# arhik/GaussianSplat

Hardware: AMD Instinct MI355X
Metric: fwd+bwd Msplats/sec at 1M Gaussians, 1920x1080, SH deg 3 (higher is better)
Workload: dtype f32; 1 GPU; C3: 1000000 gaussians, 1920x1080, SH3, ONE camera view per step, fwd+bwd; the steps cycle over the cameras [0, 4] (view k: eye rotated about +y by 45k degrees; one view slot per camera); synthetic scene of SURVEY 8d with the quaternions NORMALISED (8d leaves N(0,1)^4 raw: the reference never normalises q and |q| scales every footprint by |q|^4; un-normalised q is parity-tested, tests/test_gpu_size; views_per_rank=1, nranks=1, settle_steps=24, rank_mode=1, binning_rounds=1, schedule=3, view_slots=True, order=depth_desc, tile=16, instances=30150056, coarse_instances=2175944, walked_fwd=8350144, alpha_cull=True, list_cap=0, tile_parts=1, lists_capped=False

## Files before the change

### gaussiansplat_amd/backend.py

```python
from __future__ import annotations

import ctypes as C
import os
from collections import namedtuple

import numpy as np

_HERE = os.path.dirname(os.path.abspath(__file__))
LIB_PATH = os.environ.get("GSPLAT_HIP_LIB") or os.path.join(_HERE, "lib", "libgsplat_hip.so")

GS_MEM_HOST, GS_MEM_DEVICE = 0, 1
ORDER_INDEX, ORDER_DEPTH_DESC, ORDER_DEPTH_ASC = 0, 1, 2

(ARR_TS, ARR_TPS, ARR_MU, ARR_COV3D, ARR_COV2D, ARR_INVCOV, ARR_BBS, ARR_RGB, ARR_SIG, ARR_DEPTH_KEY,
 ARR_TILE_RECT, ARR_SORT_IDXS, ARR_TILE_RANGES, ARR_SORTED_IDS, ARR_SORTED_KEYS, ARR_GRAD2D) = range(16)

STAGES = ("preprocess", "depth_sort", "count_scan", "emit", "tile_sort", "ranges", "composite_fwd",
          "composite_bwd", "preprocess_bwd")

GS_CAMERA_GRAD_FLOATS = 40
GS_METRIC_SUMS = 4
GS_EXPOSURE_FLOATS = 12
(METRIC_MSE, METRIC_MAE, METRIC_SSIM, METRIC_PSNR, GS_METRIC_COUNT) = range(5)
GS_ABI_VERSION = 3
GS_DEBUG_WIDE_CURSORS = 1
GS_DEBUG_ALWAYS_ORDER = 2
GS_DEBUG_SUPER16 = 8
GS_DEBUG_SUPER8 = 16
GS_DEBUG_NO_TAIL_FILL = 32
GS_DEBUG_TINY_CAPS = 4
GS_MAX_VIEW_SLOTS = 4096
GS_BWD_OVERWRITE, GS_BWD_COMPOSITE_ONLY, GS_BWD_PARAMS_ONLY, GS_BWD_PARAMS_SH, GS_BWD_PARAMS_GEOM = 1, 2, 4, 8, 16
GS_ADAM_GROUPS = 6
GS_ADAM_SELECTIVE = 1
GS_ERR_INVALID, GS_ERR_UNSUPPORTED = -1, -5
KNN_BOX = 64
TOUCHED_CHUNK = 256


class GsConfig(C.Structure):
    _fields_ = [("struct_size", C.c_int32), ("abi_version", C.c_int32), ("tile_size", C.c_int32), ("order", C.c_int32), ("t_min", C.c_float),
                ("deterministic", C.c_int32), ("export_debug", C.c_int32), ("profile_stages", C.c_int32),
                ("bin_path", C.c_int32), ("rank_mode", C.c_int32), ("alpha_cull", C.c_int32), ("schedule", C.c_int32),
                ("slab_mode", C.c_int32), ("slab_max_ratio", C.c_float), ("slab_fractions", C.c_float * 3), ("debug_flags", C.c_int32),
                ("depth_sort", C.c_int32), ("list_cap", C.c_int32), ("tile_parts", C.c_int32), ("reserved", C.c_int32 * 3)]


class GsGrads(C.Structure):
    _fields_ = [("d_means", C.c_void_p), ("d_scales", C.c_void_p), ("d_quats", C.c_void_p),
                ("d_opacities", C.c_void_p), ("d_shs", C.c_void_p)]


class GsDensityStats(C.Structure):
    _fields_ = [("grad_sum", C.c_void_p), ("count", C.c_void_p), ("max_extent", C.c_void_p)]


class GsDensityParams(C.Structure):
    _fields_ = [("struct_size", C.c_int32), ("grad_threshold", C.c_float), ("log_split_scale", C.c_float), ("log_shrink", C.c_float),
                ("min_opacity_logit", C.c_float), ("log_max_world_scale", C.c_float), ("max_extent_px", C.c_int32)]


class GsError(RuntimeError):
    def __init__(self, code: int, msg: str):
# ... 47 lines not shown
    "gs_adam_step": Sig(_i, [_vp, _G, _G, _G, _fp, _f, _f, _f, _i64, _i]),
    "gs_backward_adam": Sig(_i, [_vp, _vp, _i, _G, _G, _fp, _f, _f, _f, _i64, _i]),
    "gs_density_accumulate": Sig(_i, [_vp, C.POINTER(GsDensityStats)]),
    "gs_density_decide": Sig(_i, [_vp, C.POINTER(GsDensityStats), C.POINTER(GsDensityParams), _vp]),
    "gs_density_plan": Sig(_i, [_vp, _vp, _i64p]),
    "gs_density_restructure": Sig(_i, [_vp, _vp, _vp, _G, _i32, _G, _G, _i64]),
    "gs_opacity_reset": Sig(_i, [_vp, _f, _vp, _vp]),
    "gs_mcmc_plan": Sig(_i, [_vp, _f, _vp, _vp, _i64p]),
    "gs_mcmc_sample": Sig(_i, [_vp, _vp, _i64, _vp, _i64, _vp]),
    "gs_mcmc_relocate": Sig(_i, [_vp, _vp, _vp, _i64, _f, _i32, _G]),
    "gs_mcmc_noise": Sig(_i, [_vp, _vp, _f, _f, _f]),
    "gs_mcmc_regularize": Sig(_i, [_vp, _G, _f, _f]),
    "gs_knn_mean_dist2": Sig(_i, [_vp, _vp, _i64, _vp]),
    "gs_init_from_points": Sig(_i, [_vp, _vp, _vp, _vp, _i64, _i, _f, _G]),
    "gs_view_depth": Sig(_i, [_vp, _vp]),
    "gs_view_depth_backward": Sig(_i, [_vp, _vp, _vp]),
    "gs_render_features": Sig(_i, [_vp, _vp, _vp, _vp]),
    "gs_backward_features": Sig(_i, [_vp, _vp, _vp, _vp, _vp, _G]),
    "gs_backward_camera": Sig(_i, [_vp, _vp, _i]),
    "gs_image_metrics": Sig(_i, [_vp, _vp, _vp, _vp, _i32, _i32, _i32, _vp, _vp, _i]),
    "gs_metrics_finish": Sig(_i, [_dp, _dp]),
    "gs_exposure_apply": Sig(_i, [_vp, _vp, _vp, _vp, _i32, _i32, _vp]),
    "gs_exposure_backward": Sig(_i, [_vp, _vp, _vp, _vp, _vp, _i32, _i32, _vp, _vp]),
    "gs_exposure_adam": Sig(_i, [_vp, _vp, _vp, _vp, _vp, _f, _f, _f, _f, _i64]),
    "gs_num_gaussians": Sig(_i64, [_vp]),
    "gs_num_instances": Sig(_i64, [_vp]),
    "gs_num_coarse_instances": Sig(_i64, [_vp]),
    "gs_num_rounds": Sig(_i, [_vp]),
    "gs_get_array": Sig(_i, [_vp, _i, _vp, _i64]),
    "gs_get_stage_times": Sig(_i, [_vp, _fp]),
    "gs_get_stage_stats": Sig(_i, [_vp, _dp, _i64p, _i]),
    "gs_get_work_counters": Sig(_i, [_vp, _i64p, _i64p]),
    "gs_get_list_stats": Sig(_i, [_vp, _i64p]),
    "gs_get_tile_parts": Sig(_i, [_vp]),
    "gs_get_bin_path": Sig(_i, [_vp]),
    "gs_get_work_counters_ex": Sig(_i, [_vp, _i64p]),
    "gs_debug_time_composite": Sig(_i, [_vp, _i, _i, _i, _fp]),
    "gs_debug_tile_clock": Sig(_i, [_vp, _i, _i, _vp]),
    "gs_debug_tile_clock_rows": Sig(_i, [_vp]),
    "gs_debug_tail_fill": Sig(_i, [_vp, _i32p], optional=True),
    "gs_debug_clock_mhz": Sig(_i, [_vp, _fp]),
    "gs_debug_set_window": Sig(_i, [_vp, _i32, _i32]),
    "gs_rank_probe_result": Sig(_i, [_vp]),
}
SYMBOLS = tuple(ABI)

_lib = None


def load():
    global _lib
    if _lib is not None:
        return _lib
    try:
        import torch
    except ImportError:
        pass
    if not os.path.exists(LIB_PATH):
        raise FileNotFoundError(f"{LIB_PATH} not found: build it with `python -m gaussiansplat_amd.build` "
                                "(there is no CPU fallback)")
    L = C.CDLL(LIB_PATH)
    for name, sig in ABI.items():
        try:
            f = getattr(L, name)
        except AttributeError:
            if sig.optional:
# ... 388 lines not shown
                ARR_BBS: ((n, 4), np.float32), ARR_RGB: ((n, 3), np.float32), ARR_SIG: ((n,), np.float32),
                ARR_DEPTH_KEY: ((n,), np.uint32), ARR_TILE_RECT: ((n, 4), np.uint16), ARR_SORT_IDXS: ((n,), np.uint32),
                ARR_SORTED_IDS: ((ni,), np.uint32), ARR_SORTED_KEYS: ((ni,), np.uint64), ARR_GRAD2D: ((n, 10), np.float32)}
        if which == ARR_TILE_RANGES:
            ntiles = ((self.W + 15) // 16) * ((self.H + 15) // 16)
            shape, dt = (ntiles, 2), np.uint32
        else:
            shape, dt = spec[which]
        out = np.empty(shape, dt)
        self._chk(self.L.gs_get_array(self.h, which, out.ctypes.data, out.nbytes))
        return out

    def stage_stats(self, reset: bool = False) -> dict:
        sm = (C.c_double * len(STAGES))()
        ct = (C.c_int64 * len(STAGES))()
        self._chk(self.L.gs_get_stage_stats(self.h, sm, ct, int(reset)))
        return {k: (float(sm[i]), int(ct[i])) for i, k in enumerate(STAGES)}

    def work_counters(self):
        a, b = C.c_int64(), C.c_int64()
        self._chk(self.L.gs_get_work_counters(self.h, C.byref(a), C.byref(b)))
        return int(a.value), int(b.value)

    def work_counters_ex(self) -> dict:
        o = (C.c_int64 * 4)()
        self._chk(self.L.gs_get_work_counters_ex(self.h, o))
        return dict(walked_fwd=int(o[0]), walked_bwd=int(o[1]), evaluated_fwd=int(o[2]), evaluated_bwd=int(o[3]))

    def list_stats(self) -> dict:
        o = (C.c_int64 * 3)()
        self._chk(self.L.gs_get_list_stats(self.h, o))
        return dict(listed=int(o[0]), extended_segments=int(o[1]), capped=bool(o[2]))

    def tile_parts_of_frame(self) -> int:
        rc = self.L.gs_get_tile_parts(self.h)
        if rc < 0:
            self._chk(rc)
        return int(rc)

    def bin_path_of_frame(self) -> int:
        rc = self.L.gs_get_bin_path(self.h)
        if rc < 0:
            self._chk(rc)
        return int(rc)

    def time_composite(self, which: int, variant: int, reps: int = 10) -> float:
        ms = C.c_float()
        self._chk(self.L.gs_debug_time_composite(self.h, which, variant, reps, C.byref(ms)))
        return float(ms.value)

    def tile_clock(self, which: int, variant: int = 0) -> np.ndarray:
        ntiles = ((self.W + 15) // 16) * ((self.H + 15) // 16)
        rows = ntiles
        if variant < 0:
            rows = int(self.L.gs_debug_tile_clock_rows(self.h))
            if rows <= 0:
                raise GsError(-1, "tile_clock: records by workgroup need a frame with a launch order")
        out = np.zeros((rows, 15), np.uint64)
        self._chk(self.L.gs_debug_tile_clock(self.h, which, variant, out.ctypes.data))
        return out

    def tail_fill_blocks(self):
        o = (C.c_int32 * 2)()
        self._chk(self.L.gs_debug_tail_fill(self.h, o))
        return int(o[0]), int(o[1])

# ... 20 lines not shown
```

### gaussiansplat_amd/csrc/gs_adam.hip

```cpp
#include "gs_ctx.h"
#include "gs_adam.h"
#include "gs_wave.h"

#define GS_ADAM_ROWS 64
#define GS_ADAM_MAX_BLOCKS 2048

namespace {

struct AdamSeg {
    float *p;
    const float *g;
    float *m, *v;
    int64_t len;
    int64_t units;
    int w;
    int sh;
    int vec;
    int lds_off;
    float ss;
};
struct AdamArgs {
    AdamSeg seg[5];
    int nseg;
    int64_t n;
// ... 156 lines not shown
    if (!grads || !exp_avg || !exp_avg_sq) return fail(c, GS_ERR_INVALID, "gs_adam_step: NULL argument");
    const Five<float> p = c->model5_mut(), g = five(*grads), m = five(*exp_avg), v = five(*exp_avg_sq);
    AdamArgs a{};
    if (const int rc = gs_adam_prepare(c, "gs_adam_step", p.p, g.p, m.p, v.p, lr, beta1, beta2, eps, step, flags, &a.h)) return rc;
    if (bind_device(c)) return GS_ERR_HIP;
    const int64_t n = c->n;
    int64_t most = 0;
    int lds = 0;
    for (int i = 0; i < 5; ++i) {
        if (!g[i] || n <= 0) continue;
        AdamSeg &s = a.seg[a.nseg++];
        s.p = p[i]; s.g = g[i]; s.m = m[i]; s.v = v[i];
        s.w = (int)c->width[i]; s.len = (int64_t)s.w * n;
        s.sh = i == 4; s.ss = a.h.step_size[i < 4 ? i : 4];
        s.vec = ((reinterpret_cast<uintptr_t>(s.p) | reinterpret_cast<uintptr_t>(s.g) | reinterpret_cast<uintptr_t>(s.m) |
                  reinterpret_cast<uintptr_t>(s.v)) & 15) == 0;
        s.units = s.vec ? (s.len + 3) / 4 : s.len;
        s.lds_off = lds; lds += GS_ADAM_ROWS * s.w;
        most = std::max(most, s.units);
    }
    a.n = n;
    if (a.nseg) {
        if (flags & GS_ADAM_SELECTIVE) {
            const int64_t npass = (n + GS_ADAM_ROWS - 1) / GS_ADAM_ROWS;
            const unsigned grid = (unsigned)std::min<int64_t>(npass, GS_ADAM_MAX_BLOCKS);
            hipLaunchKernelGGL(gs_adam_selective_kernel, dim3(grid), dim3(256), sizeof(float) * lds, c->stream, a);
        } else {
            const unsigned grid = (unsigned)std::min<int64_t>((most + 255) / 256, GS_ADAM_MAX_BLOCKS);
            hipLaunchKernelGGL(gs_adam_dense_kernel, dim3(grid), dim3(256), 0, c->stream, a);
        }
        HIPCHK(c, hipGetLastError());
    }
    c->inputs_changed();
    return GS_OK;
}
```

### gaussiansplat_amd/csrc/gs_api.hip

```cpp
#include "gs_ctx.h"

std::string g_create_error;

template <typename A> static int preprocess_outputs(gs_ctx *c, A &a) {
    a.gx = c->gx; a.gy = c->gy;
    a.payload = c->payload.as<GsPayload>(); a.invcov = c->invcov.as<float>(); a.depth_key = c->depth_key.as<uint32_t>(); a.rect = c->rect.as<uint16_t>();
    if (!c->cfg.export_debug) return GS_OK;
    for (int i = 0; i < gs_ctx::DBG_COUNT; ++i) HIPCHK(c, c->dbg[i].ensure(sizeof(float) * gs_ctx::DBG_WIDTH[i] * c->n1()));
    auto arr = [c](gs_ctx::Dbg i) { return c->dbg[i].as<float>(); };
    a.dbg.mu = arr(gs_ctx::DBG_MU); a.dbg.cov2d = arr(gs_ctx::DBG_COV2D); a.dbg.invcov = arr(gs_ctx::DBG_INVCOV); a.dbg.bbs = arr(gs_ctx::DBG_BBS);
    if (c->kind == 0) { a.dbg.ts = arr(gs_ctx::DBG_TS); a.dbg.tps = arr(gs_ctx::DBG_TPS); a.dbg.cov3d = arr(gs_ctx::DBG_COV3D); }
    return GS_OK;
}

extern "C" {

void gs_default_config(gs_config *cfg) {
    if (!cfg) return;
    std::memset(cfg, 0, sizeof(*cfg));
    cfg->struct_size = (int32_t)sizeof(gs_config);
    cfg->abi_version = GS_ABI_VERSION;
    cfg->tile_size = GS_TILE;
    cfg->order = GS_ORDER_DEPTH_DESC;
    cfg->t_min = 1e-5f;
    cfg->deterministic = 0;
    cfg->export_debug = 0;
    cfg->profile_stages = 0;
    cfg->rank_mode = 1;
    cfg->alpha_cull = 1;
    cfg->schedule = 3;
    cfg->slab_mode = 1;
}

int gs_abi_version(void) { return GS_ABI_VERSION; }

const char *gs_last_error(const gs_ctx *ctx) { return ctx ? ctx->err.c_str() : g_create_error.c_str(); }

int gs_create(gs_ctx **out, int device, const gs_config *cfg) {
    if (!out) return fail(nullptr, GS_ERR_INVALID, "gs_create: out is NULL");
    *out = nullptr;
    gs_config c0;
    gs_default_config(&c0);
    if (cfg) {
        if (cfg->struct_size != (int32_t)sizeof(gs_config) || cfg->abi_version != GS_ABI_VERSION)
            return fail(nullptr, GS_ERR_INVALID, "gs_create: gs_config.struct_size / abi_version mismatch (caller built against another gsplat.h)");
        c0 = *cfg;
    }
    if (c0.schedule == 0) c0.schedule = 3;
    if (c0.tile_size != GS_TILE) return fail(nullptr, GS_ERR_UNSUPPORTED, "gs_create: only tile_size 16 is supported (reference threads=(16,16))");
    if (c0.order < GS_ORDER_INDEX || c0.order > GS_ORDER_DEPTH_ASC) return fail(nullptr, GS_ERR_INVALID, "gs_create: bad order");
    if (!(c0.t_min >= 0.0f)) return fail(nullptr, GS_ERR_INVALID, "gs_create: t_min must be >= 0");
    if (c0.schedule != 1 && c0.schedule != 3 && c0.schedule != 4) return fail(nullptr, GS_ERR_INVALID, "gs_create: bad schedule (0, 1, 3 or 4)");
    if (c0.slab_mode < 0 || c0.slab_mode > 1) return fail(nullptr, GS_ERR_INVALID, "gs_create: bad slab_mode");
    if (c0.bin_path < 0 || c0.bin_path > 3) return fail(nullptr, GS_ERR_INVALID, "gs_create: bad bin_path");
    if (!(c0.slab_max_ratio >= 0.0f && c0.slab_max_ratio <= 1.0f)) return fail(nullptr, GS_ERR_INVALID, "gs_create: slab_max_ratio must be in [0, 1]");
    for (int i = 0; i < 3; ++i)
        if (!(c0.slab_fractions[i] >= 0.0f && c0.slab_fractions[i] < 1.0f)) return fail(nullptr, GS_ERR_INVALID, "gs_create: slab_fractions must be in [0, 1)");
    if (c0.debug_flags & ~(GS_DEBUG_WIDE_CURSORS | GS_DEBUG_ALWAYS_ORDER | GS_DEBUG_TINY_CAPS | GS_DEBUG_SUPER16 | GS_DEBUG_SUPER8 | GS_DEBUG_NO_TAIL_FILL)) return fail(nullptr, GS_ERR_INVALID, "gs_create: unknown debug_flags");
    if (c0.depth_sort < 0 || c0.depth_sort > 2) return fail(nullptr, GS_ERR_INVALID, "gs_create: depth_sort must be 0, 1 or 2");
    if (c0.list_cap < 0 || c0.list_cap > 2) return fail(nullptr, GS_ERR_INVALID, "gs_create: list_cap must be 0, 1 or 2");
    if (c0.tile_parts != 0 && c0.tile_parts != 1 && c0.tile_parts != 2 && c0.tile_parts != 4) return fail(nullptr, GS_ERR_INVALID, "gs_create: tile_parts must be 0, 1, 2 or 4");
    int ndev = 0;
    hipError_t e = hipGetDeviceCount(&ndev);
    if (e != hipSuccess || ndev <= 0)
        return fail(nullptr, GS_ERR_NO_DEVICE, "gs_create: no HIP device (this library has no CPU fallback)");
    if (device < 0 || device >= ndev) return fail(nullptr, GS_ERR_INVALID, "gs_create: device index out of range");
    gs_ctx *c = new (std::nothrow) gs_ctx();
    if (!c) return fail(nullptr, GS_ERR_OOM, "gs_create: host allocation failed");
    c->device = device;
    c->cfg = c0;
    c->slots.resize(GS_MAX_VIEW_SLOTS + 1);
    if ((e = hipSetDevice(device)) != hipSuccess) { delete c; return hipfail(nullptr, e, "hipSetDevice"); }
    if ((e = hipStreamCreateWithFlags(&c->stream, hipStreamNonBlocking)) != hipSuccess) { delete c; return hipfail(nullptr, e, "hipStreamCreate"); }
    c->own_stream = true;
    {
        hipDeviceProp_t prop;
        if (hipGetDeviceProperties(&prop, device) == hipSuccess && prop.multiProcessorCount > 0) c->wave_slots = prop.multiProcessorCount * 4 * 5;
        else (void)hipGetLastError();
    }
    if ((e = hipHostMalloc((void **)&c->pinned, sizeof(PinnedWords), hipHostMallocCoherent | hipHostMallocMapped)) != hipSuccess) { delete c; return hipfail(nullptr, e, "hipHostMalloc"); }
    if ((e = hipHostMalloc((void **)&c->pinned_split, sizeof(uint32_t) * 2 * (GS_MAX_VIEW_SLOTS + 1), hipHostMallocCoherent | hipHostMallocMapped)) != hipSuccess) {
        (void)hipGetLastError(); c->pinned_split = nullptr;
    } else std::memset(c->pinned_split, 0, sizeof(uint32_t) * 2 * (GS_MAX_VIEW_SLOTS + 1));
    for (auto &pair : c->ev)
        for (hipEvent_t &ev : pair) if ((e = hipEventCreate(&ev)) != hipSuccess) { delete c; return hipfail(nullptr, e, "hipEventCreate"); }
    if ((e = hipEventCreateWithFlags(&c->ev_count, hipEventDisableTiming | hipEventReleaseToSystem)) != hipSuccess) { delete c; return hipfail(nullptr, e, "hipEventCreate"); }
    if ((e = hipStreamCreateWithFlags(&c->side, hipStreamNonBlocking)) != hipSuccess) { delete c; return hipfail(nullptr, e, "hipStreamCreate"); }
    for (hipEvent_t *ev : {&c->ev_main, &c->ev_order})
        if ((e = hipEventCreateWithFlags(ev, hipEventDisableTiming)) != hipSuccess) { delete c; return hipfail(nullptr, e, "hipEventCreate"); }
    if (c->cfg.rank_mode == 0) {
        int bad = 0;
        if ((e = gs_probe_lds_atomic_order(c->stream, &bad)) != hipSuccess) { delete c; return hipfail(nullptr, e, "gs_probe_lds_atomic_order"); }
        c->rank_probe = bad ? 1 : 0;
        if (bad) c->cfg.rank_mode = 1;
    }
    *out = c;
    return GS_OK;
}

int gs_destroy(gs_ctx *c) {
    if (!c) return GS_OK;
    (void)hipSetDevice(c->device);
    (void)hipStreamSynchronize(c->stream);
    if (c->side) (void)hipStreamSynchronize(c->side);
    delete c;
    return GS_OK;
}

int gs_set_stream(gs_ctx *c, void *hip_stream) {
    if (!c) return GS_ERR_INVALID;
    hipStream_t want = hip_stream == (void *)1 ? (hipStream_t) nullptr : (hipStream_t)hip_stream;
    if (hip_stream && !c->own_stream && c->stream == want && c->borrowed_stream) return GS_OK;
    if (bind_device(c)) return GS_ERR_HIP;
    HIPCHK(c, hipStreamSynchronize(c->stream));
    if (c->side) HIPCHK(c, hipStreamSynchronize(c->side));
    if (c->own_stream && c->stream) { (void)hipStreamDestroy(c->stream); c->own_stream = false; }
    if (hip_stream) { c->stream = want; c->borrowed_stream = true; }
    else { HIPCHK(c, hipStreamCreateWithFlags(&c->stream, hipStreamNonBlocking)); c->own_stream = true; c->borrowed_stream = false; }
    return GS_OK;
}

int gs_synchronize(gs_ctx *c) {
    if (!c) return GS_ERR_INVALID;
    if (bind_device(c)) return GS_ERR_HIP;
    HIPCHK(c, hipStreamSynchronize(c->stream));
    if (c->side) HIPCHK(c, hipStreamSynchronize(c->side));
    return GS_OK;
}

static int adopt_model(gs_ctx *c, int64_t n, int sh_degree, int kind, const float *const src[5], const size_t (&width)[5], int mem) {
    if (bind_device(c)) return GS_ERR_HIP;
    const float *dst[5];
    for (int i = 0; i < 5; ++i) {
        dst[i] = src[i];
        if (mem != GS_MEM_HOST) continue;
        const size_t bytes = sizeof(float) * width[i] * (size_t)n;
        HIPCHK(c, c->model[i].ensure(bytes ? bytes : 4));
        if (bytes) HIPCHK(c, hipMemcpyAsync(c->model[i].p, src[i], bytes, hipMemcpyHostToDevice, c->stream));
        dst[i] = c->model[i].as<float>();
    }
    if (mem == GS_MEM_HOST) HIPCHK(c, hipStreamSynchronize(c->stream));
    c->n = n; c->sh_degree = sh_degree; c->kind = kind;
    for (int i = 0; i < 5; ++i) c->width[i] = width[i];
    c->set_model5(dst);
    c->inputs_changed();
    return GS_OK;
}

int gs_set_model(gs_ctx *c, int64_t n, int sh_degree, const float *means, const float *scales, const float *quats,
                 const float *opacities, const float *shs, int mem) {
    if (!c) return GS_ERR_INVALID;
    if (n < 0 || n > 0x7FFFFFF0LL) return fail(c, GS_ERR_INVALID, "gs_set_model: n out of range");
    if (sh_degree < 0 || sh_degree > 3) return fail(c, GS_ERR_UNSUPPORTED, "gs_set_model: sh_degree must be 0..3");
    if (n > 0 && (!means || !scales || !quats || !opacities || !shs)) return fail(c, GS_ERR_INVALID, "gs_set_model: NULL array");
    if (const int rc = need_mem(c, "gs_set_model", mem)) return rc;
    const int K = (sh_degree + 1) * (sh_degree + 1);
    const float *src[5] = {means, scales, quats, opacities, shs};
    return adopt_model(c, n, sh_degree, 0, src, {3, 3, 4, 1, (size_t)3 * K}, mem);
}

int gs_set_model_2d(gs_ctx *c, int64_t n, const float *means, const float *scales, const float *rotations,
                    const float *opacities, const float *colors, int mem) {
    if (!c) return GS_ERR_INVALID;
    if (n < 0 || n > 0x7FFFFFF0LL) return fail(c, GS_ERR_INVALID, "gs_set_model_2d: n out of range");
    if (n > 0 && (!means || !scales || !rotations || !opacities || !colors)) return fail(c, GS_ERR_INVALID, "gs_set_model_2d: NULL array");
    if (const int rc = need_mem(c, "gs_set_model_2d", mem)) return rc;
    const float *src[5] = {means, scales, rotations, opacities, colors};
    return adopt_model(c, n, 0, 1, src, {2, 2, 1, 1, 3}, mem);
}

int gs_set_active_sh_degree(gs_ctx *c, int degree) {
    if (!c) return GS_ERR_INVALID;
    if (const int rc = need_3d(c, "gs_set_active_sh_degree")) return rc;
    if (degree < -1 || degree > 3) return fail(c, GS_ERR_INVALID, "gs_set_active_sh_degree: degree must be -1 (the model's own) or 0..3");
    const int before = c->active_sh_degree();
    c->sh_active_request = degree;
    if (c->active_sh_degree() != before) c->inputs_changed();
    return GS_OK;
}

int gs_get_active_sh_degree(const gs_ctx *c) {
    if (!c) return GS_ERR_INVALID;
    if (c->kind != 0) return GS_ERR_UNSUPPORTED;
    return c->active_sh_degree();
}

int gs_set_background(gs_ctx *c, const float rgb[3]) {
    if (!c) return GS_ERR_INVALID;
    if (!rgb) return fail(c, GS_ERR_INVALID, "gs_set_background: NULL argument");
    for (int i = 0; i < 3; ++i)
        if (!std::isfinite(rgb[i])) return fail(c, GS_ERR_INVALID, "gs_set_background: the components must be finite");
    if (rgb[0] == c->background[0] && rgb[1] == c->background[1] && rgb[2] == c->background[2]) return GS_OK;
    for (int i = 0; i < 3; ++i) c->background[i] = rgb[i];
    c->fall_back(gs_ctx::Stage::BINNED);
    return GS_OK;
}

int gs_get_background(const gs_ctx *c, float rgb[3]) {
    if (!c || !rgb) return GS_ERR_INVALID;
    for (int i = 0; i < 3; ++i) rgb[i] = c->background[i];
    return GS_OK;
}

int gs_compose_target(gs_ctx *c, const float *rgba, int32_t W, int32_t H, float *rgb_out) {
    if (!c) return GS_ERR_INVALID;
    if (!rgba || !rgb_out) return fail(c, GS_ERR_INVALID, "gs_compose_target: NULL argument");
    if (const int rc = need_image_size(c, "gs_compose_target", W, H)) return rc;
    const size_t px = (size_t)W * H;
    if (overlaps({rgb_out, sizeof(float) * 3 * px}, {rgba, sizeof(float) * 4 * px})) return fail(c, GS_ERR_INVALID, "gs_compose_target: rgb_out overlaps rgba");
    if (bind_device(c)) return GS_ERR_HIP;
    HIPCHK(c, gs_launch_compose_target(rgba, rgb_out, px, c->background, c->stream));
    return GS_OK;
}

int gs_set_image_size(gs_ctx *c, int32_t W, int32_t H) {
    if (!c) return GS_ERR_INVALID;
    if (const int rc = need_image_size(c, "gs_set_image_size", W, H)) return rc;
    if (!c->have_cam) {
        std::memset(&c->cam, 0, sizeof(c->cam));
        c->cam.near_ = -1.0f; c->cam.far_ = 1.0f;
    }
    c->cam.W = W; c->cam.H = H;
    c->have_cam = true;
    c->inputs_changed();
    return GS_OK;
}

int gs_set_camera(gs_ctx *c, const float T[16], const float P[16], float fx, float fy, float near_, float far_,
                  const float eye[3], const float lookAt[3], int32_t W, int32_t H) {
    if (!c) return GS_ERR_INVALID;
    if (!T || !P || !eye || !lookAt) return fail(c, GS_ERR_INVALID, "gs_set_camera: NULL argument");
    if (const int rc = need_image_size(c, "gs_set_camera", W, H)) return rc;
    std::memcpy(c->cam.T, T, sizeof(float) * 16);
    std::memcpy(c->cam.P, P, sizeof(float) * 16);
    c->cam.fx = fx; c->cam.fy = fy; c->cam.near_ = near_; c->cam.far_ = far_;
    for (int i = 0; i < 3; ++i) { c->cam.eye[i] = eye[i]; c->cam.lookAt[i] = lookAt[i]; }
    c->cam.W = W; c->cam.H = H;
    c->have_cam = true;
    c->inputs_changed();
    return GS_OK;
}

int gs_preprocess(gs_ctx *c) {
    if (!c) return GS_ERR_INVALID;
    if (!c->have_cam) return fail(c, GS_ERR_INVALID, "gs_preprocess: gs_set_camera first");
    if (bind_device(c)) return GS_ERR_HIP;
    if (int rc = settle_totals(c, nullptr, false)) return rc;
    c->frame_id += 1;
    HIPCHK(c, c->payload.ensure(sizeof(GsPayload) * c->n1()));
    HIPCHK(c, c->invcov.ensure(sizeof(float) * 4 * c->n1()));
    HIPCHK(c, c->depth_key.ensure(sizeof(uint32_t) * c->n1()));
    HIPCHK(c, c->rect.ensure(sizeof(uint16_t) * 4 * c->n1()));
    c->gx = (c->cam.W + GS_TILE - 1) / GS_TILE;
    c->gy = (c->cam.H + GS_TILE - 1) / GS_TILE;
    c->range_valid = false;
    GsPreprocessArgs a{};
    GsPreprocess2DArgs a2{};
    if (c->kind == 1) {
        a2.n = c->n; a2.W = c->cam.W; a2.H = c->cam.H;
        a2.means = c->means; a2.scales = c->scales; a2.rots = c->quats; a2.opac = c->opac; a2.colors = c->shs;
        if (int rc = preprocess_outputs(c, a2)) return rc;
    } else {
        model_head(c, a);
        a.order = c->cfg.order;
        if (c->dsort_can_bucket() && c->order() != GS_ORDER_INDEX && c->n > 0 && !c->small_bin_possible()) {
            if (!c->key_range.p) {
                HIPCHK(c, c->key_range.ensure(sizeof(uint32_t) * gs_depth_range_words()));
                HIPCHK(c, gs_depth_range_reset(c->key_range.as<uint32_t>(), c->stream));
            }
            c->range_parity ^= 1;
            a.key_range = key_range_of(c, c->range_parity);
            c->range_valid = true;
        }
        if (int rc = preprocess_outputs(c, a)) return rc;
    }
    StageTimer t(c, GS_STAGE_PREPROCESS);
    HIPCHK(c, c->kind == 1 ? gs_launch_preprocess2d(a2, c->stream) : gs_launch_preprocess(a, c->cam, c->sh_row_floats(), c->stream));
    c->reach(gs_ctx::Stage::PREPROCESSED);
    return GS_OK;
}

int gs_loss_l1_dssim(gs_ctx *c, const float *img, const float *gt, int32_t W, int32_t H, int32_t C, float lam, float *dC,
                     double *loss_out, int mem) {
    if (!c || !img || !gt) return GS_ERR_INVALID;
    if (W <= 0 || H <= 0 || C <= 0) return fail(c, GS_ERR_INVALID, "gs_loss_l1_dssim: bad image size");
    if (const int rc = need_mem(c, "gs_loss_l1_dssim", mem)) return rc;
    if (bind_device(c)) return GS_ERR_HIP;
    const size_t n = (size_t)W * H * C;
    HIPCHK(c, c->loss_maps.ensure(sizeof(float) * 3 * n));
    HIPCHK(c, c->loss_acc.ensure(sizeof(double) * GS_LOSS_SLOTS * GS_LOSS_SLOT_STRIDE));
    const float *d_img = img, *d_gt = gt;
    float *d_dc = dC;
    if (mem == GS_MEM_HOST) {
        HIPCHK(c, c->loss_in[0].ensure(sizeof(float) * n));
        HIPCHK(c, c->loss_in[1].ensure(sizeof(float) * n));
        HIPCHK(c, hipMemcpyAsync(c->loss_in[0].p, img, sizeof(float) * n, hipMemcpyHostToDevice, c->stream));
        HIPCHK(c, hipMemcpyAsync(c->loss_in[1].p, gt, sizeof(float) * n, hipMemcpyHostToDevice, c->stream));
        d_img = c->loss_in[0].as<float>(); d_gt = c->loss_in[1].as<float>();
    }
    if (mem == GS_MEM_HOST || !dC) { HIPCHK(c, c->loss_dc.ensure(sizeof(float) * n)); d_dc = c->loss_dc.as<float>(); }
    float win[121];
    {
        double k[121], sum = 0.0;
        for (int j = 0; j < 11; ++j)
            for (int i = 0; i < 11; ++i) { k[j * 11 + i] = std::exp(-std::sqrt((double)((5 - j) * (5 - j) + (5 - i) * (5 - i)))); sum += k[j * 11 + i]; }
        for (int i = 0; i < 121; ++i) win[i] = (float)(k[i] / sum);
    }
    HIPCHK(c, gs_loss_run(W, H, C, d_img, d_gt, c->loss_maps.as<float>(), c->loss_acc.as<double>(), d_dc, lam, win, c->stream));
    if (mem == GS_MEM_HOST && dC) HIPCHK(c, hipMemcpyAsync(dC, d_dc, sizeof(float) * n, hipMemcpyDeviceToHost, c->stream));
    if (loss_out) {
        double slots[GS_LOSS_SLOTS * GS_LOSS_SLOT_STRIDE], acc[2] = {0.0, 0.0};
        HIPCHK(c, hipMemcpyAsync(slots, c->loss_acc.p, sizeof(slots), hipMemcpyDeviceToHost, c->stream));
        HIPCHK(c, hipStreamSynchronize(c->stream));
        for (int k = 0; k < GS_LOSS_SLOTS; ++k) { acc[0] += slots[k * GS_LOSS_SLOT_STRIDE]; acc[1] += slots[k * GS_LOSS_SLOT_STRIDE + 1]; }
        *loss_out = (1.0 - (double)lam) * acc[0] / (2.0 * (double)n) + (double)lam * (1.0 - acc[1] / (double)n) / 2.0;
    } else if (mem == GS_MEM_HOST) {
        HIPCHK(c, hipStreamSynchronize(c->stream));
    }
    return GS_OK;
}

int gs_sgd_step(gs_ctx *c, float lr, const gs_grads *g) {
    if (!c || !g) return GS_ERR_INVALID;
    if (bind_device(c)) return GS_ERR_HIP;
    const size_t n = (size_t)c->n;
    const Five<float> p = c->model5_mut(), gr = five(*g);
    for (int i = 0; i < 5; ++i) HIPCHK(c, gs_launch_sgd(p[i], gr[i], lr, c->width[i] * n, c->stream));
    c->inputs_changed();
    return GS_OK;
}

int gs_reset_grads(gs_ctx *c, const gs_grads *g) {
    if (!c || !g) return GS_ERR_INVALID;
    if (bind_device(c)) return GS_ERR_HIP;
    const size_t n = (size_t)c->n;
    const Five<float> p = five(*g);
    for (int i = 0; i < 5; ++i)
        if (p[i] && n) HIPCHK(c, hipMemsetAsync(p[i], 0, sizeof(float) * c->width[i] * n, c->stream));
    return GS_OK;
}

int gs_grads_alloc(gs_ctx *c, gs_grads *out) {
    if (!c || !out) return GS_ERR_INVALID;
    if (bind_device(c)) return GS_ERR_HIP;
    const size_t n = (size_t)c->n;
    size_t off[6] = {0, 0, 0, 0, 0, 0};
    for (int i = 0; i < 5; ++i) off[i + 1] = off[i] + c->width[i] * n;
    const size_t total = off[5];
    HIPCHK(c, c->grads_flat.ensure(sizeof(float) * (total ? total : 1)));
    HIPCHK(c, hipMemsetAsync(c->grads_flat.p, 0, sizeof(float) * total, c->stream));
    float *f = c->grads_flat.as<float>();
    out->d_means = f; out->d_scales = f + off[1]; out->d_quats = f + off[2]; out->d_opacities = f + off[3]; out->d_shs = f + off[4];
    return GS_OK;
}

int gs_grads_read(gs_ctx *c, const gs_grads *g, float *h_means, float *h_scales, float *h_quats, float *h_opacities, float *h_shs) {
    if (!c || !g) return GS_ERR_INVALID;
    if (bind_device(c)) return GS_ERR_HIP;
    const size_t n = (size_t)c->n;
    const Five<float> src = five(*g);
    float *dst[5] = {h_means, h_scales, h_quats, h_opacities, h_shs};
    for (int i = 0; i < 5; ++i)
// ... 7 lines not shown
```

### gaussiansplat_amd/csrc/gs_api_bin.hip

```cpp
#include "gs_ctx.h"
using Path = gs_ctx::BinPlan::Path;

#define GS_SLAB_MAX_RATIO 0.03
static double slab_max_ratio(const gs_ctx *c) { return c->cfg.slab_max_ratio > 0.0f ? (double)c->cfg.slab_max_ratio : GS_SLAB_MAX_RATIO; }
static void plan_rounds(const gs_ctx *c, gs_ctx::BinPlan &p) {
    p.n_rounds = 1;
    p.slab_lo[0] = 0; p.slab_lo[1] = c->n;
    if ((p.path != Path::TWO_LEVEL && p.path != Path::RADIX32) || c->cfg.t_min <= 0.0f || c->n < 1024 || c->order() == GS_ORDER_INDEX) return;
    double f[GS_MAX_ROUNDS] = {1.0, 1.0, 1.0, 1.0};
    int R = 1;
    if (c->cfg.slab_fractions[0] > 0.0f) {
        for (int k = 0; k < 3 && k + 1 < GS_MAX_ROUNDS && c->cfg.slab_fractions[k] > 0.0f; ++k) { f[k] = c->cfg.slab_fractions[k]; R = k + 2; }
    } else if (c->cfg.slab_mode == 1 && c->walked_ratio >= 0.0 && c->walked_ratio < slab_max_ratio(c)) {
        const double rho = c->walked_ratio;
        f[0] = std::min(0.9, std::max(0.02, 2.0 * rho + 0.02));
        f[1] = std::min(0.95, std::max(f[0] + 0.05, 6.0 * rho + 0.05));
        R = 3;
    }
    if (R == 1) return;
    int64_t prev = 0;
    int r = 0;
    for (int k = 0; k + 1 < R; ++k) {
        int64_t b = (int64_t)(f[k] * (double)c->n);
        b = std::min(c->n, std::max(prev, b));
        if (b > prev && b < c->n) { p.slab_lo[++r] = b; prev = b; }
    }
    p.slab_lo[++r] = c->n;
    p.n_rounds = r;
}

static void plan_bin(gs_ctx *c) {
    gs_ctx::BinPlan p{};
    const int64_t ntiles = c->ntiles();
    p.tile_bits = 1;
    while ((1LL << p.tile_bits) < ntiles) ++p.tile_bits;
    p.gid_bits = 1;
    while ((1LL << p.gid_bits) < c->n) ++p.gid_bits;
    const int passes = (p.tile_bits + 7) / 8;
    p.lo_bits = passes <= 1 ? p.tile_bits : (p.tile_bits + 1) / 2; p.hi_bits = p.tile_bits - p.lo_bits;
    p.sbs = gs_bin3_sb_shift(c->gx, c->gy, (c->cfg.debug_flags & GS_DEBUG_SUPER16) ? 4 : (c->cfg.debug_flags & GS_DEBUG_SUPER8) ? 3 : 0);
    const int sb = 1 << p.sbs;
    p.sgx = (c->gx + sb - 1) / sb; p.sgy = (c->gy + sb - 1) / sb;
    const int asked = c->cfg.bin_path == 3 ? 0 : c->cfg.bin_path;
    const bool fast = asked != 1 && passes <= 2 && p.hi_bits + p.gid_bits <= 32 && gs_tile_ranges_supported(c->gx, c->gy);
    p.path = c->small_bin_possible() ? Path::SMALL : fast && asked == 0 && gs_bin3_supported(p.ns()) ? Path::TWO_LEVEL : fast ? Path::RADIX32 : Path::RADIX64;
    p.perm_on_demand = p.path == Path::SMALL && c->order() != GS_ORDER_INDEX;
    plan_rounds(c, p);
    c->bin = p;
}

static GsBin3L1 two_level_args(gs_ctx *c, const uint32_t *perm_slab, int64_t n_all, int64_t nr, const uint8_t *sdone, size_t cap_coarse, size_t cap_fine) {
    GsBin3L1 b{};
    b.rect = c->rect.as<uint16_t>(); b.perm = perm_slab; b.sdone = sdone; b.n = n_all; b.n_slab = nr; b.sgx = c->bin.sgx; b.ns = c->bin.ns(); b.sbs = c->bin.sbs;
    b.rect_sorted = c->rect_sorted.as<uint32_t>(); b.table = c->l1_table.as<uint32_t>(); b.row_total = c->l1_rows.as<uint32_t>();
    b.partials = c->l1_partials.as<uint32_t>(); b.totals = c->bin_totals(); b.cranges = c->cranges.as<uint32_t>();
    b.cids = c->cids.as<uint32_t>(); b.clr = c->clr.as<uint16_t>();
    b.tilecnt = c->tilecnt.as<uint32_t>(); b.ntiles = (int)c->ntiles();
    b.cap_coarse = (uint32_t)std::min<size_t>(cap_coarse, 0xFFFFFFFEu); b.cap_fine = (uint32_t)std::min<size_t>(cap_fine, 0xFFFFFFFEu);
    return b;
}
static int two_level_count(gs_ctx *c, const uint32_t *perm_slab, int64_t n_all, int64_t nr, const uint8_t *sdone, bool to_host = false) {
    const int ns = c->bin.ns();
    HIPCHK(c, c->rect_sorted.ensure(sizeof(uint32_t) * 2 * (size_t)(nr ? nr : 1)));
    HIPCHK(c, c->l1_table.ensure(sizeof(uint32_t) * gs_bin3_table_words(nr, ns)));
    HIPCHK(c, c->l1_rows.ensure(sizeof(uint32_t) * (size_t)ns));
    HIPCHK(c, c->l1_partials.ensure(sizeof(uint32_t) * gs_bin3_partial_words(n_all, ns)));
    HIPCHK(c, c->counters.ensure(GS_COUNTER_BYTES));
    HIPCHK(c, c->cranges.ensure(sizeof(uint32_t) * 2 * (size_t)ns));
    HIPCHK(c, c->tilecnt.ensure(sizeof(uint32_t) * c->ntiles()));
    GsBin3L1 b = two_level_args(c, perm_slab, n_all, nr, sdone, 0, 0);
    if (to_host) {
        b.host_totals = c->pinned->counters.totals; b.host_walked = c->pinned->counters.work; b.walked_src = c->counters.as<uint32_t>();
        if (!c->counters_here()) c->prev_counters_valid = false;
        b.tile_walked = c->prev_counters_valid ? c->last_walked : nullptr; b.n_tile_walked = (int)c->ntiles();
    }
    HIPCHK(c, gs_bin3_l1_count(b, c->stream));
    return GS_OK;
}
static int two_level_lists(gs_ctx *c, const uint32_t *perm_slab, int64_t n_all, int64_t nr, size_t coarse, size_t fine, uint32_t *ranges, uint32_t *ids_out,
                           const uint8_t *done, const uint8_t *sdone, const uint32_t *cap_src = nullptr) {
    const int ns = c->bin.ns();
    gs_ctx::FrameLive &live = c->live;
    assert(done || (!live.frame_capped && !live.have_l2));
    if (!done) live.cap_src = cap_src;
    if (coarse == 0) {
        HIPCHK(c, hipMemsetAsync(ranges, 0, sizeof(uint32_t) * 2 * c->ntiles(), c->stream));
        return GS_OK;
    }
    const int64_t max_work = gs_bin3_max_work((int64_t)coarse, ns);
    HIPCHK(c, c->cids.ensure(sizeof(uint32_t) * coarse));
    HIPCHK(c, c->clr.ensure(sizeof(uint16_t) * coarse));
    HIPCHK(c, c->segcnt.ensure(sizeof(uint32_t) * ((size_t)1 << (2 * c->bin.sbs)) * (size_t)max_work));
    HIPCHK(c, gs_bin3_l1_scatter(two_level_args(c, perm_slab, n_all, nr, sdone, coarse, fine), c->stream));
    GsBin3Args a{};
    a.cranges = c->cranges.as<uint32_t>(); a.cids = c->cids.as<uint32_t>(); a.clr = c->clr.as<uint16_t>(); a.ranges = ranges; a.tilecnt = c->tilecnt.as<uint32_t>();
    a.done = done; a.segcnt = c->segcnt.as<uint32_t>(); a.ids_out = ids_out;
    a.gx = c->gx; a.gy = c->gy; a.sgx = c->bin.sgx; a.ns = ns; a.sbs = c->bin.sbs; a.max_work = (int)max_work;
    a.wide = (uint64_t)fine * 4ull >= (1ull << 32) || (c->cfg.debug_flags & GS_DEBUG_WIDE_CURSORS) != 0;
    a.totals = c->bin_totals(); a.cap_coarse = (uint32_t)std::min<size_t>(coarse, 0xFFFFFFFEu); a.cap_fine = (uint32_t)std::min<size_t>(fine, 0xFFFFFFFEu);
    if (cap_src && !done) {
        const size_t nt = (size_t)c->ntiles();
        HIPCHK(c, c->tile_nopen.ensure(sizeof(uint32_t) * nt));
        HIPCHK(c, c->smax.ensure(sizeof(uint32_t) * (size_t)ns));
        HIPCHK(c, c->tile_ext.ensure(sizeof(uint2) * nt));
        a.cap_src = cap_src; a.tile_nopen = c->tile_nopen.as<uint32_t>(); a.smax = c->smax.as<uint32_t>(); a.tile_ext = c->tile_ext.as<uint2>();
        a.ext_count = c->ext_count();
        live.frame_capped = true;
    }
    HIPCHK(c, gs_bin3_build_lists(a, c->stream));
    if (!done) { live.last_l2 = a; live.have_l2 = true; }
    return GS_OK;
}

#define GS_LIST_CAP_MAX_RATIO 0.15
static int list_cap_source(gs_ctx *c, const uint32_t **out) {
    *out = nullptr;
    const int64_t ntiles = c->ntiles(), grid = c->grid_key();
    if (c->bin.path != Path::TWO_LEVEL || c->bin.n_rounds != 1 || c->cfg.list_cap == 1 || !(c->cfg.t_min > 0.0f) || ntiles <= 0) return GS_OK;
    if (c->cfg.debug_flags & GS_DEBUG_TINY_CAPS) {
        if (c->zero_tiles.cap < sizeof(uint32_t) * (size_t)ntiles) {
            HIPCHK(c, c->zero_tiles.ensure(sizeof(uint32_t) * (size_t)ntiles));
            HIPCHK(c, hipMemsetAsync(c->zero_tiles.p, 0, c->zero_tiles.cap, c->stream));
        }
        *out = c->zero_tiles.as<uint32_t>();
        return GS_OK;
    }
    if (c->cfg.list_cap != 2 && (ntiles <= c->wave_slots || !(c->walked_ratio >= 0.0 && c->walked_ratio < GS_LIST_CAP_MAX_RATIO))) return GS_OK;
    const int k = order_index(c);
    if (k == GS_MAX_VIEW_SLOTS && c->cfg.schedule != 4) return GS_OK;
    if (c->slots[k].walked_grid != grid || !c->slots[k].walked().p) return GS_OK;
    *out = c->slots[k].walked().as<uint32_t>();
    return GS_OK;
}

static GsBin2Args bin2_args(gs_ctx *c, int r) {
    const gs_ctx::BinPlan &p = c->bin;
    GsBin2Args b{};
    b.n = p.slab_lo[r + 1] - p.slab_lo[r]; b.n_inst = c->round_gen[r]; b.gx = c->gx; b.lo_bits = p.lo_bits; b.hi_bits = p.hi_bits; b.gid_bits = p.gid_bits;
    b.offsets = (r ? c->offsets_r : c->offsets).as<uint32_t>(); b.perm = c->live.perm_ptr ? c->live.perm_ptr + p.slab_lo[r] : nullptr;
    b.rect = (r ? c->rect_r : c->rect).as<uint16_t>();
    b.cs = c->cs.as<uint32_t>(); b.block_hist = c->table.as<uint32_t>(); b.digit_total = c->digit_total.as<uint32_t>();
    b.buf_a = c->words.as<uint32_t>(); b.ids_out = c->ids.as<uint32_t>() + c->round_ids_off[r]; b.ballot_ranks = c->cfg.rank_mode != 0;
    if (r) { b.done = c->tile_done.as<uint8_t>(); b.live_total = c->live_total.as<uint32_t>() + r; }
    return b;
}

static int bin_round_two_level(gs_ctx *c, int r) {
    const gs_ctx::BinPlan &p = c->bin;
    const int64_t lo = p.slab_lo[r], nr = p.slab_lo[r + 1] - lo;
    const uint32_t *perm = c->live.perm_ptr + lo;
    HIPCHK(c, c->ranges_r[r].ensure(sizeof(uint32_t) * 2 * c->ntiles()));
    HIPCHK(c, c->sdone.ensure((size_t)p.ns()));
    {
        StageTimer t(c, GS_STAGE_COUNT_SCAN);
        HIPCHK(c, gs_launch_super_done(c->tile_done.as<uint8_t>(), c->gx, c->gy, p.sgx, p.sgy, p.sbs, c->sdone.as<uint8_t>(), c->stream));
        if (int rc = two_level_count(c, perm, nr, nr, c->sdone.as<uint8_t>())) return rc;
    }
    HIPCHK(c, hipMemcpyAsync(c->pinned->readback, c->bin_totals(), 2 * sizeof(uint32_t), hipMemcpyDeviceToHost, c->stream));
    HIPCHK(c, hipEventRecord(c->ev_count, c->stream));
    HIPCHK(c, hipEventSynchronize(c->ev_count));
    harvest_events(c);
    const int64_t coarse = (int64_t)c->pinned->readback[0];
    c->round_gen[r] = (int64_t)c->pinned->readback[1];
    c->round_ids_off[r] = c->round_ids_off[r - 1] + (size_t)c->round_gen[r - 1];
    if (c->round_ids_off[r] + (size_t)c->round_gen[r] > (size_t)c->n_inst) return fail(c, GS_ERR_HIP, "gs_forward: slab instance accounting out of range");
    {
        StageTimer t(c, GS_STAGE_TILE_SORT);
        if (int rc = two_level_lists(c, perm, nr, nr, (size_t)coarse, (size_t)c->round_gen[r], c->ranges_r[r].as<uint32_t>(), c->ids.as<uint32_t>() + c->round_ids_off[r],
                                     c->tile_done.as<uint8_t>(), c->sdone.as<uint8_t>())) return rc;
    }
    return GS_OK;
}

int bin_round(gs_ctx *c, int r) {
    if (c->bin.path == Path::TWO_LEVEL) return bin_round_two_level(c, r);
    const int64_t lo = c->bin.slab_lo[r], nr = c->bin.slab_lo[r + 1] - lo;
    const uint32_t *perm = c->live.perm_ptr + lo;
    HIPCHK(c, c->live2d.ensure(sizeof(uint32_t) * 2 * (size_t)(c->gx + 1) * (c->gy + 1)));
    HIPCHK(c, c->rect_r.ensure(sizeof(uint16_t) * 4 * c->n1()));
    HIPCHK(c, c->offsets_r.ensure(sizeof(uint32_t) * ((size_t)nr + 1)));
    HIPCHK(c, c->live_total.ensure(sizeof(uint32_t) * GS_MAX_ROUNDS));
    HIPCHK(c, c->ranges_r[r].ensure(sizeof(uint32_t) * 2 * c->ntiles()));
    {
        StageTimer t(c, GS_STAGE_COUNT_SCAN);
        HIPCHK(c, gs_launch_live_prefix(c->tile_done.as<uint8_t>(), c->gx, c->gy, c->live2d.as<uint32_t>(),
                                        c->live2d.as<uint32_t>() + (size_t)(c->gx + 1) * (c->gy + 1), c->stream));
        HIPCHK(c, gs_launch_count_scan_live(c->rect.as<uint16_t>(), perm, c->live2d.as<uint32_t>(), c->gx, c->rect_r.as<uint16_t>(),
                                            c->offsets_r.as<uint32_t>(), c->block_sums.as<uint32_t>(), nr, c->stream));
    }
    HIPCHK(c, hipMemcpyAsync(c->pinned->readback, c->offsets_r.as<uint32_t>() + nr, sizeof(uint32_t), hipMemcpyDeviceToHost, c->stream));
    HIPCHK(c, hipEventRecord(c->ev_count, c->stream));
    {
        StageTimer t(c, GS_STAGE_RANGES);
        HIPCHK(c, gs_launch_tile_ranges(c->rect_r.as<uint16_t>(), perm, nr, c->diff.as<int>(), c->gx, c->gy, c->ranges_r[r].as<uint32_t>(),
                                        c->tile_done.as<uint8_t>(), c->stream));
    }
    HIPCHK(c, hipEventSynchronize(c->ev_count));
    harvest_events(c, GS_STAGE_RANGES);
    c->round_gen[r] = (int64_t)c->pinned->readback[0];
    c->round_ids_off[r] = c->round_ids_off[r - 1] + (size_t)c->round_gen[r - 1];
    if (c->round_gen[r] == 0) return GS_OK;
    if (c->round_ids_off[r] + (size_t)c->round_gen[r] > (size_t)c->n_inst) return fail(c, GS_ERR_HIP, "gs_forward: slab instance accounting out of range");
    {
        StageTimer t(c, GS_STAGE_TILE_SORT);
        HIPCHK(c, gs_bin2_build_lists(bin2_args(c, r), c->stream));
    }
    return GS_OK;
}

static void dsort_feedback(gs_ctx *c) {
    if (!c->dsort_buckets_used) return;
    c->dsort_buckets_used = false;
    if (*c->dsort_stat() != 0u && c->cfg.depth_sort != 2) c->dsort_classic_until = c->frame_id + 64;
}

static int totals_arrived(gs_ctx *c, uint32_t coarse, uint32_t fine_slab, uint32_t fine_all, const uint32_t *walked_prev) {
    if (fine_all == 0xFFFFFFFFu)
        return fail(c, GS_ERR_UNSUPPORTED, "gs_bin: more than 2^32 - 2 tile instances (32-bit list offsets); reduce the scene or the image");
    if (c->prev_counters_valid && c->prev_n_inst > 0) {
        unsigned long long w = 0;
        std::memcpy(&w, walked_prev, sizeof(w));
        c->walked_ratio = (double)w / (double)c->prev_n_inst;
    }
    c->prev_counters_valid = false;
    c->n_inst = (int64_t)fine_all;
    c->n_coarse = (int64_t)coarse;
    c->round_gen[0] = c->bin.n_rounds > 1 ? (int64_t)fine_slab : c->n_inst;
    c->round_ids_off[0] = 0;
    return GS_OK;
}

int settle_totals(gs_ctx *c, bool *redo, bool may_relist) {
    if (redo) *redo = false;
    if (!c->pending_totals) return GS_OK;
    HIPCHK(c, hipEventSynchronize(c->ev_count));
    c->pending_totals = false;
    harvest_events(c);
    dsort_feedback(c);
    const CounterBlock &h = c->pinned->counters;
    const uint32_t coarse = h.totals[0], fine_slab = h.totals[1];
    if (int rc = totals_arrived(c, coarse, fine_slab, h.totals[2], h.work)) return rc;
    if (!c->live.spec_lists || c->live.speculation_held(coarse, fine_slab)) return GS_OK;
    if (!may_relist) { c->fall_back(gs_ctx::Stage::PREPROCESSED); return GS_OK; }
    HIPCHK(c, c->ids.ensure(sizeof(uint32_t) * (size_t)(c->n_inst ? c->n_inst : 1)));
    c->live.relist_in_full();
    {
        StageTimer t(c, GS_STAGE_TILE_SORT);
        if (int rc = two_level_lists(c, c->live.perm_ptr, c->n, c->bin.slab_lo[1], (size_t)coarse, (size_t)fine_slab, c->ranges.as<uint32_t>(), c->ids.as<uint32_t>(), nullptr, nullptr,
                                     nullptr)) return rc;
    }
    if (redo) *redo = true;
    return GS_OK;
}

int depth_order(gs_ctx *c) {
    const size_t n1 = c->n1();
    StageTimer t(c, GS_STAGE_DEPTH_SORT);
    HIPCHK(c, c->pairs_a.ensure(sizeof(uint64_t) * n1));
    HIPCHK(c, c->pairs_b.ensure(sizeof(uint64_t) * n1));
    HIPCHK(c, c->perm.ensure(sizeof(uint32_t) * n1));
    HIPCHK(c, c->table.ensure(sizeof(uint32_t) * gs_sort_table_entries(c->n)));
    HIPCHK(c, c->digit_total.ensure(sizeof(uint32_t) * 4 * 256));
    int in_b = 0;
    uint32_t *perm = c->perm.as<uint32_t>();
    const bool buckets = c->range_valid && c->dsort_can_bucket();
    c->dsort_buckets_used = buckets;
    if (c->range_valid && !buckets)
        HIPCHK(c, gs_depth_range_reset(key_range_of(c, c->range_parity), c->stream, 1));
    if (buckets) {
        uint32_t *range = key_range_of(c, c->range_parity), *other = key_range_of(c, c->range_parity ^ 1);
        c->dsort_stat_parity = c->range_parity;
        *c->dsort_stat() = 0u;
        HIPCHK(c, gs_depth_sort_buckets(c->depth_key.as<uint32_t>(), c->pairs_a.as<uint64_t>(), c->pairs_b.as<uint64_t>(), c->n, c->table.as<uint32_t>(),
                                        c->digit_total.as<uint32_t>(), perm, range, other, c->dsort_stat(), c->stream, c->cfg.rank_mode != 0));
    } else {
        HIPCHK(c, gs_radix_sort_u64(c->pairs_a.as<uint64_t>(), c->pairs_b.as<uint64_t>(), c->n, 32, 64, c->table.as<uint32_t>(),
                                    c->digit_total.as<uint32_t>(), &in_b, c->stream, c->cfg.rank_mode != 0, perm, c->depth_key.as<uint32_t>()));
    }
    c->live.perm_ptr = perm;
    return GS_OK;
}

static int bin_small(gs_ctx *c) {
    const size_t n = (size_t)c->n, nt = (size_t)c->ntiles();
    HIPCHK(c, c->ids.ensure(sizeof(uint32_t) * n * nt));
    if (c->range_valid)
        HIPCHK(c, gs_depth_range_reset(key_range_of(c, c->range_parity), c->stream, 1));
    GsBinSmallArgs a{};
    a.depth_key = c->order() != GS_ORDER_INDEX ? c->depth_key.as<uint32_t>() : nullptr; a.rect = c->rect.as<uint2>();
    a.n = (int)c->n; a.gx = c->gx; a.gy = c->gy; a.ntiles = (int)nt;
    a.ranges = c->ranges.as<uint32_t>(); a.ids = c->ids.as<uint32_t>(); a.totals = c->bin_totals();
    a.host_totals = c->pinned->counters.totals; a.host_walked = c->pinned->counters.work; a.walked_src = c->counters.as<uint32_t>();
    if (!c->counters_here()) c->prev_counters_valid = false;
    a.tile_walked = c->prev_counters_valid ? c->last_walked : nullptr; a.n_tile_walked = (int)nt;
    {
        HIPCHK(c, c->g2d.ensure(c->g2d_bytes()));
        a.zero = c->g2d.as<uint4>(); a.zero_words16 = c->g2d_bytes() / sizeof(uint4);
    }
    {
        StageTimer t(c, GS_STAGE_TILE_SORT);
        HIPCHK(c, gs_bin_small(a, c->stream));
    }
    c->live.g2d_clean = true;
    HIPCHK(c, hipEventRecord(c->ev_count, c->stream));
    c->pending_totals = true;
    return GS_OK;
}

static int bin_two_level(gs_ctx *c) {
    uint32_t *perm = c->live.perm_ptr;
    const int64_t n0 = c->bin.slab_lo[1];
    {
        StageTimer t(c, GS_STAGE_COUNT_SCAN);
        if (int rc = two_level_count(c, perm, c->n, n0, nullptr, c->n > 0)) return rc;
    }
    if (c->n <= 0) HIPCHK(c, hipMemcpyAsync(&c->pinned->counters, c->counters.p, GS_COUNTER_BYTES, hipMemcpyDeviceToHost, c->stream));
    HIPCHK(c, hipEventRecord(c->ev_count, c->stream));
    c->pending_totals = true;
    const size_t cap_coarse = std::min(c->cids.cap / sizeof(uint32_t), c->clr.cap / sizeof(uint16_t)), cap_fine = c->ids.cap / sizeof(uint32_t);
    const uint32_t *cap_src = nullptr;
    if (int rc = list_cap_source(c, &cap_src)) return rc;
    if (c->bin.n_rounds == 1 && cap_coarse > 0 && cap_fine > 0) {
        c->live.speculate(cap_coarse, cap_fine);
        StageTimer t(c, GS_STAGE_TILE_SORT);
        return two_level_lists(c, perm, c->n, n0, cap_coarse, cap_fine, c->ranges.as<uint32_t>(), c->ids.as<uint32_t>(), nullptr, nullptr, cap_src);
    }
    if (int rc = settle_totals(c, nullptr, true)) return rc;
    HIPCHK(c, c->ids.ensure(sizeof(uint32_t) * (size_t)(c->n_inst ? c->n_inst : 1)));
    StageTimer t(c, GS_STAGE_TILE_SORT);
    return two_level_lists(c, perm, c->n, n0, (size_t)c->n_coarse, (size_t)c->round_gen[0], c->ranges.as<uint32_t>(), c->ids.as<uint32_t>(), nullptr, nullptr, cap_src);
}

static int radix64_lists(gs_ctx *c) {
    const size_t ni1 = c->n_inst ? (size_t)c->n_inst : 1;
    HIPCHK(c, c->inst_a.ensure(sizeof(uint64_t) * ni1));
    HIPCHK(c, c->inst_b.ensure(sizeof(uint64_t) * ni1));
    {
        StageTimer t(c, GS_STAGE_EMIT);
        HIPCHK(c, gs_launch_emit(c->rect.as<uint16_t>(), c->live.perm_ptr, c->offsets.as<uint32_t>(), c->inst_a.as<uint64_t>(), c->n, c->gx, c->stream));
    }
    uint64_t *sorted = nullptr;
    {
        StageTimer t(c, GS_STAGE_TILE_SORT);
        int in_b = 0;
        HIPCHK(c, gs_radix_sort_u64(c->inst_a.as<uint64_t>(), c->inst_b.as<uint64_t>(), c->n_inst, 32, 32 + c->bin.tile_bits,
                                    c->table.as<uint32_t>(), c->digit_total.as<uint32_t>(), &in_b, c->stream, c->cfg.rank_mode != 0));
        sorted = in_b ? c->inst_b.as<uint64_t>() : c->inst_a.as<uint64_t>();
    }
    StageTimer t(c, GS_STAGE_RANGES);
    HIPCHK(c, gs_launch_ranges(sorted, c->n_inst, c->ranges.as<uint32_t>(), c->ntiles(), c->stream));
    HIPCHK(c, gs_launch_split_ids(sorted, c->ids.as<uint32_t>(), c->n_inst, c->stream));
    return GS_OK;
}

static int bin_radix(gs_ctx *c) {
    const size_t n = (size_t)c->n;
    const bool fast = c->bin.path == Path::RADIX32, slabs = c->bin.n_rounds > 1;
    const int64_t n0 = c->bin.slab_lo[1];
    uint32_t *perm = c->live.perm_ptr;
    PinnedWords *h = c->pinned;
    {
        StageTimer t(c, GS_STAGE_COUNT_SCAN);
        HIPCHK(c, c->offsets.ensure(sizeof(uint32_t) * (n + 1)));
        HIPCHK(c, gs_launch_count_scan(c->rect.as<uint16_t>(), perm, c->offsets.as<uint32_t>(), c->block_sums.as<uint32_t>(), c->n, c->stream));
    }
    HIPCHK(c, hipMemcpyAsync(&h->readback[0], c->offsets.as<uint32_t>() + n, sizeof(uint32_t), hipMemcpyDeviceToHost, c->stream));
    HIPCHK(c, hipMemcpyAsync(&h->readback[1], c->offsets.as<uint32_t>() + n0, sizeof(uint32_t), hipMemcpyDeviceToHost, c->stream));
    if (!c->counters_here()) c->prev_counters_valid = false;
    if (c->prev_counters_valid) {
        HIPCHK(c, gs_launch_sum_tiles(c->last_walked, c->tile_work.as<uint32_t>(), (int)c->ntiles(), c->counters.as<unsigned long long>(), c->stream));
        HIPCHK(c, hipMemcpyAsync(h->walked_prev, c->counters.p, sizeof(uint64_t), hipMemcpyDeviceToHost, c->stream));
    }
    HIPCHK(c, hipEventRecord(c->ev_count, c->stream));
    if (fast) {
        HIPCHK(c, c->diff.ensure(sizeof(int) * gs_tile_ranges_scratch_ints(c->gx, c->gy)));
        StageTimer t(c, GS_STAGE_RANGES);
        HIPCHK(c, gs_launch_tile_ranges(c->rect.as<uint16_t>(), slabs ? perm : nullptr, slabs ? n0 : c->n, c->diff.as<int>(), c->gx, c->gy,
                                        c->ranges.as<uint32_t>(), nullptr, c->stream));
    }
    HIPCHK(c, hipEventSynchronize(c->ev_count));
    harvest_events(c, fast ? GS_STAGE_RANGES : -1);
    dsort_feedback(c);
    if (int rc = totals_arrived(c, 0, h->readback[1], h->readback[0], h->walked_prev)) return rc;
    const size_t ni1 = c->n_inst ? (size_t)c->n_inst : 1;
    HIPCHK(c, c->table.ensure(sizeof(uint32_t) * gs_sort_table_entries(c->n_inst > c->n ? c->n_inst : c->n)));
    HIPCHK(c, c->digit_total.ensure(sizeof(uint32_t) * 4 * 256));
    HIPCHK(c, c->ids.ensure(sizeof(uint32_t) * ni1));
    if (!fast) return radix64_lists(c);
    const size_t nchunks = ((size_t)c->n_inst + 4095) / 4096;
    HIPCHK(c, c->cs.ensure(sizeof(uint32_t) * (nchunks + 2)));
    if (c->bin.hi_bits > 0) HIPCHK(c, c->words.ensure(sizeof(uint32_t) * ni1));
    StageTimer t(c, GS_STAGE_TILE_SORT);
    HIPCHK(c, gs_bin2_build_lists(bin2_args(c, 0), c->stream));
    return GS_OK;
}

static int bin_frame(gs_ctx *c) {
    const Path path = c->bin.path;
    if (c->order() != GS_ORDER_INDEX && path != Path::SMALL) { if (int rc = depth_order(c)) return rc; }
    HIPCHK(c, c->ranges.ensure(sizeof(uint32_t) * 2 * c->ntiles1()));
    HIPCHK(c, c->counters.ensure(GS_COUNTER_BYTES));
    if (path != Path::SMALL) HIPCHK(c, c->block_sums.ensure(sizeof(uint32_t) * 3 * ((size_t)c->n / 2048 + 2)));
    if (int rc = path == Path::SMALL ? bin_small(c) : path == Path::TWO_LEVEL ? bin_two_level(c) : bin_radix(c)) return rc;
    c->reach(gs_ctx::Stage::BINNED);
    return GS_OK;
}

extern "C" int gs_bin(gs_ctx *c, int32_t gx, int32_t gy) {
    if (!c) return GS_ERR_INVALID;
    if (const int rc = need_stage(c, gs_ctx::Stage::PREPROCESSED, "gs_bin: gs_preprocess first")) return rc;
    if ((gx != 0 || gy != 0) && (gx != c->gx || gy != c->gy))
        return fail(c, GS_ERR_UNSUPPORTED, "gs_bin: blocks must equal ceil(W/16) x ceil(H/16)");
    if (bind_device(c)) return GS_ERR_HIP;
    if (int rc = settle_totals(c, nullptr, false)) return rc;
    c->live = gs_ctx::FrameLive{};
    plan_bin(c);
    return bin_frame(c);
}
```

### gaussiansplat_amd/csrc/gs_api_composite.hip

```cpp
#include "gs_ctx.h"

using Snap = gs_ctx::FramePlan::Snap;
using Stage = gs_ctx::Stage;
using BackwardPlan = gs_ctx::BackwardPlan;
using Update = BackwardPlan::Update;

static const uint32_t *forward_order(gs_ctx *c, const uint32_t **split) {
    const int64_t ntiles = c->ntiles();
    if (!lpt_schedule(c) || ntiles <= 0 || ntiles > GS_LPT_MAX_TILES) return nullptr;
    const int k = order_index(c);
    if (k == GS_MAX_VIEW_SLOTS && c->cfg.schedule != 4) return nullptr;
    gs_ctx::ViewSlot &vs = c->slots[k];
    if (vs.tiles != c->grid_key()) return nullptr;
    if (c->order_pending) {
        if (hipStreamWaitEvent(c->stream, c->ev_order, 0) != hipSuccess) return nullptr;
        c->order_pending = false;
    }
    *split = c->split_word(k, vs.sel);
    return vs.order[vs.sel].as<uint32_t>();
}

static int parts_that_fit(const gs_ctx *c, int units) {
    const long long w = (long long)units * c->ntiles();
    return 4 * w <= c->wave_slots ? 4 : 2 * w <= c->wave_slots ? 2 : 1;
}

static void plan_frame(gs_ctx *c, const uint32_t *order, const uint32_t *order_split, const uint32_t *hist) {
    gs_ctx::FramePlan p;
    const int want = c->cfg.tile_parts;
    const bool whole = !(c->cfg.t_min > 0.0f) || c->bin.n_rounds > 1 || c->live.frame_capped;
    p.parts = p.bwd_parts = want == 1 || whole ? 1 : (want == 2 || want == 4) ? want : parts_that_fit(c, 1);
    p.order = p.bwd_order = order;
    p.side = order && use_side_stream(c);
    p.front = lpt_front(c);
    p.split = p.front > 0 && p.parts == 1 && c->bin.n_rounds == 1;
    const bool may_split = !order_split || *order_split != 0u;
    if (order && p.split && c->snap_walked.p && may_split) {
        p.snap = Snap::HEAVY;
        p.snap_walked = c->snap_walked.as<uint32_t>() + (size_t)c->snap_parity * GS_SEG_SLOTS;
    } else if (hist && want == 0 && p.parts > 1 && !lpt_schedule(c) && c->kind == 0 && c->ntiles() > 0) {
        p.snap = Snap::ALL;
        p.seg_n = 2; p.seg_hist = hist;
        p.bwd_parts = parts_that_fit(c, p.seg_n);
    }
    c->plan = p;
}

GsCompositeArgs composite_args(gs_ctx *c, bool bwd, int r, bool debug) {
    const gs_ctx::FramePlan &p = c->plan;
    GsCompositeArgs a{};
    a.W = c->cam.W; a.H = c->cam.H; a.gx = c->gx; a.gy = c->gy; a.t_min = c->cfg.t_min;
    a.payload = c->payload.as<GsPayload>(); a.image = c->img(); a.trans = c->tr();
    a.cull = c->cfg.alpha_cull != 0;
    for (int q = 0; q < c->bin.n_rounds; ++q) {
        if (q > 0 && c->round_gen[q] == 0) continue;
        a.seg_ranges[a.nseg] = q == 0 ? c->ranges.as<uint32_t>() : c->ranges_r[q].as<uint32_t>();
        a.seg_ids[a.nseg] = c->ids.as<uint32_t>() + c->round_ids_off[q];
        ++a.nseg;
    }
    a.ranges = r == 0 ? c->ranges.as<uint32_t>() : c->ranges_r[r].as<uint32_t>(); a.ids = c->ids.as<uint32_t>() + c->round_ids_off[r];
    if (bwd) c->rows_mut(c->g2d).into(a);
    a.tile_order = bwd || debug ? p.bwd_order : p.order; a.order_len = a.tile_order ? lpt_order_entries(c) : 0;
    a.parts = bwd ? p.bwd_parts : p.parts;
    a.split_ok = a.tile_order && p.split && !c->live.frame_capped;
    if (c->live.frame_capped && c->bin.n_rounds == 1) {
        a.tile_ext = c->tile_ext.as<uint2>();
        if (!bwd) {
            a.cranges = c->cranges.as<uint32_t>(); a.cids = c->cids.as<uint32_t>(); a.clr = c->clr.as<uint16_t>();
            a.ids_w = c->ids.as<uint32_t>(); a.sgx = c->bin.sgx; a.sbs = c->bin.sbs; a.ext_count = c->ext_count();
        }
    }
    if (bwd ? p.bwd_segments : !debug) {
        if (p.snap == Snap::ALL) { a.snap = c->snap.as<float>(); a.seg_hist = p.seg_hist; a.seg_n = p.seg_n; }
        if (p.snap == Snap::HEAVY && a.split_ok) {
            a.snap = c->snap.as<float>(); a.seg_len = order_seg_len(c, a.tile_order); a.front = p.front; a.snap_walked = p.snap_walked;
        }
    }
    return a;
}

static int build_frame_order(gs_ctx *c) {
    gs_ctx::FramePlan &p = c->plan;
    const int64_t ntiles = c->ntiles();
    if (!lpt_schedule(c) || ntiles <= 0 || ntiles > GS_LPT_MAX_TILES) return GS_OK;
    const int k = order_index(c);
    gs_ctx::ViewSlot &vs = c->slots[k];
    const int dst = vs.order_dst(p.order != nullptr);
    DevBuf &ob = vs.order[dst];
    HIPCHK(c, ob.ensure(sizeof(uint32_t) * ((size_t)lpt_order_entries(c) + GS_SEG_SLOTS + 16)));
    const uint32_t *walked = p.front > 0 ? c->last_walked : nullptr;
    uint32_t *rearm = nullptr, *nsplit = c->split_word(k, dst);
    if (nsplit) *nsplit = 0xFFFFFFFFu;
    if (p.front > 0) {
        if (!c->snap_walked.p) {
            HIPCHK(c, c->snap_walked.ensure(sizeof(uint32_t) * 2 * GS_SEG_SLOTS));
            HIPCHK(c, hipMemsetAsync(c->snap_walked.p, 0, sizeof(uint32_t) * 2 * GS_SEG_SLOTS, c->stream));
        }
        rearm = c->snap_walked.as<uint32_t>() + (size_t)(c->snap_parity ^ 1) * GS_SEG_SLOTS;
    }
    if (p.side) {
        if (c->order_pending) HIPCHK(c, hipStreamWaitEvent(c->stream, c->ev_order, 0));
        HIPCHK(c, hipEventRecord(c->ev_main, c->stream));
// ... 72 lines not shown
    c->counters_grid = c->grid_key();
    gs_ctx::ViewSlot *vs = order_index(c) < GS_MAX_VIEW_SLOTS || c->cfg.schedule == 4 ? &c->slots[order_index(c)] : nullptr;
    const uint32_t *hist = nullptr;
    if (vs) {
        HIPCHK(c, vs->walk_dst().ensure(sizeof(uint32_t) * nt1));
        if (vs->walked_grid == c->counters_grid) hist = vs->walked().as<uint32_t>();
        c->last_walked = vs->walk_dst().as<uint32_t>();
    } else {
        HIPCHK(c, c->tile_walked.ensure(sizeof(uint32_t) * nt1));
        c->last_walked = c->tile_walked.as<uint32_t>();
    }
    const int R = c->bin.n_rounds;
    if (R > 1) {
        HIPCHK(c, c->tile_pos.ensure(sizeof(uint32_t) * nt1));
        HIPCHK(c, c->tile_done.ensure(nt1));
        HIPCHK(c, c->tile_dead.ensure(sizeof(unsigned long long) * 4 * nt1));
        HIPCHK(c, hipMemsetAsync(c->tile_pos.p, 0, sizeof(uint32_t) * ntiles, c->stream));
    }
    c->snap_parity ^= 1;
    const uint32_t *order_split = nullptr, *const order = forward_order(c, &order_split);
    if (c->order_pending) { HIPCHK(c, hipStreamWaitEvent(c->stream, c->ev_order, 0)); c->order_pending = false; }
    plan_frame(c, order, order_split, hist);
    c->fwd_fills_g2d = c->tail_fill() && !c->live.g2d_clean && c->g2d.p && c->g2d.cap >= c->g2d_bytes() &&
                       gs_composite_fill_blocks(c->g2d.p, c->g2d_bytes()) > 0;
    for (int r = 0; r < R; ++r) {
        if (r > 0) { if (int rc = bin_round(c, r)) return rc; }
        if (int rc = enqueue_forward_round(c, r)) return rc;
        if (r == 0) {
            bool redo = false;
            if (int rc = settle_totals(c, &redo, true)) return rc;
            if (redo) { if (int rc = enqueue_forward_round(c, 0)) return rc; }
        }
    }
    if (c->fwd_fills_g2d) c->live.g2d_clean = true;
    if (vs) vs->walk_written(c->counters_grid);
    if (int rc = build_frame_order(c)) return rc;
    const hipMemcpyKind kind = mem == GS_MEM_HOST ? hipMemcpyDeviceToHost : hipMemcpyDeviceToDevice;
    if (image && image != c->img()) HIPCHK(c, hipMemcpyAsync(image, c->img(), sizeof(float) * 3 * px, kind, c->stream));
    if (transmittance && transmittance != c->tr()) HIPCHK(c, hipMemcpyAsync(transmittance, c->tr(), sizeof(float) * px, kind, c->stream));
    if (mem == GS_MEM_HOST && (image || transmittance)) HIPCHK(c, hipStreamSynchronize(c->stream));
    c->reach(Stage::RENDERED);
    c->prev_counters_valid = true; c->prev_n_inst = c->n_inst;
    return GS_OK;
}

static int plan_backward(gs_ctx *c, const float *dC, int mem, const gs_grads *grads, int flags, BackwardPlan &p) {
    if (!c) return GS_ERR_INVALID;
    if (p.fused()) { if (const int rc = need_3d(c, p.update == Update::SGD ? "gs_backward_sgd" : "gs_backward_adam")) return rc; }
    if (const int rc = need_stage(c, Stage::RENDERED, "gs_backward: gs_forward first")) return rc;
    const bool params_only = (flags & GS_BWD_PARAMS_ONLY) != 0, composite_only = (flags & GS_BWD_COMPOSITE_ONLY) != 0;
    if (params_only && composite_only) return fail(c, GS_ERR_INVALID, "gs_backward: COMPOSITE_ONLY and PARAMS_ONLY exclude each other");
    const int chain = (flags & (GS_BWD_PARAMS_SH | GS_BWD_PARAMS_GEOM)) >> 3;
    if (chain && !params_only) return fail(c, GS_ERR_INVALID, "gs_backward: GS_BWD_PARAMS_SH / _GEOM need GS_BWD_PARAMS_ONLY");
    if (chain) { if (const int rc = need_3d(c, "gs_backward: GS_BWD_PARAMS_SH / _GEOM")) return rc; }
    if (params_only) { if (const int rc = need_stage(c, Stage::COMPOSITE_ADJOINT, "gs_backward: GS_BWD_PARAMS_ONLY needs a GS_BWD_COMPOSITE_ONLY call on this frame")) return rc; }
    if ((!dC && !params_only) || (!grads && !p.fused() && !composite_only)) return fail(c, GS_ERR_INVALID, "gs_backward: NULL argument");
    if (const int rc = need_mem(c, "gs_backward", mem)) return rc;
    p.composite = !params_only;
    p.chain = composite_only ? 0 : chain ? chain : 3;
    if (!p.fused() && (flags & GS_BWD_OVERWRITE)) p.update = Update::OVERWRITE;
    if (p.fused()) p.target = c->model5_mut(); else if (grads) p.target = five(*grads);
    p.dC = dC;
    p.stage_dC = mem == GS_MEM_HOST && p.composite;
    p.host_sync = mem == GS_MEM_HOST;
    p.fill_g2d = p.composite && !c->live.g2d_clean;
    p.fill_shs = c->tail_fill() && p.composite && p.chain == 3 && c->kind == 0 && p.update == Update::OVERWRITE &&
                 gs_composite_fill_blocks(p.target[4], c->shs_bytes()) > 0;
    return GS_OK;
}

static int run_backward(gs_ctx *c, const BackwardPlan &p) {
    if (bind_device(c)) return GS_ERR_HIP;
    const size_t px = c->pixels();
    const float *dC_dev = p.dC;
    if (p.stage_dC) {
        HIPCHK(c, c->stage_in.ensure(sizeof(float) * 3 * px));
        HIPCHK(c, hipMemcpyAsync(c->stage_in.p, p.dC, sizeof(float) * 3 * px, hipMemcpyHostToDevice, c->stream));
        dC_dev = c->stage_in.as<float>();
    }
    HIPCHK(c, c->g2d.ensure(c->g2d_bytes()));
    HIPCHK(c, c->ensure_bwd_counters());
    if (p.composite) {
        GsCompositeArgs a = composite_args(c, true, 0);
        a.dC = c->last_dC = dC_dev;
        a.tile_walked = c->tile_walked_b.as<uint32_t>(); a.tile_work = c->tile_work_b.as<uint32_t>();
        if (p.fill_shs) { a.fill_dst = p.target[4]; a.fill_bytes = c->shs_bytes(); a.fill_blocks = gs_composite_fill_blocks(a.fill_dst, a.fill_bytes); a.fill_nt = 1; }
        if (p.fill_g2d) HIPCHK(c, hipMemsetAsync(c->g2d.p, 0, c->g2d_bytes(), c->stream));
        c->live.rows_dirtied();
        {
            StageTimer t(c, GS_STAGE_COMPOSITE_BWD);
            HIPCHK(c, gs_launch_composite_bwd(a, c->stream));
        }
        c->fill_blocks_bwd = a.fill_blocks;
    }
    const int overwrite = p.update == Update::ACCUMULATE || p.update == Update::SGD ? 0 : 1;
    if (p.chain && c->kind == 1) {
        GsPreprocess2DBwdArgs b2{};
        b2.n = c->n; b2.W = c->cam.W; b2.H = c->cam.H;
        b2.scales = c->scales; b2.rots = c->quats; b2.opac = c->opac;
        c->rows(c->g2d).into(b2); b2.overwrite = overwrite;
        b2.d_means = p.target[0]; b2.d_scales = p.target[1]; b2.d_rots = p.target[2]; b2.d_opac = p.target[3]; b2.d_colors = p.target[4];
        StageTimer t(c, GS_STAGE_PREPROCESS_BWD);
        HIPCHK(c, gs_launch_preprocess2d_bwd(b2, c->stream));
    } else if (p.chain) {
        HIPCHK(c, c->dpc.ensure(sizeof(float) * 4 * c->n1()));
        const GsPreprocessBwdArgs b = chain_args(c, c->rows(c->g2d), c->dpc.as<float>(), p.target, overwrite, p.fill_shs ? 1 : 0,
                                                 p.update == Update::SGD ? -p.lr : 0.0f);
        const GsPreprocessBwdMode mode{p.chain, p.adam, p.update == Update::ADAM_DENSE ? 1 : p.update == Update::ADAM_SELECTIVE ? 2 : 0};
        StageTimer t(c, GS_STAGE_PREPROCESS_BWD);
        HIPCHK(c, gs_launch_preprocess_bwd(b, c->cam, c->stream, mode));
    }
    if (p.host_sync) HIPCHK(c, hipStreamSynchronize(c->stream));
    if (p.model_changes()) c->inputs_changed();
    else c->reach(p.chain ? Stage::BACKWARD : Stage::COMPOSITE_ADJOINT);
    return GS_OK;
}

int gs_backward(gs_ctx *c, const float *dC, int mem, const gs_grads *grads) { return gs_backward_ex(c, dC, mem, grads, 0); }

int gs_backward_ex(gs_ctx *c, const float *dC, int mem, const gs_grads *grads, int flags) {
    BackwardPlan p;
    if (const int rc = plan_backward(c, dC, mem, grads, flags, p)) return rc;
    return run_backward(c, p);
}

int gs_backward_sgd(gs_ctx *c, const float *dC, int mem, float lr) {
    if (!c) return GS_ERR_INVALID;
    if (!(lr != 0.0f)) return fail(c, GS_ERR_INVALID, "gs_backward_sgd: lr must be non-zero");
    BackwardPlan p;
    p.update = Update::SGD; p.lr = lr;
    if (const int rc = plan_backward(c, dC, mem, nullptr, 0, p)) return rc;
    return run_backward(c, p);
}

int gs_backward_adam(gs_ctx *c, const float *dC, int mem, const gs_grads *exp_avg, const gs_grads *exp_avg_sq, const float lr[GS_ADAM_GROUPS],
                     float beta1, float beta2, float eps, int64_t step, int flags) {
    if (!c) return GS_ERR_INVALID;
    if (!dC || !exp_avg || !exp_avg_sq) return fail(c, GS_ERR_INVALID, "gs_backward_adam: NULL argument");
    GsAdamFused ad{};
    const Five<float> m = five(*exp_avg), v = five(*exp_avg_sq);
    for (int i = 0; i < 5; ++i) {
        if (!m[i] || !v[i]) return fail(c, GS_ERR_INVALID, "gs_backward_adam: all ten moment arrays must be non-NULL");
        ad.m[i] = m[i]; ad.v[i] = v[i];
    }
    if (const int rc = gs_adam_prepare(c, "gs_backward_adam", c->model5().p, nullptr, m.p, v.p, lr, beta1, beta2, eps, step, flags, &ad.h)) return rc;
    BackwardPlan p;
    p.update = (flags & GS_ADAM_SELECTIVE) ? Update::ADAM_SELECTIVE : Update::ADAM_DENSE; p.adam = &ad;
// ... 28 lines not shown
```

### gaussiansplat_amd/csrc/gs_api_debug.hip

```cpp
#include "gs_ctx.h"
#include "gs_pergaussian.h"

using Stage = gs_ctx::Stage;

extern "C" {

int64_t gs_num_gaussians(const gs_ctx *c) { return c ? c->n : 0; }
int64_t gs_num_instances(gs_ctx *c) { if (!c) return 0; (void)settle_totals(c, nullptr, true); return c->n_inst; }
int64_t gs_num_coarse_instances(gs_ctx *c) { if (!c) return 0; (void)settle_totals(c, nullptr, true); return c->bin.radix() ? 0 : c->n_coarse; }
int gs_num_rounds(const gs_ctx *c) { return c ? c->bin.n_rounds : 0; }

int gs_get_array(gs_ctx *c, int which, void *dst, int64_t bytes) {
    if (!c || !dst) return GS_ERR_INVALID;
    if (bind_device(c)) return GS_ERR_HIP;
    const size_t n = (size_t)c->n;
    const void *src = nullptr;
    size_t need = 0;
    auto need_dbg = [&](gs_ctx::Dbg i) -> int {
        if (!c->cfg.export_debug) return fail(c, GS_ERR_INVALID, "gs_get_array: needs gs_config.export_debug = 1");
        src = c->dbg[i].p; need = sizeof(float) * gs_ctx::DBG_WIDTH[i] * n; return GS_OK;
    };
    int rc = GS_OK;
    if (which <= GS_ARR_TILE_RECT && (rc = need_stage(c, Stage::PREPROCESSED, "gs_get_array: gs_preprocess first"))) return rc;
    if (which >= GS_ARR_SORT_IDXS && which <= GS_ARR_SORTED_KEYS && (rc = need_stage(c, Stage::BINNED, "gs_get_array: gs_bin first"))) return rc;
    if (which >= GS_ARR_TILE_RANGES && which <= GS_ARR_SORTED_KEYS && (rc = settle_totals(c, nullptr, true))) return rc;
    if (which >= GS_ARR_TILE_RANGES && which <= GS_ARR_SORTED_KEYS && c->bin.n_rounds > 1)
        return fail(c, GS_ERR_INVALID, "gs_get_array: this frame was binned in depth slabs (lists spread over rounds); use gs_config.slab_mode = 0");
    if ((which == GS_ARR_SORTED_IDS || which == GS_ARR_SORTED_KEYS) && c->live.frame_capped && c->live.have_l2) {
        GsBin3Args a = c->live.last_l2;
        a.cap_src = nullptr; a.tile_nopen = nullptr; a.smax = nullptr; a.tile_ext = nullptr;
        HIPCHK(c, gs_bin3_write_lists(a, c->stream));
        c->live.frame_capped = false;
    }
    switch (which) {
        case GS_ARR_TS: if ((rc = need_dbg(gs_ctx::DBG_TS))) return rc; break;
        case GS_ARR_TPS: if ((rc = need_dbg(gs_ctx::DBG_TPS))) return rc; break;
        case GS_ARR_COV3D: if ((rc = need_dbg(gs_ctx::DBG_COV3D))) return rc; break;
        case GS_ARR_COV2D: if ((rc = need_dbg(gs_ctx::DBG_COV2D))) return rc; break;
        case GS_ARR_BBS: if ((rc = need_dbg(gs_ctx::DBG_BBS))) return rc; break;
        case GS_ARR_INVCOV: src = c->invcov.p; need = sizeof(float) * 4 * n; break;
        case GS_ARR_MU: case GS_ARR_RGB: case GS_ARR_SIG: {
            const size_t w = which == GS_ARR_MU ? 2 : which == GS_ARR_RGB ? 3 : 1;
            if ((size_t)bytes != sizeof(float) * w * n) return fail(c, GS_ERR_INVALID, "gs_get_array: size mismatch");
            std::vector<GsPayload> h(c->n1());
            HIPCHK(c, hipMemcpyAsync(h.data(), c->payload.p, sizeof(GsPayload) * n, hipMemcpyDeviceToHost, c->stream));
            HIPCHK(c, hipStreamSynchronize(c->stream));
            float *o = static_cast<float *>(dst);
            for (size_t g = 0; g < n; ++g) {
                const GsPayload &p = h[g];
                if (which == GS_ARR_MU) { o[2 * g] = p.mx; o[2 * g + 1] = p.my; }
                else if (which == GS_ARR_RGB) { o[3 * g] = p.r; o[3 * g + 1] = p.g; o[3 * g + 2] = p.b; }
                else o[g] = p.sig;
            }
            return GS_OK;
        }
        case GS_ARR_DEPTH_KEY: src = c->depth_key.p; need = sizeof(uint32_t) * n; break;
        case GS_ARR_TILE_RECT: src = c->rect.p; need = sizeof(uint16_t) * 4 * n; break;
        case GS_ARR_SORT_IDXS: {
            if ((size_t)bytes != sizeof(uint32_t) * n) return fail(c, GS_ERR_INVALID, "gs_get_array: size mismatch");
            if (c->bin.perm_on_demand && !c->live.perm_ptr && (rc = depth_order(c))) return rc;
            if (c->live.perm_ptr) { src = c->live.perm_ptr; need = sizeof(uint32_t) * n; break; }
            uint32_t *o = static_cast<uint32_t *>(dst);
            for (size_t g = 0; g < n; ++g) o[g] = (uint32_t)g;
            return GS_OK;
        }
        case GS_ARR_TILE_RANGES: src = c->ranges.p; need = sizeof(uint32_t) * 2 * c->ntiles(); break;
        case GS_ARR_SORTED_IDS: case GS_ARR_SORTED_KEYS: {
            const size_t ni = (size_t)c->n_inst, nt = (size_t)c->ntiles();
            const size_t w = which == GS_ARR_SORTED_IDS ? sizeof(uint32_t) : sizeof(uint64_t);
            if ((size_t)bytes != w * ni) return fail(c, GS_ERR_INVALID, "gs_get_array: size mismatch");
            std::vector<uint32_t> h(ni ? ni : 1), dk(c->n1()), rg(2 * c->ntiles1());
            HIPCHK(c, hipMemcpyAsync(h.data(), c->ids.p, sizeof(uint32_t) * ni, hipMemcpyDeviceToHost, c->stream));
            HIPCHK(c, hipMemcpyAsync(dk.data(), c->depth_key.p, sizeof(uint32_t) * n, hipMemcpyDeviceToHost, c->stream));
            HIPCHK(c, hipMemcpyAsync(rg.data(), c->ranges.p, sizeof(uint32_t) * 2 * nt, hipMemcpyDeviceToHost, c->stream));
            HIPCHK(c, hipStreamSynchronize(c->stream));
            if (which == GS_ARR_SORTED_IDS) {
                std::memcpy(dst, h.data(), sizeof(uint32_t) * ni);
            } else {
                uint64_t *o = static_cast<uint64_t *>(dst);
                const bool by_index = c->order() == GS_ORDER_INDEX;
                for (size_t t = 0; t < nt; ++t)
                    for (size_t p = rg[2 * t]; p < rg[2 * t + 1] && p < ni; ++p)
                        o[p] = ((uint64_t)t << 32) | (by_index ? h[p] : dk[h[p]]);
            }
            return GS_OK;
        }
        case GS_ARR_GRAD2D: {
            if ((rc = need_stage(c, Stage::COMPOSITE_ADJOINT, "gs_get_array: gs_backward first"))) return rc;
            if ((size_t)bytes != sizeof(float) * 10 * n) return fail(c, GS_ERR_INVALID, "gs_get_array: size mismatch");
            float *o = static_cast<float *>(dst);
            const bool fixed = c->cfg.deterministic;
            std::vector<long long> fx(fixed ? GS_G2D_STRIDE * c->n1() : 0);
            std::vector<float> fl(fixed ? 0 : GS_G2D_STRIDE * c->n1());
            std::vector<GsPayload> pay(c->n1());
            std::vector<float> ic(4 * c->n1());
            if (n) HIPCHK(c, hipMemcpyAsync(fixed ? (void *)fx.data() : (void *)fl.data(), c->g2d.p, c->g2d_bytes(), hipMemcpyDeviceToHost, c->stream));
            if (n) HIPCHK(c, hipMemcpyAsync(pay.data(), c->payload.p, sizeof(GsPayload) * n, hipMemcpyDeviceToHost, c->stream));
            if (n) HIPCHK(c, hipMemcpyAsync(ic.data(), c->invcov.p, sizeof(float) * 4 * n, hipMemcpyDeviceToHost, c->stream));
            HIPCHK(c, hipStreamSynchronize(c->stream));
            for (size_t g = 0; g < n; ++g) {
                float row[10];
                gs_g2d_row_load(GsG2dRows{fl.data(), fixed ? fx.data() : nullptr}, (int64_t)g, row);
                gs_g2d_to_grads(row, pay[g].sig, ic[4 * g], 0.5f * (ic[4 * g + 1] + ic[4 * g + 2]), ic[4 * g + 3]);
                for (int i = 0; i < 10; ++i) o[10 * g + i] = row[i];
            }
            return GS_OK;
        }
        default: return fail(c, GS_ERR_INVALID, "gs_get_array: unknown array");
    }
    if ((size_t)bytes != need) return fail(c, GS_ERR_INVALID, "gs_get_array: size mismatch");
    if (need) HIPCHK(c, hipMemcpyAsync(dst, src, need, hipMemcpyDeviceToHost, c->stream));
    HIPCHK(c, hipStreamSynchronize(c->stream));
    return GS_OK;
}

int gs_get_stage_times(gs_ctx *c, float ms[GS_STAGE_COUNT]) {
    if (!c || !ms) return GS_ERR_INVALID;
    if (!c->cfg.profile_stages) return fail(c, GS_ERR_INVALID, "gs_get_stage_times: needs gs_config.profile_stages = 1");
    if (bind_device(c)) return GS_ERR_HIP;
    HIPCHK(c, hipStreamSynchronize(c->stream));
    for (int s = 0; s < GS_STAGE_COUNT; ++s) {
        ms[s] = 0.0f;
        if (c->ev_valid[s]) HIPCHK(c, hipEventElapsedTime(&ms[s], c->ev[s][0], c->ev[s][1]));
    }
    return GS_OK;
}

int gs_get_stage_stats(gs_ctx *c, double sum_ms[GS_STAGE_COUNT], int64_t count[GS_STAGE_COUNT], int reset) {
    if (!c || !sum_ms || !count) return GS_ERR_INVALID;
    if (!c->cfg.profile_stages) return fail(c, GS_ERR_INVALID, "gs_get_stage_stats: needs gs_config.profile_stages = 1");
    if (bind_device(c)) return GS_ERR_HIP;
// ... 114 lines not shown
}

int gs_rank_probe_result(const gs_ctx *c) { return c ? c->rank_probe : -1; }

static int sum_work_counters(gs_ctx *c) {
    unsigned long long *w = c->counters.as<unsigned long long>();
    const int nt = (int)c->ntiles();
    HIPCHK(c, gs_launch_sum_tiles(c->last_walked, c->tile_work.as<uint32_t>(), nt, w, c->stream));
    if (c->stage >= Stage::COMPOSITE_ADJOINT && c->tile_walked_b.p && c->tile_work_b.p)
        HIPCHK(c, gs_launch_sum_tiles(c->tile_walked_b.as<uint32_t>(), c->tile_work_b.as<uint32_t>(), nt, w + 2, c->stream));
    else HIPCHK(c, hipMemsetAsync(w + 2, 0, 16, c->stream));
    return GS_OK;
}

int gs_get_work_counters(gs_ctx *c, int64_t *walked_fwd, int64_t *walked_bwd) {
    if (!c) return GS_ERR_INVALID;
    if (const int rc = need_stage(c, Stage::RENDERED, "gs_get_work_counters: gs_forward first")) return rc;
    int64_t o[4];
    if (int rc = gs_get_work_counters_ex(c, o)) return rc;
    if (walked_fwd) *walked_fwd = o[0];
    if (walked_bwd) *walked_bwd = o[1];
    return GS_OK;
}

int gs_get_list_stats(gs_ctx *c, int64_t out[3]) {
    if (!c || !out) return GS_ERR_INVALID;
    if (const int rc = need_stage(c, Stage::RENDERED, "gs_get_list_stats: gs_forward first")) return rc;
    if (bind_device(c)) return GS_ERR_HIP;
    if (int rc = settle_totals(c, nullptr, true)) return rc;
    out[0] = c->n_inst; out[1] = 0; out[2] = 0;
    if (!c->live.frame_capped || c->bin.n_rounds != 1) return GS_OK;
    unsigned long long *d = c->counters.as<CounterBlock>()->scratch, h = 0;
    uint32_t e = 0;
    HIPCHK(c, gs_launch_sum_listed(c->tile_ext.as<uint2>(), (int)c->ntiles(), d, c->stream));
    HIPCHK(c, hipMemcpyAsync(&h, d, sizeof(h), hipMemcpyDeviceToHost, c->stream));
    HIPCHK(c, hipMemcpyAsync(&e, c->ext_count(), sizeof(e), hipMemcpyDeviceToHost, c->stream));
    HIPCHK(c, hipStreamSynchronize(c->stream));
    out[0] = (int64_t)h; out[1] = (int64_t)e; out[2] = 1;
    return GS_OK;
}

int gs_get_tile_parts(gs_ctx *c) {
    if (!c) return GS_ERR_INVALID;
    if (const int rc = need_stage(c, Stage::RENDERED, "gs_get_tile_parts: gs_forward first")) return rc;
    return c->plan.parts;
}

int gs_get_bin_path(gs_ctx *c) {
    if (!c) return GS_ERR_INVALID;
    if (const int rc = need_stage(c, Stage::BINNED, "gs_get_bin_path: gs_bin first")) return rc;
    return (int)c->bin.path;
}

int gs_get_work_counters_ex(gs_ctx *c, int64_t out[4]) {
    if (!c || !out) return GS_ERR_INVALID;
    if (const int rc = need_stage(c, Stage::RENDERED, "gs_get_work_counters_ex: gs_forward first")) return rc;
    if (bind_device(c)) return GS_ERR_HIP;
    unsigned long long h[4] = {0, 0, 0, 0};
    if (int rc = sum_work_counters(c)) return rc;
    HIPCHK(c, hipMemcpyAsync(h, c->counters.p, 32, hipMemcpyDeviceToHost, c->stream));
    HIPCHK(c, hipStreamSynchronize(c->stream));
    out[0] = (int64_t)h[0]; out[1] = (int64_t)h[2]; out[2] = (int64_t)h[1]; out[3] = (int64_t)h[3];
    return GS_OK;
}

}
```

### gaussiansplat_amd/csrc/gs_api_density.hip

```cpp
#include "gs_ctx.h"
#include "gs_density.h"


extern "C" {

int gs_density_accumulate(gs_ctx *c, const gs_density_stats *st) {
    if (!c) return GS_ERR_INVALID;
    if (!st) return fail(c, GS_ERR_INVALID, "gs_density_accumulate: NULL stats");
    if (const int rc = need_3d(c, "gs_density_accumulate")) return rc;
    if (const int rc = need_stage(c, gs_ctx::Stage::COMPOSITE_ADJOINT, "gs_density_accumulate: gs_backward first (a non-fused backward of the frame)")) return rc;
    if (c->n > 0 && (!st->grad_sum || !st->count || !st->max_extent)) return fail(c, GS_ERR_INVALID, "gs_density_accumulate: NULL statistics array");
    if (bind_device(c)) return GS_ERR_HIP;
    GsDensityAccArgs a{};
    a.n = c->n;
    a.payload = c->payload.as<GsPayload>(); a.invcov = c->invcov.as<float>();
    c->rows(c->g2d).into(a);
    a.half_w = 0.5f * (float)c->cam.W; a.half_h = 0.5f * (float)c->cam.H;
    a.grad_sum = st->grad_sum; a.count = st->count; a.max_extent = st->max_extent;
    HIPCHK(c, gs_launch_density_accumulate(a, c->stream));
    return GS_OK;
}

int gs_density_decide(gs_ctx *c, const gs_density_stats *st, const gs_density_params *p, int32_t *action) {
    if (!c) return GS_ERR_INVALID;
    if (!st || !p) return fail(c, GS_ERR_INVALID, "gs_density_decide: NULL argument");
    if (const int rc = need_3d(c, "gs_density_decide")) return rc;
    if (p->struct_size != (int32_t)sizeof(gs_density_params)) return fail(c, GS_ERR_INVALID, "gs_density_decide: gs_density_params.struct_size mismatch");
    if (std::isnan(p->grad_threshold) || std::isnan(p->log_shrink)) return fail(c, GS_ERR_INVALID, "gs_density_decide: grad_threshold and log_shrink must not be NaN");
    if (c->n > 0 && (!st->grad_sum || !st->count || !st->max_extent || !action)) return fail(c, GS_ERR_INVALID, "gs_density_decide: NULL array");
    if (bind_device(c)) return GS_ERR_HIP;
    GsDensityDecideArgs a{};
    a.n = c->n; a.scales = c->scales; a.opac = c->opac;
    a.grad_sum = st->grad_sum; a.count = st->count; a.max_extent = st->max_extent;
    a.grad_threshold = p->grad_threshold; a.log_split_scale = p->log_split_scale; a.log_shrink = p->log_shrink;
    a.min_opacity_logit = p->min_opacity_logit; a.log_max_world_scale = p->log_max_world_scale; a.max_extent_px = p->max_extent_px;
    a.action = action;
    HIPCHK(c, gs_launch_density_decide(a, c->stream));
    c->density_log_shrink = p->log_shrink;
    return GS_OK;
}

int gs_density_plan(gs_ctx *c, const int32_t *action, int64_t counts[4]) {
    if (!c) return GS_ERR_INVALID;
    if (!counts) return fail(c, GS_ERR_INVALID, "gs_density_plan: NULL counts");
    if (const int rc = need_3d(c, "gs_density_plan")) return rc;
    if (c->n > 0 && !action) return fail(c, GS_ERR_INVALID, "gs_density_plan: NULL action");
    if (bind_device(c)) return GS_ERR_HIP;
    c->density.planned = false;
// ... 42 lines not shown
    for (int t = 0; t < nsets; ++t) {
        const Five<float> ss = five(src_sets[t]), sd = five(dst_sets[t]);
        for (int i = 0; i < 5; ++i) {
            if (!ss[i] || !sd[i]) continue;
            a.set_src[t][i] = ss[i]; a.set_dst[t][i] = sd[i];
            rd[nd++] = {sd[i], sizeof(float) * c->width[i] * no};
            rs[ns++] = {ss[i], sizeof(float) * c->width[i] * n};
        }
    }
    for (int i = 0; i < nd; ++i) {
        for (int j = 0; j < ns; ++j)
            if (overlaps(rd[i], rs[j])) return fail(c, GS_ERR_INVALID, "gs_density_restructure: a destination overlaps the model or a source set");
        for (int j = i + 1; j < nd; ++j)
            if (overlaps(rd[i], rd[j])) return fail(c, GS_ERR_INVALID, "gs_density_restructure: destinations overlap");
    }
    if (bind_device(c)) return GS_ERR_HIP;
    if (!n || !no) return GS_OK;
    a.n = c->n; a.k3 = (int)c->width[4];
    a.action = action; a.noise = noise; a.chunk_off = c->density_off.as<int64_t>();
    a.survivors = d.survivors; a.clones = d.clones; a.splits = d.splits;
    a.log_shrink = c->density_log_shrink;
    a.nsets = nsets;
    HIPCHK(c, gs_launch_density_restructure(a, c->stream));
    return GS_OK;
}

int gs_opacity_reset(gs_ctx *c, float max_logit, float *m_opac, float *v_opac) {
    if (!c) return GS_ERR_INVALID;
    if (const int rc = need_3d(c, "gs_opacity_reset")) return rc;
    if (c->n > 0 && !c->opac) return fail(c, GS_ERR_INVALID, "gs_opacity_reset: no model (gs_set_model first)");
    if (bind_device(c)) return GS_ERR_HIP;
    HIPCHK(c, gs_launch_opacity_reset(const_cast<float *>(c->opac), max_logit, m_opac, v_opac, c->n, c->stream));
    c->inputs_changed();
    return GS_OK;
}

}
```

### gaussiansplat_amd/csrc/gs_api_features.hip

```cpp
#include "gs_ctx.h"
#include "gs_features.h"

using Stage = gs_ctx::Stage;

static int feature_frame_ok(gs_ctx *c, const char *who) {
    if (const int rc = need_3d(c, who)) return rc;
    if (c->stage < Stage::RENDERED) return fail(c, GS_ERR_INVALID, std::string(who) + ": gs_forward first");
    if (c->bin.n_rounds > 1)
        return fail(c, GS_ERR_UNSUPPORTED, std::string(who) + ": this frame was binned in depth slabs (lists spread over rounds); use gs_config.slab_mode = 0");
    return GS_OK;
}

static int build_feature_payload(gs_ctx *c, const float *feat) {
    HIPCHK(c, c->feat_payload.ensure(sizeof(GsPayload) * c->n1()));
    HIPCHK(c, gs_launch_feature_payload(c->payload.as<GsPayload>(), feat, c->n, c->feat_payload.as<GsPayload>(), c->stream));
    return GS_OK;
}

extern "C" {

int gs_view_depth(gs_ctx *c, float *z) {
    if (!c) return GS_ERR_INVALID;
    if (const int rc = need_3d(c, "gs_view_depth")) return rc;
    if (!z) return fail(c, GS_ERR_INVALID, "gs_view_depth: NULL argument");
    if (!c->have_cam || (c->n > 0 && !c->means)) return fail(c, GS_ERR_INVALID, "gs_view_depth: gs_set_model and gs_set_camera first");
    if (bind_device(c)) return GS_ERR_HIP;
    HIPCHK(c, gs_launch_view_depth(c->means, c->n, c->cam, z, c->stream));
    return GS_OK;
}

int gs_view_depth_backward(gs_ctx *c, const float *dz, float *d_means) {
    if (!c) return GS_ERR_INVALID;
    if (const int rc = need_3d(c, "gs_view_depth_backward")) return rc;
    if (!dz || !d_means) return fail(c, GS_ERR_INVALID, "gs_view_depth_backward: NULL argument");
    if (!c->have_cam) return fail(c, GS_ERR_INVALID, "gs_view_depth_backward: gs_set_camera first");
    if (bind_device(c)) return GS_ERR_HIP;
    HIPCHK(c, gs_launch_view_depth_bwd(dz, c->n, c->cam, d_means, c->stream));
    return GS_OK;
}

int gs_render_features(gs_ctx *c, const float *feat, float *out, float *trans_out) {
    if (!c) return GS_ERR_INVALID;
    if (const int rc = feature_frame_ok(c, "gs_render_features")) return rc;
    if (!feat || !out) return fail(c, GS_ERR_INVALID, "gs_render_features: NULL argument");
    const size_t px = c->pixels(), fb = sizeof(float);
    const ByteRange o{out, 3 * px * fb}, t{trans_out, px * fb}, image{c->img(), 3 * px * fb}, trans{c->tr(), px * fb};
    if (overlaps(o, image) || overlaps(o, trans) || overlaps(t, image) || overlaps(t, trans) || overlaps(o, t))
        return fail(c, GS_ERR_INVALID, "gs_render_features: out / trans_out overlap the frame's image or transmittance, or each other");
    if (bind_device(c)) return GS_ERR_HIP;
    if (!trans_out) HIPCHK(c, c->feat_trans.ensure(fb * (px ? px : 1)));
    if (const int rc = build_feature_payload(c, feat)) return rc;
    GsCompositeArgs a = composite_args(c, false, 0, true);
    a.payload = c->feat_payload.as<GsPayload>();
    a.image = out;
    a.trans = trans_out ? trans_out : c->feat_trans.as<float>();
    a.final_round = 1;
    HIPCHK(c, gs_launch_composite_fwd(a, c->stream));
    return GS_OK;
}

int gs_backward_features(gs_ctx *c, const float *feat, const float *image_f, const float *dF, float *d_feat, const gs_grads *grads) {
    if (!c) return GS_ERR_INVALID;
    if (const int rc = feature_frame_ok(c, "gs_backward_features")) return rc;
    if (!feat || !image_f || !dF || !d_feat) return fail(c, GS_ERR_INVALID, "gs_backward_features: NULL argument");
    if (bind_device(c)) return GS_ERR_HIP;
    HIPCHK(c, c->feat_g2d.ensure(c->g2d_bytes()));
    const bool chain = grads && (grads->d_means || grads->d_scales || grads->d_quats || grads->d_opacities);
    if (chain) {
        HIPCHK(c, c->feat_dpc.ensure(sizeof(float) * 4 * c->n1()));
        if (c->feat_dpc_zeroed != c->feat_dpc.cap) {
            HIPCHK(c, hipMemsetAsync(c->feat_dpc.p, 0, c->feat_dpc.cap, c->stream));
            c->feat_dpc_zeroed = c->feat_dpc.cap;
        }
    }
    if (const int rc = build_feature_payload(c, feat)) return rc;
    HIPCHK(c, hipMemsetAsync(c->feat_g2d.p, 0, c->g2d_bytes(), c->stream));
    GsCompositeArgs a = composite_args(c, true, 0, true);
    a.split_ok = 0; a.snap = nullptr; a.seg_hist = nullptr; a.seg_n = 0; a.seg_len = nullptr; a.snap_walked = nullptr; a.front = 0;
    a.payload = c->feat_payload.as<GsPayload>();
    a.image = const_cast<float *>(image_f);
    a.trans = c->tr();
    a.dC = dF;
    c->rows_mut(c->feat_g2d).into(a);
    HIPCHK(c, gs_launch_composite_bwd(a, c->stream));
    const gs_ctx::Rows rows = c->rows(c->feat_g2d);
    HIPCHK(c, gs_launch_pack_drgb(rows.g2d, rows.g2d_fixed, d_feat, c->n, c->stream));
    if (chain) {
        const GsPreprocessBwdArgs b = chain_args(c, rows, c->feat_dpc.as<float>(), {{grads->d_means, grads->d_scales, grads->d_quats, grads->d_opacities, nullptr}}, 0, 0, 0.0f);
        const GsPreprocessBwdMode mode{2, nullptr, 0};
        HIPCHK(c, gs_launch_preprocess_bwd(b, c->cam, c->stream, mode));
    }
// ... 5 lines not shown
```

### gaussiansplat_amd/csrc/gs_api_mcmc.hip

```cpp
#include "gs_ctx.h"
#include "gs_mcmc.h"

typedef unsigned long long u64;

extern "C" {

int gs_mcmc_plan(gs_ctx *c, float min_opacity_logit, uint64_t *cdf, int32_t *dead, int64_t counts[3]) {
    if (!c) return GS_ERR_INVALID;
    if (!counts) return fail(c, GS_ERR_INVALID, "gs_mcmc_plan: NULL counts");
    if (const int rc = need_3d(c, "gs_mcmc_plan")) return rc;
    if (std::isnan(min_opacity_logit)) return fail(c, GS_ERR_INVALID, "gs_mcmc_plan: min_opacity_logit must not be NaN");
    if (const int rc = need_model(c, "gs_mcmc_plan")) return rc;
    if (c->n > 0 && (!cdf || !dead)) return fail(c, GS_ERR_INVALID, "gs_mcmc_plan: NULL array");
    if (c->n > 0x7fffffffLL) return fail(c, GS_ERR_UNSUPPORTED, "gs_mcmc_plan: more than 2^31 - 1 gaussians");
    if (bind_device(c)) return GS_ERR_HIP;
    c->mcmc.planned = false;
    const size_t cells = 2 * (size_t)std::max<int64_t>(gs_chunks(c->n), 1);
    HIPCHK(c, c->mcmc_sum.ensure(sizeof(u64) * cells));
    HIPCHK(c, c->mcmc_off.ensure(sizeof(u64) * cells));
    HIPCHK(c, c->mcmc_tot.ensure(sizeof(u64) * 2));
    HIPCHK(c, gs_launch_mcmc_plan(c->opac, c->n, min_opacity_logit, c->mcmc_sum.as<u64>(), c->mcmc_off.as<u64>(), c->mcmc_tot.as<u64>(),
                                  reinterpret_cast<u64 *>(cdf), dead, c->stream));
    u64 tot[2] = {0, 0};
    HIPCHK(c, hipMemcpyAsync(tot, c->mcmc_tot.p, sizeof(tot), hipMemcpyDeviceToHost, c->stream));
// ... 27 lines not shown
    if (nsets > 0 && !sets) return fail(c, GS_ERR_INVALID, "gs_mcmc_relocate: NULL companion sets");
    if (m > 0 && !src) return fail(c, GS_ERR_INVALID, "gs_mcmc_relocate: NULL src");
    if (!dst) {
        const gs_ctx::McmcPlan &p = c->mcmc;
        if (!p.planned || p.n != c->n)
            return fail(c, GS_ERR_INVALID, "gs_mcmc_relocate: dst is NULL and there is no plan for this model (gs_mcmc_plan first; a model change, a step or noise drop it)");
        if (m > p.dead_count) return fail(c, GS_ERR_INVALID, "gs_mcmc_relocate: m exceeds the plan's dead count");
        dst = p.dead;
    }
    if (const int rc = need_model(c, "gs_mcmc_relocate")) return rc;
    if (bind_device(c)) return GS_ERR_HIP;
    if (m == 0 || c->n == 0) return GS_OK;
    if (!c->mcmc_binom_ready) {
        static double table[GS_MCMC_BINOM];
        gs_mcmc_binom_fill(table);
        HIPCHK(c, c->mcmc_binom.ensure(sizeof(table)));
        HIPCHK(c, hipMemcpyAsync(c->mcmc_binom.p, table, sizeof(table), hipMemcpyHostToDevice, c->stream));
        c->mcmc_binom_ready = true;
    }
    HIPCHK(c, c->mcmc_hist.ensure(sizeof(int32_t) * c->n1()));
    GsMcmcRelocateArgs a{};
    a.n = c->n; a.m = m; a.k3 = (int)c->width[4];
    a.src = src; a.dst = dst; a.hist = c->mcmc_hist.as<int32_t>(); a.binom = c->mcmc_binom.as<double>();
    a.min_opacity = min_opacity;
    const Five<float> model = c->model5_mut();
    for (int i = 0; i < 5; ++i) a.model[i] = model[i];
    a.nsets = nsets;
    for (int t = 0; t < nsets; ++t) {
        const Five<float> s = five(sets[t]);
        for (int i = 0; i < 5; ++i) a.set[t][i] = s[i];
    }
    HIPCHK(c, gs_launch_mcmc_relocate(a, c->stream));
    c->inputs_changed();
    return GS_OK;
}

int gs_mcmc_noise(gs_ctx *c, const float *z, float lr, float gate_k, float gate_t) {
    if (!c) return GS_ERR_INVALID;
    if (const int rc = need_3d(c, "gs_mcmc_noise")) return rc;
    if (!std::isfinite(lr) || !std::isfinite(gate_k) || !std::isfinite(gate_t)) return fail(c, GS_ERR_INVALID, "gs_mcmc_noise: lr, gate_k and gate_t must be finite");
    if (lr < 0.0f) return fail(c, GS_ERR_INVALID, "gs_mcmc_noise: lr must be >= 0");
    if (lr == 0.0f) return GS_OK;
    if (const int rc = need_model(c, "gs_mcmc_noise")) return rc;
    if (c->n > 0 && !z) return fail(c, GS_ERR_INVALID, "gs_mcmc_noise: NULL z");
    const size_t n = (size_t)c->n;
    const Five<const float> model = c->model5();
    for (int i = 0; i < 5; ++i)
        if (overlaps({z, sizeof(float) * 3 * n}, {model[i], sizeof(float) * c->width[i] * n})) return fail(c, GS_ERR_INVALID, "gs_mcmc_noise: z overlaps the model");
    if (bind_device(c)) return GS_ERR_HIP;
    if (c->n == 0) return GS_OK;
    HIPCHK(c, gs_launch_mcmc_noise(const_cast<float *>(c->means), c->scales, c->quats, c->opac, z, c->n, lr, gate_k, gate_t, c->stream));
    c->inputs_changed();
    return GS_OK;
}

int gs_mcmc_regularize(gs_ctx *c, const gs_grads *grads, float c_opacity, float c_scale) {
    if (!c) return GS_ERR_INVALID;
    if (!grads) return fail(c, GS_ERR_INVALID, "gs_mcmc_regularize: NULL grads");
    if (const int rc = need_3d(c, "gs_mcmc_regularize")) return rc;
    if (!std::isfinite(c_opacity) || !std::isfinite(c_scale)) return fail(c, GS_ERR_INVALID, "gs_mcmc_regularize: the coefficients must be finite");
    if (const int rc = need_model(c, "gs_mcmc_regularize")) return rc;
    float *d_opac = c_opacity != 0.0f ? grads->d_opacities : nullptr;
    float *d_scales = c_scale != 0.0f ? grads->d_scales : nullptr;
    const size_t n = (size_t)c->n;
    const Five<const float> model = c->model5();
    for (int i = 0; i < 5; ++i)
        if (overlaps({d_opac, sizeof(float) * n}, {model[i], sizeof(float) * c->width[i] * n}) ||
            overlaps({d_scales, sizeof(float) * 3 * n}, {model[i], sizeof(float) * c->width[i] * n}))
            return fail(c, GS_ERR_INVALID, "gs_mcmc_regularize: a gradient array overlaps the model");
    if (bind_device(c)) return GS_ERR_HIP;
    HIPCHK(c, gs_launch_mcmc_regularize(c->scales, c->opac, d_scales, d_opac, c->n, c_opacity, c_scale, c->stream));
    return GS_OK;
}

}
```

### gaussiansplat_amd/csrc/gs_ctx.h

```cpp
#pragma once
#include "../../include/gsplat.h"
#include "gs_common.h"

#include <rccl/rccl.h>

#include <algorithm>
#include <cassert>
#include <cmath>
#include <cstddef>
#include <cstdio>
#include <cstdlib>
#include <cstring>
#include <new>
#include <string>
#include <vector>

struct DevBuf {
    void *p = nullptr;
    size_t cap = 0;
    DevBuf() = default;
    DevBuf(DevBuf &&o) noexcept : p(o.p), cap(o.cap) { o.p = nullptr; o.cap = 0; }
    ~DevBuf() { if (p) (void)hipFree(p); }
    hipError_t ensure(size_t bytes) {
        if (bytes <= cap) return hipSuccess;
        if (p) { hipError_t e = hipFree(p); p = nullptr; cap = 0; if (e != hipSuccess) return e; }
        size_t want = bytes + bytes / 8 + 256;
        hipError_t e = hipMalloc(&p, want);
        if (e == hipSuccess) cap = want;
        return e;
    }
    template <typename T> T *as() const { return static_cast<T *>(p); }
};
template <typename T> struct Five { T *p[5]; T *operator[](int i) const { return p[i]; } };
inline Five<float> five(const gs_grads &g) { return {{g.d_means, g.d_scales, g.d_quats, g.d_opacities, g.d_shs}}; }

extern std::string g_create_error;

#define GS_COUNTER_BYTES 192
struct CounterBlock {
    uint32_t work[8];
    uint32_t pad0[24];
    uint32_t totals[4];
    uint32_t ext_count;
    uint32_t pad1[3];
    unsigned long long scratch[4];
};
struct PinnedWords {
    uint32_t readback[2];
    uint32_t walked_prev[2];
    uint32_t pad0[4];
    CounterBlock counters;
    uint32_t pad1[44];
    uint32_t dsort_stat[2];
    uint32_t pad2[26];
};
static_assert(sizeof(CounterBlock) == GS_COUNTER_BYTES && offsetof(CounterBlock, totals) == 128 && offsetof(CounterBlock, ext_count) == 144 &&
              offsetof(CounterBlock, scratch) == 160, "counter block layout (the kernels address it by these offsets)");
static_assert(sizeof(PinnedWords) == 512 && offsetof(PinnedWords, readback) == 0 && offsetof(PinnedWords, walked_prev) == 8 &&
              offsetof(PinnedWords, counters) == 32 && offsetof(PinnedWords, dsort_stat) == 400, "pinned block layout");
void comm_release(struct gs_ctx *c);
struct gs_ctx {
    ~gs_ctx() {
        comm_release(this);
        for (auto &pair : ev) for (hipEvent_t e : pair) if (e) (void)hipEventDestroy(e);
        for (hipEvent_t e : {ev_count, ev_main, ev_order}) if (e) (void)hipEventDestroy(e);
        if (side) (void)hipStreamDestroy(side);
        for (void *h : {(void *)pinned, (void *)pinned_split}) if (h) (void)hipHostFree(h);
        if (own_stream && stream) (void)hipStreamDestroy(stream);
    }
    int device = 0;
    hipStream_t stream = nullptr;
    bool own_stream = false, borrowed_stream = false;
    gs_config cfg{};
    std::string err;

    int64_t n = 0;
    int sh_degree = 0;
    int sh_active_request = -1;
    int active_sh_degree() const { return sh_active_request < 0 || sh_active_request > sh_degree ? sh_degree : sh_active_request; }
    int sh_row_floats() const { return 3 * (sh_degree + 1) * (sh_degree + 1); }
    float background[3] = {0.0f, 0.0f, 0.0f};
    bool has_background() const { return background[0] != 0.0f || background[1] != 0.0f || background[2] != 0.0f; }
    int kind = 0;
    size_t width[5] = {3, 3, 4, 1, 3};
    int order() const { return kind == 1 ? (int)GS_ORDER_INDEX : cfg.order; }
    const float *means = nullptr, *scales = nullptr, *quats = nullptr, *opac = nullptr, *shs = nullptr;
    DevBuf model[5];
    Five<const float> model5() const { return {{means, scales, quats, opac, shs}}; }
    Five<float> model5_mut() const { return {{const_cast<float *>(means), const_cast<float *>(scales), const_cast<float *>(quats), const_cast<float *>(opac), const_cast<float *>(shs)}}; }
    void set_model5(const float *const a[5]) { means = a[0]; scales = a[1]; quats = a[2]; opac = a[3]; shs = a[4]; }
    GsCamera cam{};
    bool have_cam = false;
    enum class Stage {
        NOTHING,
        PREPROCESSED,
        BINNED,
        RENDERED,
        COMPOSITE_ADJOINT,
        BACKWARD
    } stage = Stage::NOTHING;
    void reach(Stage s) { stage = s; }
    void fall_back(Stage s) { if (stage > s) stage = s; }
    void inputs_changed() { fall_back(Stage::NOTHING); density.planned = false; mcmc.planned = false; }
    int gx = 0, gy = 0;
    int64_t grid_key() const { return ((int64_t)gx << 32) | (int64_t)gy; }
    int64_t ntiles() const { return (int64_t)gx * gy; }
    size_t ntiles1() const { const size_t nt = (size_t)ntiles(); return nt ? nt : 1; }
    size_t n1() const { return n ? (size_t)n : 1; }
    size_t pixels() const { return (size_t)cam.W * cam.H; }

    DevBuf invcov;
    DevBuf payload, depth_key, rect, pairs_a, pairs_b, perm, offsets, block_sums;
    DevBuf inst_a, inst_b, table, digit_total, ranges, image, trans, g2d, stage_in;
    enum Dbg { DBG_TS, DBG_TPS, DBG_MU, DBG_COV3D, DBG_COV2D, DBG_INVCOV, DBG_BBS, DBG_COUNT };
    static constexpr size_t DBG_WIDTH[DBG_COUNT] = {4, 4, 2, 9, 4, 4, 4};
    DevBuf dbg[DBG_COUNT];
    DevBuf ids, words, cs, diff;
    int64_t n_inst = 0;
    PinnedWords *pinned = nullptr;
    const float *last_dC = nullptr;

    hipEvent_t ev_count = nullptr;
    hipEvent_t ev[GS_STAGE_COUNT][2] = {};
    bool ev_valid[GS_STAGE_COUNT] = {};
    bool ev_fresh[GS_STAGE_COUNT] = {};
    double ev_sum[GS_STAGE_COUNT] = {};
    int64_t ev_cnt[GS_STAGE_COUNT] = {};
    DevBuf counters;
    DevBuf tile_work, tile_clock;
    int view_slot = -1;
    struct ViewSlot {
        DevBuf order[2];
        int sel = 0;
        int64_t tiles = 0;
        int order_dst(bool in_use) const { return in_use ? sel ^ 1 : sel; }
        void order_written(int buf, int64_t grid) { sel = buf; tiles = grid; }
        DevBuf walkbuf[2];
        int wsel = 0;
        int64_t walked_grid = 0;
        DevBuf &walked() { return walkbuf[wsel]; }
        DevBuf &walk_dst() { return walkbuf[wsel ^ 1]; }
        void walk_written(int64_t grid) { wsel ^= 1; walked_grid = grid; }
    };
    std::vector<ViewSlot> slots;
    const uint32_t *last_walked = nullptr;
    int wave_slots = 5120;
    DevBuf tile_nopen, smax, tile_ext, zero_tiles;
    struct FrameLive {
        bool frame_capped = false;
        const uint32_t *cap_src = nullptr;
        bool have_l2 = false;
        GsBin3Args last_l2{};
        bool spec_lists = false;
        size_t spec_cap_coarse = 0, spec_cap_fine = 0;
        bool g2d_clean = false;
        uint32_t *perm_ptr = nullptr;
        void speculate(size_t cap_coarse, size_t cap_fine) { spec_lists = true; spec_cap_coarse = cap_coarse; spec_cap_fine = cap_fine; }
        bool speculation_held(size_t coarse, size_t fine) { spec_lists = false; return coarse <= spec_cap_coarse && fine <= spec_cap_fine; }
        void relist_in_full() { cap_src = nullptr; frame_capped = false; have_l2 = false; }
        void rows_dirtied() { g2d_clean = false; }
    } live;
    struct BinPlan {
        enum class Path { TWO_LEVEL = 0, RADIX64 = 1, RADIX32 = 2, SMALL = 3 } path = Path::RADIX64;
        int tile_bits = 0, gid_bits = 0, lo_bits = 0, hi_bits = 0;
        int sbs = 3, sgx = 0, sgy = 0;
        int n_rounds = 1;
        int64_t slab_lo[GS_MAX_ROUNDS + 1] = {};
        bool perm_on_demand = false;
        int ns() const { return sgx * sgy; }
        bool radix() const { return path == Path::RADIX32 || path == Path::RADIX64; }
    } bin;
    struct FramePlan {
        int parts = 1;
        int bwd_parts = 1;
        const uint32_t *order = nullptr;
        const uint32_t *bwd_order = nullptr;
        bool side = false;
        int front = 0;
        bool split = false;
        enum class Snap { NONE, HEAVY, ALL } snap = Snap::NONE;
        uint32_t *snap_walked = nullptr;
        int seg_n = 0;
        const uint32_t *seg_hist = nullptr;
        bool bwd_segments = false;
    } plan;
    struct BackwardPlan {
        bool composite = true;
        int chain = 3;
        enum class Update { ACCUMULATE, OVERWRITE, SGD, ADAM_DENSE, ADAM_SELECTIVE } update = Update::ACCUMULATE;
        float lr = 0.0f; const GsAdamFused *adam = nullptr;
        bool fused() const { return update >= Update::SGD; }
        Five<float> target{};
        const float *dC = nullptr; bool stage_dC = false;
        bool host_sync = false;
        bool fill_g2d = false;
        bool fill_shs = false;
        bool model_changes() const { return fused(); }
    };
    DevBuf snap, snap_walked;
    uint32_t *pinned_split = nullptr;
    uint32_t *split_word(int slot, int buf) { return pinned_split ? pinned_split + 2 * slot + buf : nullptr; }
    int snap_parity = 0;
    hipStream_t side = nullptr;
    hipEvent_t ev_main = nullptr, ev_order = nullptr;
    bool order_pending = false;
    bool pending_totals = false;
    int64_t n_coarse = 0;
    DevBuf tile_dead;
    int dbg_win_start = 0, dbg_win_len = 0;
    int rank_probe = -1;
    int64_t round_gen[GS_MAX_ROUNDS] = {};
    size_t round_ids_off[GS_MAX_ROUNDS] = {};
    DevBuf ranges_r[GS_MAX_ROUNDS];
    DevBuf tile_pos, tile_done, live2d, rect_r, offsets_r, live_total;
    DevBuf rect_sorted, l1_table, l1_rows, l1_partials, cids, clr, cranges, segcnt, sdone, tilecnt;
    uint32_t *bin_totals() { return counters.as<CounterBlock>()->totals; }
    uint32_t *ext_count() { return &counters.as<CounterBlock>()->ext_count; }
    DevBuf tile_walked, tile_walked_b, tile_work_b;
    hipError_t ensure_bwd_counters() { const hipError_t e = tile_walked_b.ensure(sizeof(uint32_t) * ntiles1()); return e != hipSuccess ? e : tile_work_b.ensure(sizeof(uint32_t) * ntiles1()); }
    int64_t counters_grid = 0;
    bool counters_here() const { return counters_grid == grid_key() && last_walked; }
    DevBuf key_range;
    int range_parity = 0;
    bool range_valid = false;
    bool dsort_buckets_used = false;
    int64_t dsort_classic_until = 0;
    int dsort_stat_parity = 0;
    uint32_t *dsort_stat() { return &pinned->dsort_stat[dsort_stat_parity & 1]; }
    bool dsort_can_bucket() const {
        return cfg.depth_sort != 1 && (cfg.depth_sort == 2 || (n <= gs_depth_buckets_max_n() && frame_id > dsort_classic_until));
    }
    bool small_bin_possible() const {
        if (cfg.bin_path != 0 || cfg.depth_sort != 0 || cfg.list_cap == 2 || cfg.slab_fractions[0] > 0.0f) return false;
        if (cfg.debug_flags & (GS_DEBUG_WIDE_CURSORS | GS_DEBUG_SUPER8 | GS_DEBUG_SUPER16 | GS_DEBUG_TINY_CAPS)) return false;
        return gs_bin_small_supported(n, gx, gy);
    }
    template <typename F, typename L> struct RowsOf {
        F *g2d; L *g2d_fixed;
// ... 71 lines not shown
}
inline int need_stage(gs_ctx *c, gs_ctx::Stage s, const char *msg) { return c->stage >= s ? GS_OK : fail(c, GS_ERR_INVALID, msg); }
struct ByteRange { const void *p; size_t bytes; };
inline bool overlaps(const ByteRange &a, const ByteRange &b) {
    const uintptr_t x = reinterpret_cast<uintptr_t>(a.p), y = reinterpret_cast<uintptr_t>(b.p);
    return a.p && b.p && a.bytes && b.bytes && x < y + b.bytes && y < x + a.bytes;
}

template <typename A> auto model_head_stride(A &a, int stride, int) -> decltype((void)a.sh_stride) { a.sh_stride = stride; }
template <typename A> void model_head_stride(A &, int, long) {}
template <typename A> void model_head(const gs_ctx *c, A &a) {
    a.n = c->n; a.sh_degree = c->active_sh_degree(); model_head_stride(a, c->sh_row_floats(), 0);
    a.means = c->means; a.scales = c->scales; a.quats = c->quats; a.opac = c->opac; a.shs = c->shs;
}
inline GsPreprocessBwdArgs chain_args(const gs_ctx *c, gs_ctx::Rows rows, float *dpc, const Five<float> &target, int overwrite, int shs_zeroed, float sgd_scale) {
    GsPreprocessBwdArgs b{};
    model_head(c, b); rows.into(b);
    b.dpc = dpc; b.overwrite = overwrite; b.shs_zeroed = shs_zeroed; b.sgd_scale = sgd_scale;
    b.d_means = target[0]; b.d_scales = target[1]; b.d_quats = target[2]; b.d_opac = target[3]; b.d_shs = target[4];
    return b;
}

inline bool harvest_stage(gs_ctx *c, int s) {
    if (!c->ev_fresh[s]) return true;
    float ms = 0.0f;
    if (hipEventElapsedTime(&ms, c->ev[s][0], c->ev[s][1]) != hipSuccess) { (void)hipGetLastError(); return false; }
    c->ev_sum[s] += ms;
    if (c->ev_counted[s] != c->ev_frame[s]) { c->ev_counted[s] = c->ev_frame[s]; c->ev_cnt[s] += 1; }
    c->ev_fresh[s] = false;
    return true;
}
struct StageTimer {
    gs_ctx *c; int st; bool on;
    StageTimer(gs_ctx *c_, int st_) : c(c_), st(st_), on(c_->cfg.profile_stages == 1 || c_->cfg.profile_stages == 2 + st_) {
        if (on) {
            if (c->ev_fresh[st] && !harvest_stage(c, st)) {
                (void)hipEventSynchronize(c->ev[st][1]);
                (void)harvest_stage(c, st);
            }
            c->ev_frame[st] = c->frame_id;
            (void)hipEventRecord(c->ev[st][0], c->stream);
        }
    }
    ~StageTimer() {
        if (on) { (void)hipEventRecord(c->ev[st][1], c->stream); c->ev_valid[st] = true; c->ev_fresh[st] = true; }
    }
};

inline void harvest_events(gs_ctx *c, int skip_stage = -1) {
    if (!c->cfg.profile_stages) return;
    for (int s = 0; s < GS_STAGE_COUNT; ++s)
        if (s != skip_stage) (void)harvest_stage(c, s);
}

inline int bind_device(gs_ctx *c) {
    HIPCHK(c, hipSetDevice(c->device));
    return GS_OK;
}

inline bool lpt_schedule(const gs_ctx *c) {
    return (c->cfg.schedule == 3 || c->cfg.schedule == 4) && (c->ntiles() > c->wave_slots || (c->cfg.debug_flags & GS_DEBUG_ALWAYS_ORDER));
}
inline int lpt_front(const gs_ctx *c) {
    const int64_t ntiles = c->ntiles();
    return (lpt_schedule(c) && c->cfg.tile_parts == 0 && c->cfg.t_min > 0.0f && 2 * ntiles > c->wave_slots && ntiles <= GS_LPT_MAX_TILES) ? GS_LPT_FRONT : 0;
}
inline const uint32_t *order_seg_len(const gs_ctx *c, const uint32_t *order) { return order + lpt_front(c) + gs_lpt_order_len(c->gx, c->gy); }
inline int lpt_order_entries(const gs_ctx *c) { return lpt_front(c) + gs_lpt_order_len(c->gx, c->gy); }
inline int lpt_split_div(const gs_ctx *c) { return c->wave_slots * 4 / 5; }
inline bool use_side_stream(const gs_ctx *c) { return c->n >= 262144 || (c->cfg.debug_flags & GS_DEBUG_ALWAYS_ORDER); }
inline uint32_t *key_range_of(const gs_ctx *c, int parity) { return c->key_range.as<uint32_t>() + (size_t)parity * gs_depth_range_parity_words(); }
inline int order_index(const gs_ctx *c) { return c->view_slot >= 0 ? c->view_slot : GS_MAX_VIEW_SLOTS; }

int settle_totals(gs_ctx *c, bool *redo, bool may_relist);
int bin_round(gs_ctx *c, int r);
int depth_order(gs_ctx *c);
int blend_background(gs_ctx *c);
GsCompositeArgs composite_args(gs_ctx *c, bool bwd, int r, bool debug = false);
```

### include/gsplat.h

```cpp
#ifndef GSPLAT_H
#define GSPLAT_H

#include <stdint.h>

#ifdef __cplusplus
extern "C" {
#endif

#define GS_ABI_VERSION 3

typedef enum {
    GS_OK = 0,
    GS_ERR_INVALID = -1,
    GS_ERR_NO_DEVICE = -2,
    GS_ERR_HIP = -3,
    GS_ERR_OOM = -4,
    GS_ERR_UNSUPPORTED = -5
} gs_status;

typedef enum { GS_MEM_HOST = 0, GS_MEM_DEVICE = 1 } gs_mem;

typedef enum { GS_ORDER_INDEX = 0, GS_ORDER_DEPTH_DESC = 1, GS_ORDER_DEPTH_ASC = 2 } gs_order;

typedef struct {
    int32_t struct_size;
    int32_t abi_version;
    int32_t tile_size;
    int32_t order;
    float   t_min;
    int32_t deterministic;
    int32_t export_debug;
    int32_t profile_stages;
    int32_t bin_path;
    int32_t rank_mode;
    int32_t alpha_cull;
    int32_t schedule;
    int32_t slab_mode;
    float   slab_max_ratio;
    float   slab_fractions[3];
    int32_t debug_flags;
    int32_t depth_sort;
    int32_t list_cap;
    int32_t tile_parts;
    int32_t reserved[3];
} gs_config;
#define GS_DEBUG_WIDE_CURSORS 1
#define GS_DEBUG_ALWAYS_ORDER 2
#define GS_DEBUG_SUPER16 8
#define GS_DEBUG_SUPER8 16
#define GS_DEBUG_TINY_CAPS 4
#define GS_DEBUG_NO_TAIL_FILL 32

typedef struct gs_ctx gs_ctx;

void gs_default_config(gs_config *cfg);

int gs_abi_version(void);

int gs_create(gs_ctx **out, int device, const gs_config *cfg);
int gs_destroy(gs_ctx *ctx);
const char *gs_last_error(const gs_ctx *ctx);

#define GS_STREAM_LEGACY ((void *)1)
int gs_set_stream(gs_ctx *ctx, void *hip_stream);
int gs_synchronize(gs_ctx *ctx);

int gs_set_model(gs_ctx *ctx, int64_t n, int sh_degree,
                 const float *means, const float *scales, const float *quats,
                 const float *opacities, const float *shs, int mem);

int gs_set_model_2d(gs_ctx *ctx, int64_t n, const float *means, const float *scales, const float *rotations,
                    const float *opacities, const float *colors, int mem);

int gs_set_active_sh_degree(gs_ctx *ctx, int degree);
int gs_get_active_sh_degree(const gs_ctx *ctx);

int gs_set_background(gs_ctx *ctx, const float rgb[3]);
int gs_get_background(const gs_ctx *ctx, float rgb[3]);
int gs_compose_target(gs_ctx *ctx, const float *rgba, int32_t W, int32_t H, float *rgb_out);

int gs_set_image_size(gs_ctx *ctx, int32_t W, int32_t H);

int gs_set_camera(gs_ctx *ctx, const float T[16], const float P[16], float fx, float fy,
                  float near_, float far_, const float eye[3], const float lookAt[3],
// ... 143 lines not shown
    GS_ARR_BBS = 6,
    GS_ARR_RGB = 7,
    GS_ARR_SIG = 8,
    GS_ARR_DEPTH_KEY = 9,
    GS_ARR_TILE_RECT = 10,
    GS_ARR_SORT_IDXS = 11,
    GS_ARR_TILE_RANGES = 12,
    GS_ARR_SORTED_IDS = 13,
    GS_ARR_SORTED_KEYS = 14,
    GS_ARR_GRAD2D = 15
} gs_array;

int64_t gs_num_gaussians(const gs_ctx *ctx);
int64_t gs_num_instances(gs_ctx *ctx);
int64_t gs_num_coarse_instances(gs_ctx *ctx);
int gs_num_rounds(const gs_ctx *ctx);

int gs_get_array(gs_ctx *ctx, int which, void *host_dst, int64_t bytes);

typedef enum {
    GS_STAGE_PREPROCESS = 0, GS_STAGE_DEPTH_SORT, GS_STAGE_COUNT_SCAN, GS_STAGE_EMIT,
    GS_STAGE_TILE_SORT, GS_STAGE_RANGES, GS_STAGE_COMPOSITE_FWD, GS_STAGE_COMPOSITE_BWD,
    GS_STAGE_PREPROCESS_BWD, GS_STAGE_COUNT
} gs_stage;

int gs_get_stage_times(gs_ctx *ctx, float ms[GS_STAGE_COUNT]);

int gs_get_stage_stats(gs_ctx *ctx, double sum_ms[GS_STAGE_COUNT], int64_t count[GS_STAGE_COUNT], int reset);

int gs_get_work_counters(gs_ctx *ctx, int64_t *walked_fwd, int64_t *walked_bwd);

int gs_get_list_stats(gs_ctx *ctx, int64_t out[3]);

int gs_get_tile_parts(gs_ctx *ctx);

int gs_get_bin_path(gs_ctx *ctx);

int gs_get_work_counters_ex(gs_ctx *ctx, int64_t out[4]);

int gs_debug_time_composite(gs_ctx *ctx, int which, int variant, int reps, float *mean_ms);

int gs_debug_tile_clock(gs_ctx *ctx, int which, int variant, uint64_t *out);
int gs_debug_tile_clock_rows(gs_ctx *ctx);
int gs_debug_tail_fill(gs_ctx *ctx, int32_t blocks[2]);

int gs_debug_clock_mhz(gs_ctx *ctx, float *mhz);

int gs_debug_set_window(gs_ctx *ctx, int32_t start, int32_t len);

int gs_rank_probe_result(const gs_ctx *ctx);

#ifdef __cplusplus
}
#endif
#endif
```

Measured before the change: 834.2 Msplats/s.

## Overlap next frame's preprocess and binning with previous backward on a front stream

Adds a 'front' stream and double-buffers the per-frame payload, invcov, ranges, ids and tile_ext buffers by parity. When the model has not been written since the last forward, the single-round two-level binning path runs the next frame's preprocess and binning on the front stream while the previous frame's backward runs on the main stream. Events join the two streams before compositing. Model-writing calls such as Adam, SGD and MCMC now mark the model dirty and record an event, which disables overlap for that frame. The aim is to hide the front-half stages behind backward compute, at the cost of extra memory and more complex event bookkeeping.

```diff
diff --git a/gaussiansplat_amd/backend.py b/gaussiansplat_amd/backend.py
--- a/gaussiansplat_amd/backend.py
+++ b/gaussiansplat_amd/backend.py
@@ -29,6 +29,7 @@
 GS_DEBUG_SUPER8 = 16
 GS_DEBUG_NO_TAIL_FILL = 32
 GS_DEBUG_TINY_CAPS = 4
+GS_DEBUG_SERIAL_FRAMES = 64
 GS_MAX_VIEW_SLOTS = 4096
 GS_BWD_OVERWRITE, GS_BWD_COMPOSITE_ONLY, GS_BWD_PARAMS_ONLY, GS_BWD_PARAMS_SH, GS_BWD_PARAMS_GEOM = 1, 2, 4, 8, 16
 GS_ADAM_GROUPS = 6
@@ -142,6 +143,7 @@
     "gs_get_stage_stats": Sig(_i, [_vp, _dp, _i64p, _i]),
     "gs_get_work_counters": Sig(_i, [_vp, _i64p, _i64p]),
     "gs_get_list_stats": Sig(_i, [_vp, _i64p]),
+    "gs_get_overlapped_frames": Sig(_i, [_vp, _i64p]),
     "gs_get_tile_parts": Sig(_i, [_vp]),
     "gs_get_bin_path": Sig(_i, [_vp]),
     "gs_get_work_counters_ex": Sig(_i, [_vp, _i64p]),
@@ -596,6 +598,11 @@
         self._chk(self.L.gs_get_list_stats(self.h, o))
         return dict(listed=int(o[0]), extended_segments=int(o[1]), capped=bool(o[2]))
 
+    def overlapped_frames(self) -> int:
+        o = C.c_int64()
+        self._chk(self.L.gs_get_overlapped_frames(self.h, C.byref(o)))
+        return int(o.value)
+
     def tile_parts_of_frame(self) -> int:
         rc = self.L.gs_get_tile_parts(self.h)
         if rc < 0:
diff --git a/gaussiansplat_amd/csrc/gs_adam.hip b/gaussiansplat_amd/csrc/gs_adam.hip
--- a/gaussiansplat_amd/csrc/gs_adam.hip
+++ b/gaussiansplat_amd/csrc/gs_adam.hip
@@ -212,5 +212,5 @@
         HIPCHK(c, hipGetLastError());
     }
     c->inputs_changed();
-    return GS_OK;
-}
+    return model_written(c);
+}
diff --git a/gaussiansplat_amd/csrc/gs_api.hip b/gaussiansplat_amd/csrc/gs_api.hip
--- a/gaussiansplat_amd/csrc/gs_api.hip
+++ b/gaussiansplat_amd/csrc/gs_api.hip
@@ -1,10 +1,42 @@
 #include "gs_ctx.h"
 
 std::string g_create_error;
+
+#include <atomic>
+#include <mutex>
+static std::mutex g_ctx_mu;
+static std::vector<gs_ctx *> g_ctxs;
+static std::atomic<int> g_ctx_count{0};
+static void register_ctx(gs_ctx *c) { std::lock_guard<std::mutex> lock(g_ctx_mu); g_ctxs.push_back(c); g_ctx_count = (int)g_ctxs.size(); }
+static void unregister_ctx(gs_ctx *c) {
+    std::lock_guard<std::mutex> lock(g_ctx_mu);
+    g_ctxs.erase(std::remove(g_ctxs.begin(), g_ctxs.end(), c), g_ctxs.end());
+    g_ctx_count = (int)g_ctxs.size();
+}
+int model_written(gs_ctx *c) {
+    c->fr.model_written();
+    if (g_ctx_count.load(std::memory_order_relaxed) < 2) return GS_OK;
+    std::lock_guard<std::mutex> lock(g_ctx_mu);
+    HIPCHK(c, hipEventRecord(c->ev_model, c->stream));
+    c->model_ev_set = true;
+    return GS_OK;
+}
+int wait_model_final(gs_ctx *c, hipStream_t s) {
+    std::lock_guard<std::mutex> lock(g_ctx_mu);
+    for (gs_ctx *o : g_ctxs)
+        if (o->device == c->device && o->model_ev_set) HIPCHK(c, hipStreamWaitEvent(s, o->ev_model, 0));
+    return GS_OK;
+}
+int frame_read(gs_ctx *c) {
+    if (!c->front || !use_side_stream(c)) return GS_OK;
+    HIPCHK(c, hipEventRecord(c->ev_fwd, c->stream));
+    c->fr.mark();
+    return GS_OK;
+}
 
 template <typename A> static int preprocess_outputs(gs_ctx *c, A &a) {
     a.gx = c->gx; a.gy = c->gy;
-    a.payload = c->payload.as<GsPayload>(); a.invcov = c->invcov.as<float>(); a.depth_key = c->depth_key.as<uint32_t>(); a.rect = c->rect.as<uint16_t>();
+    a.payload = c->payload().as<GsPayload>(); a.invcov = c->invcov().as<float>(); a.depth_key = c->depth_key.as<uint32_t>(); a.rect = c->rect.as<uint16_t>();
     if (!c->cfg.export_debug) return GS_OK;
     for (int i = 0; i < gs_ctx::DBG_COUNT; ++i) HIPCHK(c, c->dbg[i].ensure(sizeof(float) * gs_ctx::DBG_WIDTH[i] * c->n1()));
     auto arr = [c](gs_ctx::Dbg i) { return c->dbg[i].as<float>(); };
@@ -56,7 +88,7 @@
     if (!(c0.slab_max_ratio >= 0.0f && c0.slab_max_ratio <= 1.0f)) return fail(nullptr, GS_ERR_INVALID, "gs_create: slab_max_ratio must be in [0, 1]");
     for (int i = 0; i < 3; ++i)
         if (!(c0.slab_fractions[i] >= 0.0f && c0.slab_fractions[i] < 1.0f)) return fail(nullptr, GS_ERR_INVALID, "gs_create: slab_fractions must be in [0, 1)");
-    if (c0.debug_flags & ~(GS_DEBUG_WIDE_CURSORS | GS_DEBUG_ALWAYS_ORDER | GS_DEBUG_TINY_CAPS | GS_DEBUG_SUPER16 | GS_DEBUG_SUPER8 | GS_DEBUG_NO_TAIL_FILL)) return fail(nullptr, GS_ERR_INVALID, "gs_create: unknown debug_flags");
+    if (c0.debug_flags & ~(GS_DEBUG_WIDE_CURSORS | GS_DEBUG_ALWAYS_ORDER | GS_DEBUG_TINY_CAPS | GS_DEBUG_SUPER16 | GS_DEBUG_SUPER8 | GS_DEBUG_NO_TAIL_FILL | GS_DEBUG_SERIAL_FRAMES)) return fail(nullptr, GS_ERR_INVALID, "gs_create: unknown debug_flags");
     if (c0.depth_sort < 0 || c0.depth_sort > 2) return fail(nullptr, GS_ERR_INVALID, "gs_create: depth_sort must be 0, 1 or 2");
     if (c0.list_cap < 0 || c0.list_cap > 2) return fail(nullptr, GS_ERR_INVALID, "gs_create: list_cap must be 0, 1 or 2");
     if (c0.tile_parts != 0 && c0.tile_parts != 1 && c0.tile_parts != 2 && c0.tile_parts != 4) return fail(nullptr, GS_ERR_INVALID, "gs_create: tile_parts must be 0, 1, 2 or 4");
@@ -86,7 +118,8 @@
         for (hipEvent_t &ev : pair) if ((e = hipEventCreate(&ev)) != hipSuccess) { delete c; return hipfail(nullptr, e, "hipEventCreate"); }
     if ((e = hipEventCreateWithFlags(&c->ev_count, hipEventDisableTiming | hipEventReleaseToSystem)) != hipSuccess) { delete c; return hipfail(nullptr, e, "hipEventCreate"); }
     if ((e = hipStreamCreateWithFlags(&c->side, hipStreamNonBlocking)) != hipSuccess) { delete c; return hipfail(nullptr, e, "hipStreamCreate"); }
-    for (hipEvent_t *ev : {&c->ev_main, &c->ev_order})
+    if ((e = hipStreamCreateWithFlags(&c->front, hipStreamNonBlocking)) != hipSuccess) { delete c; return hipfail(nullptr, e, "hipStreamCreate"); }
+    for (hipEvent_t *ev : {&c->ev_main, &c->ev_order, &c->ev_front, &c->ev_fwd, &c->ev_model})
         if ((e = hipEventCreateWithFlags(ev, hipEventDisableTiming)) != hipSuccess) { delete c; return hipfail(nullptr, e, "hipEventCreate"); }
     if (c->cfg.rank_mode == 0) {
         int bad = 0;
@@ -94,6 +127,7 @@
         c->rank_probe = bad ? 1 : 0;
         if (bad) c->cfg.rank_mode = 1;
     }
+    register_ctx(c);
     *out = c;
     return GS_OK;
 }
@@ -103,6 +137,8 @@
     (void)hipSetDevice(c->device);
     (void)hipStreamSynchronize(c->stream);
     if (c->side) (void)hipStreamSynchronize(c->side);
+    if (c->front) (void)hipStreamSynchronize(c->front);
+    unregister_ctx(c);
     delete c;
     return GS_OK;
 }
@@ -114,6 +150,8 @@
     if (bind_device(c)) return GS_ERR_HIP;
     HIPCHK(c, hipStreamSynchronize(c->stream));
     if (c->side) HIPCHK(c, hipStreamSynchronize(c->side));
+    if (c->front) HIPCHK(c, hipStreamSynchronize(c->front));
+    c->fr.stream_changed();
     if (c->own_stream && c->stream) { (void)hipStreamDestroy(c->stream); c->own_stream = false; }
     if (hip_stream) { c->stream = want; c->borrowed_stream = true; }
     else { HIPCHK(c, hipStreamCreateWithFlags(&c->stream, hipStreamNonBlocking)); c->own_stream = true; c->borrowed_stream = false; }
@@ -125,6 +163,7 @@
     if (bind_device(c)) return GS_ERR_HIP;
     HIPCHK(c, hipStreamSynchronize(c->stream));
     if (c->side) HIPCHK(c, hipStreamSynchronize(c->side));
+    if (c->front) HIPCHK(c, hipStreamSynchronize(c->front));
     return GS_OK;
 }
 
@@ -144,7 +183,7 @@
     for (int i = 0; i < 5; ++i) c->width[i] = width[i];
     c->set_model5(dst);
     c->inputs_changed();
-    return GS_OK;
+    return model_written(c);
 }
 
 int gs_set_model(gs_ctx *c, int64_t n, int sh_degree, const float *means, const float *scales, const float *quats,
@@ -175,8 +214,9 @@
     if (degree < -1 || degree > 3) return fail(c, GS_ERR_INVALID, "gs_set_active_sh_degree: degree must be -1 (the model's own) or 0..3");
     const int before = c->active_sh_degree();
     c->sh_active_request = degree;
-    if (c->active_sh_degree() != before) c->inputs_changed();
-    return GS_OK;
+    if (c->active_sh_degree() == before) return GS_OK;
+    c->inputs_changed();
+    return bind_device(c) ? GS_ERR_HIP : model_written(c);
 }
 
 int gs_get_active_sh_degree(const gs_ctx *c) {
@@ -193,7 +233,7 @@
     if (rgb[0] == c->background[0] && rgb[1] == c->background[1] && rgb[2] == c->background[2]) return GS_OK;
     for (int i = 0; i < 3; ++i) c->background[i] = rgb[i];
     c->fall_back(gs_ctx::Stage::BINNED);
-    return GS_OK;
+    return bind_device(c) ? GS_ERR_HIP : model_written(c);
 }
 
 int gs_get_background(const gs_ctx *c, float rgb[3]) {
@@ -241,18 +281,11 @@
     return GS_OK;
 }
 
-int gs_preprocess(gs_ctx *c) {
-    if (!c) return GS_ERR_INVALID;
-    if (!c->have_cam) return fail(c, GS_ERR_INVALID, "gs_preprocess: gs_set_camera first");
-    if (bind_device(c)) return GS_ERR_HIP;
-    if (int rc = settle_totals(c, nullptr, false)) return rc;
-    c->frame_id += 1;
-    HIPCHK(c, c->payload.ensure(sizeof(GsPayload) * c->n1()));
-    HIPCHK(c, c->invcov.ensure(sizeof(float) * 4 * c->n1()));
+static int preprocess_frame(gs_ctx *c) {
+    HIPCHK(c, c->payload().ensure(sizeof(GsPayload) * c->n1()));
+    HIPCHK(c, c->invcov().ensure(sizeof(float) * 4 * c->n1()));
     HIPCHK(c, c->depth_key.ensure(sizeof(uint32_t) * c->n1()));
     HIPCHK(c, c->rect.ensure(sizeof(uint16_t) * 4 * c->n1()));
-    c->gx = (c->cam.W + GS_TILE - 1) / GS_TILE;
-    c->gy = (c->cam.H + GS_TILE - 1) / GS_TILE;
     c->range_valid = false;
     GsPreprocessArgs a{};
     GsPreprocess2DArgs a2{};
@@ -266,7 +299,7 @@
         if (c->dsort_can_bucket() && c->order() != GS_ORDER_INDEX && c->n > 0 && !c->small_bin_possible()) {
             if (!c->key_range.p) {
                 HIPCHK(c, c->key_range.ensure(sizeof(uint32_t) * gs_depth_range_words()));
-                HIPCHK(c, gs_depth_range_reset(c->key_range.as<uint32_t>(), c->stream));
+                HIPCHK(c, gs_depth_range_reset(c->key_range.as<uint32_t>(), c->fs()));
             }
             c->range_parity ^= 1;
             a.key_range = key_range_of(c, c->range_parity);
@@ -274,10 +307,26 @@
         }
         if (int rc = preprocess_outputs(c, a)) return rc;
     }
-    StageTimer t(c, GS_STAGE_PREPROCESS);
-    HIPCHK(c, c->kind == 1 ? gs_launch_preprocess2d(a2, c->stream) : gs_launch_preprocess(a, c->cam, c->sh_row_floats(), c->stream));
+    {
+        StageTimer t(c, GS_STAGE_PREPROCESS);
+        HIPCHK(c, c->kind == 1 ? gs_launch_preprocess2d(a2, c->fs()) : gs_launch_preprocess(a, c->cam, c->sh_row_floats(), c->fs()));
+    }
     c->reach(gs_ctx::Stage::PREPROCESSED);
     return GS_OK;
+}
+
+int gs_preprocess(gs_ctx *c) {
+    if (!c) return GS_ERR_INVALID;
+    if (!c->have_cam) return fail(c, GS_ERR_INVALID, "gs_preprocess: gs_set_camera first");
+    if (bind_device(c)) return GS_ERR_HIP;
+    if (int rc = settle_totals(c, nullptr, false)) return rc;
+    c->frame_id += 1;
+    c->gx = (c->cam.W + GS_TILE - 1) / GS_TILE;
+    c->gy = (c->cam.H + GS_TILE - 1) / GS_TILE;
+    int rc = begin_frame(c);
+    if (!rc) rc = preprocess_frame(c);
+    const int rj = join_front(c, rc != GS_OK);
+    return rc ? rc : rj;
 }
 
 int gs_loss_l1_dssim(gs_ctx *c, const float *img, const float *gt, int32_t W, int32_t H, int32_t C, float lam, float *dC,
@@ -327,7 +376,7 @@
     const Five<float> p = c->model5_mut(), gr = five(*g);
     for (int i = 0; i < 5; ++i) HIPCHK(c, gs_launch_sgd(p[i], gr[i], lr, c->width[i] * n, c->stream));
     c->inputs_changed();
-    return GS_OK;
+    return model_written(c);
 }
 
 int gs_reset_grads(gs_ctx *c, const gs_grads *g) {
diff --git a/gaussiansplat_amd/csrc/gs_api_bin.hip b/gaussiansplat_amd/csrc/gs_api_bin.hip
--- a/gaussiansplat_amd/csrc/gs_api_bin.hip
+++ b/gaussiansplat_amd/csrc/gs_api_bin.hip
@@ -29,7 +29,7 @@
     p.n_rounds = r;
 }
 
-static void plan_bin(gs_ctx *c) {
+static gs_ctx::BinPlan bin_plan_of(const gs_ctx *c) {
     gs_ctx::BinPlan p{};
     const int64_t ntiles = c->ntiles();
     p.tile_bits = 1;
@@ -46,7 +46,27 @@
     p.path = c->small_bin_possible() ? Path::SMALL : fast && asked == 0 && gs_bin3_supported(p.ns()) ? Path::TWO_LEVEL : fast ? Path::RADIX32 : Path::RADIX64;
     p.perm_on_demand = p.path == Path::SMALL && c->order() != GS_ORDER_INDEX;
     plan_rounds(c, p);
-    c->bin = p;
+    return p;
+}
+static void plan_bin(gs_ctx *c) { c->bin = bin_plan_of(c); }
+
+static bool frame_overlaps(gs_ctx *c) {
+    const gs_ctx::BinPlan p = bin_plan_of(c);
+    const GsFrontInputs in{c->front != nullptr, use_side_stream(c), c->ev_model != nullptr, (c->cfg.debug_flags & GS_DEBUG_SERIAL_FRAMES) != 0,
+                           c->cfg.profile_stages, p.path == Path::TWO_LEVEL, p.n_rounds};
+    return c->fr.begin(in);
+}
+int begin_frame(gs_ctx *c) {
+    if (!frame_overlaps(c)) return GS_OK;
+    if (int rc = wait_model_final(c, c->front)) return rc;
+    HIPCHK(c, hipStreamWaitEvent(c->front, c->ev_fwd, 0));
+    return GS_OK;
+}
+int join_front(gs_ctx *c, bool close) {
+    if (!(close ? c->fr.close() : c->fr.open)) return GS_OK;
+    HIPCHK(c, hipEventRecord(c->ev_front, c->front));
+    HIPCHK(c, hipStreamWaitEvent(c->stream, c->ev_front, 0));
+    return GS_OK;
 }
 
 static GsBin3L1 two_level_args(gs_ctx *c, const uint32_t *perm_slab, int64_t n_all, int64_t nr, const uint8_t *sdone, size_t cap_coarse, size_t cap_fine) {
@@ -74,7 +94,7 @@
         if (!c->counters_here()) c->prev_counters_valid = false;
         b.tile_walked = c->prev_counters_valid ? c->last_walked : nullptr; b.n_tile_walked = (int)c->ntiles();
     }
-    HIPCHK(c, gs_bin3_l1_count(b, c->stream));
+    HIPCHK(c, gs_bin3_l1_count(b, c->fs()));
     return GS_OK;
 }
 static int two_level_lists(gs_ctx *c, const uint32_t *perm_slab, int64_t n_all, int64_t nr, size_t coarse, size_t fine, uint32_t *ranges, uint32_t *ids_out,
@@ -84,14 +104,14 @@
     assert(done || (!live.frame_capped && !live.have_l2));
     if (!done) live.cap_src = cap_src;
     if (coarse == 0) {
-        HIPCHK(c, hipMemsetAsync(ranges, 0, sizeof(uint32_t) * 2 * c->ntiles(), c->stream));
+        HIPCHK(c, hipMemsetAsync(ranges, 0, sizeof(uint32_t) * 2 * c->ntiles(), c->fs()));
         return GS_OK;
     }
     const int64_t max_work = gs_bin3_max_work((int64_t)coarse, ns);
     HIPCHK(c, c->cids.ensure(sizeof(uint32_t) * coarse));
     HIPCHK(c, c->clr.ensure(sizeof(uint16_t) * coarse));
     HIPCHK(c, c->segcnt.ensure(sizeof(uint32_t) * ((size_t)1 << (2 * c->bin.sbs)) * (size_t)max_work));
-    HIPCHK(c, gs_bin3_l1_scatter(two_level_args(c, perm_slab, n_all, nr, sdone, coarse, fine), c->stream));
+    HIPCHK(c, gs_bin3_l1_scatter(two_level_args(c, perm_slab, n_all, nr, sdone, coarse, fine), c->fs()));
     GsBin3Args a{};
     a.cranges = c->cranges.as<uint32_t>(); a.cids = c->cids.as<uint32_t>(); a.clr = c->clr.as<uint16_t>(); a.ranges = ranges; a.tilecnt = c->tilecnt.as<uint32_t>();
     a.done = done; a.segcnt = c->segcnt.as<uint32_t>(); a.ids_out = ids_out;
@@ -102,12 +122,12 @@
         const size_t nt = (size_t)c->ntiles();
         HIPCHK(c, c->tile_nopen.ensure(sizeof(uint32_t) * nt));
         HIPCHK(c, c->smax.ensure(sizeof(uint32_t) * (size_t)ns));
-        HIPCHK(c, c->tile_ext.ensure(sizeof(uint2) * nt));
-        a.cap_src = cap_src; a.tile_nopen = c->tile_nopen.as<uint32_t>(); a.smax = c->smax.as<uint32_t>(); a.tile_ext = c->tile_ext.as<uint2>();
+        HIPCHK(c, c->tile_ext().ensure(sizeof(uint2) * nt));
+        a.cap_src = cap_src; a.tile_nopen = c->tile_nopen.as<uint32_t>(); a.smax = c->smax.as<uint32_t>(); a.tile_ext = c->tile_ext().as<uint2>();
         a.ext_count = c->ext_count();
         live.frame_capped = true;
     }
-    HIPCHK(c, gs_bin3_build_lists(a, c->stream));
+    HIPCHK(c, gs_bin3_build_lists(a, c->fs()));
     if (!done) { live.last_l2 = a; live.have_l2 = true; }
     return GS_OK;
 }
@@ -120,7 +140,7 @@
     if (c->cfg.debug_flags & GS_DEBUG_TINY_CAPS) {
         if (c->zero_tiles.cap < sizeof(uint32_t) * (size_t)ntiles) {
             HIPCHK(c, c->zero_tiles.ensure(sizeof(uint32_t) * (size_t)ntiles));
-            HIPCHK(c, hipMemsetAsync(c->zero_tiles.p, 0, c->zero_tiles.cap, c->stream));
+            HIPCHK(c, hipMemsetAsync(c->zero_tiles.p, 0, c->zero_tiles.cap, c->fs()));
         }
         *out = c->zero_tiles.as<uint32_t>();
         return GS_OK;
@@ -140,7 +160,7 @@
     b.offsets = (r ? c->offsets_r : c->offsets).as<uint32_t>(); b.perm = c->live.perm_ptr ? c->live.perm_ptr + p.slab_lo[r] : nullptr;
     b.rect = (r ? c->rect_r : c->rect).as<uint16_t>();
     b.cs = c->cs.as<uint32_t>(); b.block_hist = c->table.as<uint32_t>(); b.digit_total = c->digit_total.as<uint32_t>();
-    b.buf_a = c->words.as<uint32_t>(); b.ids_out = c->ids.as<uint32_t>() + c->round_ids_off[r]; b.ballot_ranks = c->cfg.rank_mode != 0;
+    b.buf_a = c->words.as<uint32_t>(); b.ids_out = c->ids().as<uint32_t>() + c->round_ids_off[r]; b.ballot_ranks = c->cfg.rank_mode != 0;
     if (r) { b.done = c->tile_done.as<uint8_t>(); b.live_total = c->live_total.as<uint32_t>() + r; }
     return b;
 }
@@ -153,11 +173,11 @@
     HIPCHK(c, c->sdone.ensure((size_t)p.ns()));
     {
         StageTimer t(c, GS_STAGE_COUNT_SCAN);
-        HIPCHK(c, gs_launch_super_done(c->tile_done.as<uint8_t>(), c->gx, c->gy, p.sgx, p.sgy, p.sbs, c->sdone.as<uint8_t>(), c->stream));
+        HIPCHK(c, gs_launch_super_done(c->tile_done.as<uint8_t>(), c->gx, c->gy, p.sgx, p.sgy, p.sbs, c->sdone.as<uint8_t>(), c->fs()));
         if (int rc = two_level_count(c, perm, nr, nr, c->sdone.as<uint8_t>())) return rc;
     }
-    HIPCHK(c, hipMemcpyAsync(c->pinned->readback, c->bin_totals(), 2 * sizeof(uint32_t), hipMemcpyDeviceToHost, c->stream));
-    HIPCHK(c, hipEventRecord(c->ev_count, c->stream));
+    HIPCHK(c, hipMemcpyAsync(c->pinned->readback, c->bin_totals(), 2 * sizeof(uint32_t), hipMemcpyDeviceToHost, c->fs()));
+    HIPCHK(c, hipEventRecord(c->ev_count, c->fs()));
     HIPCHK(c, hipEventSynchronize(c->ev_count));
     harvest_events(c);
     const int64_t coarse = (int64_t)c->pinned->readback[0];
@@ -166,7 +186,7 @@
     if (c->round_ids_off[r] + (size_t)c->round_gen[r] > (size_t)c->n_inst) return fail(c, GS_ERR_HIP, "gs_forward: slab instance accounting out of range");
     {
         StageTimer t(c, GS_STAGE_TILE_SORT);
-        if (int rc = two_level_lists(c, perm, nr, nr, (size_t)coarse, (size_t)c->round_gen[r], c->ranges_r[r].as<uint32_t>(), c->ids.as<uint32_t>() + c->round_ids_off[r],
+        if (int rc = two_level_lists(c, perm, nr, nr, (size_t)coarse, (size_t)c->round_gen[r], c->ranges_r[r].as<uint32_t>(), c->ids().as<uint32_t>() + c->round_ids_off[r],
                                      c->tile_done.as<uint8_t>(), c->sdone.as<uint8_t>())) return rc;
     }
     return GS_OK;
@@ -184,16 +204,16 @@
     {
         StageTimer t(c, GS_STAGE_COUNT_SCAN);
         HIPCHK(c, gs_launch_live_prefix(c->tile_done.as<uint8_t>(), c->gx, c->gy, c->live2d.as<uint32_t>(),
-                                        c->live2d.as<uint32_t>() + (size_t)(c->gx + 1) * (c->gy + 1), c->stream));
+                                        c->live2d.as<uint32_t>() + (size_t)(c->gx + 1) * (c->gy + 1), c->fs()));
         HIPCHK(c, gs_launch_count_scan_live(c->rect.as<uint16_t>(), perm, c->live2d.as<uint32_t>(), c->gx, c->rect_r.as<uint16_t>(),
-                                            c->offsets_r.as<uint32_t>(), c->block_sums.as<uint32_t>(), nr, c->stream));
-    }
-    HIPCHK(c, hipMemcpyAsync(c->pinned->readback, c->offsets_r.as<uint32_t>() + nr, sizeof(uint32_t), hipMemcpyDeviceToHost, c->stream));
-    HIPCHK(c, hipEventRecord(c->ev_count, c->stream));
+                                            c->offsets_r.as<uint32_t>(), c->block_sums.as<uint32_t>(), nr, c->fs()));
+    }
+    HIPCHK(c, hipMemcpyAsync(c->pinned->readback, c->offsets_r.as<uint32_t>() + nr, sizeof(uint32_t), hipMemcpyDeviceToHost, c->fs()));
+    HIPCHK(c, hipEventRecord(c->ev_count, c->fs()));
     {
         StageTimer t(c, GS_STAGE_RANGES);
         HIPCHK(c, gs_launch_tile_ranges(c->rect_r.as<uint16_t>(), perm, nr, c->diff.as<int>(), c->gx, c->gy, c->ranges_r[r].as<uint32_t>(),
-                                        c->tile_done.as<uint8_t>(), c->stream));
+                                        c->tile_done.as<uint8_t>(), c->fs()));
     }
     HIPCHK(c, hipEventSynchronize(c->ev_count));
     harvest_events(c, GS_STAGE_RANGES);
@@ -203,7 +223,7 @@
     if (c->round_ids_off[r] + (size_t)c->round_gen[r] > (size_t)c->n_inst) return fail(c, GS_ERR_HIP, "gs_forward: slab instance accounting out of range");
     {
         StageTimer t(c, GS_STAGE_TILE_SORT);
-        HIPCHK(c, gs_bin2_build_lists(bin2_args(c, r), c->stream));
+        HIPCHK(c, gs_bin2_build_lists(bin2_args(c, r), c->fs()));
     }
     return GS_OK;
 }
@@ -242,11 +262,11 @@
     if (int rc = totals_arrived(c, coarse, fine_slab, h.totals[2], h.work)) return rc;
     if (!c->live.spec_lists || c->live.speculation_held(coarse, fine_slab)) return GS_OK;
     if (!may_relist) { c->fall_back(gs_ctx::Stage::PREPROCESSED); return GS_OK; }
-    HIPCHK(c, c->ids.ensure(sizeof(uint32_t) * (size_t)(c->n_inst ? c->n_inst : 1)));
+    HIPCHK(c, c->ids().ensure(sizeof(uint32_t) * (size_t)(c->n_inst ? c->n_inst : 1)));
     c->live.relist_in_full();
     {
         StageTimer t(c, GS_STAGE_TILE_SORT);
-        if (int rc = two_level_lists(c, c->live.perm_ptr, c->n, c->bin.slab_lo[1], (size_t)coarse, (size_t)fine_slab, c->ranges.as<uint32_t>(), c->ids.as<uint32_t>(), nullptr, nullptr,
+        if (int rc = two_level_lists(c, c->live.perm_ptr, c->n, c->bin.slab_lo[1], (size_t)coarse, (size_t)fine_slab, c->ranges().as<uint32_t>(), c->ids().as<uint32_t>(), nullptr, nullptr,
                                      nullptr)) return rc;
     }
     if (redo) *redo = true;
@@ -266,16 +286,16 @@
     const bool buckets = c->range_valid && c->dsort_can_bucket();
     c->dsort_buckets_used = buckets;
     if (c->range_valid && !buckets)
-        HIPCHK(c, gs_depth_range_reset(key_range_of(c, c->range_parity), c->stream, 1));
+        HIPCHK(c, gs_depth_range_reset(key_range_of(c, c->range_parity), c->fs(), 1));
     if (buckets) {
         uint32_t *range = key_range_of(c, c->range_parity), *other = key_range_of(c, c->range_parity ^ 1);
         c->dsort_stat_parity = c->range_parity;
         *c->dsort_stat() = 0u;
         HIPCHK(c, gs_depth_sort_buckets(c->depth_key.as<uint32_t>(), c->pairs_a.as<uint64_t>(), c->pairs_b.as<uint64_t>(), c->n, c->table.as<uint32_t>(),
-                                        c->digit_total.as<uint32_t>(), perm, range, other, c->dsort_stat(), c->stream, c->cfg.rank_mode != 0));
+                                        c->digit_total.as<uint32_t>(), perm, range, other, c->dsort_stat(), c->fs(), c->cfg.rank_mode != 0));
     } else {
         HIPCHK(c, gs_radix_sort_u64(c->pairs_a.as<uint64_t>(), c->pairs_b.as<uint64_t>(), c->n, 32, 64, c->table.as<uint32_t>(),
-                                    c->digit_total.as<uint32_t>(), &in_b, c->stream, c->cfg.rank_mode != 0, perm, c->depth_key.as<uint32_t>()));
+                                    c->digit_total.as<uint32_t>(), &in_b, c->fs(), c->cfg.rank_mode != 0, perm, c->depth_key.as<uint32_t>()));
     }
     c->live.perm_ptr = perm;
     return GS_OK;
@@ -283,13 +303,13 @@
 
 static int bin_small(gs_ctx *c) {
     const size_t n = (size_t)c->n, nt = (size_t)c->ntiles();
-    HIPCHK(c, c->ids.ensure(sizeof(uint32_t) * n * nt));
+    HIPCHK(c, c->ids().ensure(sizeof(uint32_t) * n * nt));
     if (c->range_valid)
-        HIPCHK(c, gs_depth_range_reset(key_range_of(c, c->range_parity), c->stream, 1));
+        HIPCHK(c, gs_depth_range_reset(key_range_of(c, c->range_parity), c->fs(), 1));
     GsBinSmallArgs a{};
     a.depth_key = c->order() != GS_ORDER_INDEX ? c->depth_key.as<uint32_t>() : nullptr; a.rect = c->rect.as<uint2>();
     a.n = (int)c->n; a.gx = c->gx; a.gy = c->gy; a.ntiles = (int)nt;
-    a.ranges = c->ranges.as<uint32_t>(); a.ids = c->ids.as<uint32_t>(); a.totals = c->bin_totals();
+    a.ranges = c->ranges().as<uint32_t>(); a.ids = c->ids().as<uint32_t>(); a.totals = c->bin_totals();
     a.host_totals = c->pinned->counters.totals; a.host_walked = c->pinned->counters.work; a.walked_src = c->counters.as<uint32_t>();
     if (!c->counters_here()) c->prev_counters_valid = false;
     a.tile_walked = c->prev_counters_valid ? c->last_walked : nullptr; a.n_tile_walked = (int)nt;
@@ -299,10 +319,10 @@
     }
     {
         StageTimer t(c, GS_STAGE_TILE_SORT);
-        HIPCHK(c, gs_bin_small(a, c->stream));
+        HIPCHK(c, gs_bin_small(a, c->fs()));
     }
     c->live.g2d_clean = true;
-    HIPCHK(c, hipEventRecord(c->ev_count, c->stream));
+    HIPCHK(c, hipEventRecord(c->ev_count, c->fs()));
     c->pending_totals = true;
     return GS_OK;
 }
@@ -314,21 +334,21 @@
         StageTimer t(c, GS_STAGE_COUNT_SCAN);
         if (int rc = two_level_count(c, perm, c->n, n0, nullptr, c->n > 0)) return rc;
     }
-    if (c->n <= 0) HIPCHK(c, hipMemcpyAsync(&c->pinned->counters, c->counters.p, GS_COUNTER_BYTES, hipMemcpyDeviceToHost, c->stream));
-    HIPCHK(c, hipEventRecord(c->ev_count, c->stream));
+    if (c->n <= 0) HIPCHK(c, hipMemcpyAsync(&c->pinned->counters, c->counters.p, GS_COUNTER_BYTES, hipMemcpyDeviceToHost, c->fs()));
+    HIPCHK(c, hipEventRecord(c->ev_count, c->fs()));
     c->pending_totals = true;
-    const size_t cap_coarse = std::min(c->cids.cap / sizeof(uint32_t), c->clr.cap / sizeof(uint16_t)), cap_fine = c->ids.cap / sizeof(uint32_t);
+    const size_t cap_coarse = std::min(c->cids.cap / sizeof(uint32_t), c->clr.cap / sizeof(uint16_t)), cap_fine = c->ids().cap / sizeof(uint32_t);
     const uint32_t *cap_src = nullptr;
     if (int rc = list_cap_source(c, &cap_src)) return rc;
     if (c->bin.n_rounds == 1 && cap_coarse > 0 && cap_fine > 0) {
         c->live.speculate(cap_coarse, cap_fine);
         StageTimer t(c, GS_STAGE_TILE_SORT);
-        return two_level_lists(c, perm, c->n, n0, cap_coarse, cap_fine, c->ranges.as<uint32_t>(), c->ids.as<uint32_t>(), nullptr, nullptr, cap_src);
+        return two_level_lists(c, perm, c->n, n0, cap_coarse, cap_fine, c->ranges().as<uint32_t>(), c->ids().as<uint32_t>(), nullptr, nullptr, cap_src);
     }
     if (int rc = settle_totals(c, nullptr, true)) return rc;
-    HIPCHK(c, c->ids.ensure(sizeof(uint32_t) * (size_t)(c->n_inst ? c->n_inst : 1)));
+    HIPCHK(c, c->ids().ensure(sizeof(uint32_t) * (size_t)(c->n_inst ? c->n_inst : 1)));
     StageTimer t(c, GS_STAGE_TILE_SORT);
-    return two_level_lists(c, perm, c->n, n0, (size_t)c->n_coarse, (size_t)c->round_gen[0], c->ranges.as<uint32_t>(), c->ids.as<uint32_t>(), nullptr, nullptr, cap_src);
+    return two_level_lists(c, perm, c->n, n0, (size_t)c->n_coarse, (size_t)c->round_gen[0], c->ranges().as<uint32_t>(), c->ids().as<uint32_t>(), nullptr, nullptr, cap_src);
 }
 
 static int radix64_lists(gs_ctx *c) {
@@ -337,19 +357,19 @@
     HIPCHK(c, c->inst_b.ensure(sizeof(uint64_t) * ni1));
     {
         StageTimer t(c, GS_STAGE_EMIT);
-        HIPCHK(c, gs_launch_emit(c->rect.as<uint16_t>(), c->live.perm_ptr, c->offsets.as<uint32_t>(), c->inst_a.as<uint64_t>(), c->n, c->gx, c->stream));
+        HIPCHK(c, gs_launch_emit(c->rect.as<uint16_t>(), c->live.perm_ptr, c->offsets.as<uint32_t>(), c->inst_a.as<uint64_t>(), c->n, c->gx, c->fs()));
     }
     uint64_t *sorted = nullptr;
     {
         StageTimer t(c, GS_STAGE_TILE_SORT);
         int in_b = 0;
         HIPCHK(c, gs_radix_sort_u64(c->inst_a.as<uint64_t>(), c->inst_b.as<uint64_t>(), c->n_inst, 32, 32 + c->bin.tile_bits,
-                                    c->table.as<uint32_t>(), c->digit_total.as<uint32_t>(), &in_b, c->stream, c->cfg.rank_mode != 0));
+                                    c->table.as<uint32_t>(), c->digit_total.as<uint32_t>(), &in_b, c->fs(), c->cfg.rank_mode != 0));
         sorted = in_b ? c->inst_b.as<uint64_t>() : c->inst_a.as<uint64_t>();
     }
     StageTimer t(c, GS_STAGE_RANGES);
-    HIPCHK(c, gs_launch_ranges(sorted, c->n_inst, c->ranges.as<uint32_t>(), c->ntiles(), c->stream));
-    HIPCHK(c, gs_launch_split_ids(sorted, c->ids.as<uint32_t>(), c->n_inst, c->stream));
+    HIPCHK(c, gs_launch_ranges(sorted, c->n_inst, c->ranges().as<uint32_t>(), c->ntiles(), c->fs()));
+    HIPCHK(c, gs_launch_split_ids(sorted, c->ids().as<uint32_t>(), c->n_inst, c->fs()));
     return GS_OK;
 }
 
@@ -362,21 +382,21 @@
     {
         StageTimer t(c, GS_STAGE_COUNT_SCAN);
         HIPCHK(c, c->offsets.ensure(sizeof(uint32_t) * (n + 1)));
-        HIPCHK(c, gs_launch_count_scan(c->rect.as<uint16_t>(), perm, c->offsets.as<uint32_t>(), c->block_sums.as<uint32_t>(), c->n, c->stream));
-    }
-    HIPCHK(c, hipMemcpyAsync(&h->readback[0], c->offsets.as<uint32_t>() + n, sizeof(uint32_t), hipMemcpyDeviceToHost, c->stream));
-    HIPCHK(c, hipMemcpyAsync(&h->readback[1], c->offsets.as<uint32_t>() + n0, sizeof(uint32_t), hipMemcpyDeviceToHost, c->stream));
+        HIPCHK(c, gs_launch_count_scan(c->rect.as<uint16_t>(), perm, c->offsets.as<uint32_t>(), c->block_sums.as<uint32_t>(), c->n, c->fs()));
+    }
+    HIPCHK(c, hipMemcpyAsync(&h->readback[0], c->offsets.as<uint32_t>() + n, sizeof(uint32_t), hipMemcpyDeviceToHost, c->fs()));
+    HIPCHK(c, hipMemcpyAsync(&h->readback[1], c->offsets.as<uint32_t>() + n0, sizeof(uint32_t), hipMemcpyDeviceToHost, c->fs()));
     if (!c->counters_here()) c->prev_counters_valid = false;
     if (c->prev_counters_valid) {
-        HIPCHK(c, gs_launch_sum_tiles(c->last_walked, c->tile_work.as<uint32_t>(), (int)c->ntiles(), c->counters.as<unsigned long long>(), c->stream));
-        HIPCHK(c, hipMemcpyAsync(h->walked_prev, c->counters.p, sizeof(uint64_t), hipMemcpyDeviceToHost, c->stream));
-    }
-    HIPCHK(c, hipEventRecord(c->ev_count, c->stream));
+        HIPCHK(c, gs_launch_sum_tiles(c->last_walked, c->tile_work.as<uint32_t>(), (int)c->ntiles(), c->counters.as<unsigned long long>(), c->fs()));
+        HIPCHK(c, hipMemcpyAsync(h->walked_prev, c->counters.p, sizeof(uint64_t), hipMemcpyDeviceToHost, c->fs()));
+    }
+    HIPCHK(c, hipEventRecord(c->ev_count, c->fs()));
     if (fast) {
         HIPCHK(c, c->diff.ensure(sizeof(int) * gs_tile_ranges_scratch_ints(c->gx, c->gy)));
         StageTimer t(c, GS_STAGE_RANGES);
         HIPCHK(c, gs_launch_tile_ranges(c->rect.as<uint16_t>(), slabs ? perm : nullptr, slabs ? n0 : c->n, c->diff.as<int>(), c->gx, c->gy,
-                                        c->ranges.as<uint32_t>(), nullptr, c->stream));
+                                        c->ranges().as<uint32_t>(), nullptr, c->fs()));
     }
     HIPCHK(c, hipEventSynchronize(c->ev_count));
     harvest_events(c, fast ? GS_STAGE_RANGES : -1);
@@ -385,20 +405,20 @@
     const size_t ni1 = c->n_inst ? (size_t)c->n_inst : 1;
     HIPCHK(c, c->table.ensure(sizeof(uint32_t) * gs_sort_table_entries(c->n_inst > c->n ? c->n_inst : c->n)));
     HIPCHK(c, c->digit_total.ensure(sizeof(uint32_t) * 4 * 256));
-    HIPCHK(c, c->ids.ensure(sizeof(uint32_t) * ni1));
+    HIPCHK(c, c->ids().ensure(sizeof(uint32_t) * ni1));
     if (!fast) return radix64_lists(c);
     const size_t nchunks = ((size_t)c->n_inst + 4095) / 4096;
     HIPCHK(c, c->cs.ensure(sizeof(uint32_t) * (nchunks + 2)));
     if (c->bin.hi_bits > 0) HIPCHK(c, c->words.ensure(sizeof(uint32_t) * ni1));
     StageTimer t(c, GS_STAGE_TILE_SORT);
-    HIPCHK(c, gs_bin2_build_lists(bin2_args(c, 0), c->stream));
+    HIPCHK(c, gs_bin2_build_lists(bin2_args(c, 0), c->fs()));
     return GS_OK;
 }
 
 static int bin_frame(gs_ctx *c) {
     const Path path = c->bin.path;
     if (c->order() != GS_ORDER_INDEX && path != Path::SMALL) { if (int rc = depth_order(c)) return rc; }
-    HIPCHK(c, c->ranges.ensure(sizeof(uint32_t) * 2 * c->ntiles1()));
+    HIPCHK(c, c->ranges().ensure(sizeof(uint32_t) * 2 * c->ntiles1()));
     HIPCHK(c, c->counters.ensure(GS_COUNTER_BYTES));
     if (path != Path::SMALL) HIPCHK(c, c->block_sums.ensure(sizeof(uint32_t) * 3 * ((size_t)c->n / 2048 + 2)));
     if (int rc = path == Path::SMALL ? bin_small(c) : path == Path::TWO_LEVEL ? bin_two_level(c) : bin_radix(c)) return rc;
@@ -415,5 +435,8 @@
     if (int rc = settle_totals(c, nullptr, false)) return rc;
     c->live = gs_ctx::FrameLive{};
     plan_bin(c);
-    return bin_frame(c);
-}
+    if (c->fr.plan_disagrees(c->bin.path == Path::TWO_LEVEL, c->bin.n_rounds)) { if (int rc = join_front(c, true)) return rc; }
+    c->fr.binning_on_main();
+    const int rc = bin_frame(c), rj = join_front(c, true);
+    return rc ? rc : rj;
+}
diff --git a/gaussiansplat_amd/csrc/gs_api_composite.hip b/gaussiansplat_amd/csrc/gs_api_composite.hip
--- a/gaussiansplat_amd/csrc/gs_api_composite.hip
+++ b/gaussiansplat_amd/csrc/gs_api_composite.hip
@@ -50,24 +50,24 @@
     const gs_ctx::FramePlan &p = c->plan;
     GsCompositeArgs a{};
     a.W = c->cam.W; a.H = c->cam.H; a.gx = c->gx; a.gy = c->gy; a.t_min = c->cfg.t_min;
-    a.payload = c->payload.as<GsPayload>(); a.image = c->img(); a.trans = c->tr();
+    a.payload = c->payload().as<GsPayload>(); a.image = c->img(); a.trans = c->tr();
     a.cull = c->cfg.alpha_cull != 0;
     for (int q = 0; q < c->bin.n_rounds; ++q) {
         if (q > 0 && c->round_gen[q] == 0) continue;
-        a.seg_ranges[a.nseg] = q == 0 ? c->ranges.as<uint32_t>() : c->ranges_r[q].as<uint32_t>();
-        a.seg_ids[a.nseg] = c->ids.as<uint32_t>() + c->round_ids_off[q];
+        a.seg_ranges[a.nseg] = q == 0 ? c->ranges().as<uint32_t>() : c->ranges_r[q].as<uint32_t>();
+        a.seg_ids[a.nseg] = c->ids().as<uint32_t>() + c->round_ids_off[q];
         ++a.nseg;
     }
-    a.ranges = r == 0 ? c->ranges.as<uint32_t>() : c->ranges_r[r].as<uint32_t>(); a.ids = c->ids.as<uint32_t>() + c->round_ids_off[r];
+    a.ranges = r == 0 ? c->ranges().as<uint32_t>() : c->ranges_r[r].as<uint32_t>(); a.ids = c->ids().as<uint32_t>() + c->round_ids_off[r];
     if (bwd) c->rows_mut(c->g2d).into(a);
     a.tile_order = bwd || debug ? p.bwd_order : p.order; a.order_len = a.tile_order ? lpt_order_entries(c) : 0;
     a.parts = bwd ? p.bwd_parts : p.parts;
     a.split_ok = a.tile_order && p.split && !c->live.frame_capped;
     if (c->live.frame_capped && c->bin.n_rounds == 1) {
-        a.tile_ext = c->tile_ext.as<uint2>();
+        a.tile_ext = c->tile_ext().as<uint2>();
         if (!bwd) {
             a.cranges = c->cranges.as<uint32_t>(); a.cids = c->cids.as<uint32_t>(); a.clr = c->clr.as<uint16_t>();
-            a.ids_w = c->ids.as<uint32_t>(); a.sgx = c->bin.sgx; a.sbs = c->bin.sbs; a.ext_count = c->ext_count();
+            a.ids_w = c->ids().as<uint32_t>(); a.sgx = c->bin.sgx; a.sbs = c->bin.sbs; a.ext_count = c->ext_count();
         }
     }
     if (bwd ? p.bwd_segments : !debug) {
@@ -206,6 +206,7 @@
             if (redo) { if (int rc = enqueue_forward_round(c, 0)) return rc; }
         }
     }
+    c->fr.forward_marked(false);
     if (c->fwd_fills_g2d) c->live.g2d_clean = true;
     if (vs) vs->walk_written(c->counters_grid);
     if (int rc = build_frame_order(c)) return rc;
@@ -254,6 +255,7 @@
     }
     HIPCHK(c, c->g2d.ensure(c->g2d_bytes()));
     HIPCHK(c, c->ensure_bwd_counters());
+    if (!p.fused()) { if (int rc = frame_read(c)) return rc; }
     if (p.composite) {
         GsCompositeArgs a = composite_args(c, true, 0);
         a.dC = c->last_dC = dC_dev;
@@ -285,8 +287,9 @@
         HIPCHK(c, gs_launch_preprocess_bwd(b, c->cam, c->stream, mode));
     }
     if (p.host_sync) HIPCHK(c, hipStreamSynchronize(c->stream));
-    if (p.model_changes()) c->inputs_changed();
-    else c->reach(p.chain ? Stage::BACKWARD : Stage::COMPOSITE_ADJOINT);
+    c->fr.backward_enqueued();
+    if (p.model_changes()) { c->inputs_changed(); return model_written(c); }
+    c->reach(p.chain ? Stage::BACKWARD : Stage::COMPOSITE_ADJOINT);
     return GS_OK;
 }
 
diff --git a/gaussiansplat_amd/csrc/gs_api_debug.hip b/gaussiansplat_amd/csrc/gs_api_debug.hip
--- a/gaussiansplat_amd/csrc/gs_api_debug.hip
+++ b/gaussiansplat_amd/csrc/gs_api_debug.hip
@@ -38,12 +38,12 @@
         case GS_ARR_COV3D: if ((rc = need_dbg(gs_ctx::DBG_COV3D))) return rc; break;
         case GS_ARR_COV2D: if ((rc = need_dbg(gs_ctx::DBG_COV2D))) return rc; break;
         case GS_ARR_BBS: if ((rc = need_dbg(gs_ctx::DBG_BBS))) return rc; break;
-        case GS_ARR_INVCOV: src = c->invcov.p; need = sizeof(float) * 4 * n; break;
+        case GS_ARR_INVCOV: src = c->invcov().p; need = sizeof(float) * 4 * n; break;
         case GS_ARR_MU: case GS_ARR_RGB: case GS_ARR_SIG: {
             const size_t w = which == GS_ARR_MU ? 2 : which == GS_ARR_RGB ? 3 : 1;
             if ((size_t)bytes != sizeof(float) * w * n) return fail(c, GS_ERR_INVALID, "gs_get_array: size mismatch");
             std::vector<GsPayload> h(c->n1());
-            HIPCHK(c, hipMemcpyAsync(h.data(), c->payload.p, sizeof(GsPayload) * n, hipMemcpyDeviceToHost, c->stream));
+            HIPCHK(c, hipMemcpyAsync(h.data(), c->payload().p, sizeof(GsPayload) * n, hipMemcpyDeviceToHost, c->stream));
             HIPCHK(c, hipStreamSynchronize(c->stream));
             float *o = static_cast<float *>(dst);
             for (size_t g = 0; g < n; ++g) {
@@ -64,15 +64,15 @@
             for (size_t g = 0; g < n; ++g) o[g] = (uint32_t)g;
             return GS_OK;
         }
-        case GS_ARR_TILE_RANGES: src = c->ranges.p; need = sizeof(uint32_t) * 2 * c->ntiles(); break;
+        case GS_ARR_TILE_RANGES: src = c->ranges().p; need = sizeof(uint32_t) * 2 * c->ntiles(); break;
         case GS_ARR_SORTED_IDS: case GS_ARR_SORTED_KEYS: {
             const size_t ni = (size_t)c->n_inst, nt = (size_t)c->ntiles();
             const size_t w = which == GS_ARR_SORTED_IDS ? sizeof(uint32_t) : sizeof(uint64_t);
             if ((size_t)bytes != w * ni) return fail(c, GS_ERR_INVALID, "gs_get_array: size mismatch");
             std::vector<uint32_t> h(ni ? ni : 1), dk(c->n1()), rg(2 * c->ntiles1());
-            HIPCHK(c, hipMemcpyAsync(h.data(), c->ids.p, sizeof(uint32_t) * ni, hipMemcpyDeviceToHost, c->stream));
+            HIPCHK(c, hipMemcpyAsync(h.data(), c->ids().p, sizeof(uint32_t) * ni, hipMemcpyDeviceToHost, c->stream));
             HIPCHK(c, hipMemcpyAsync(dk.data(), c->depth_key.p, sizeof(uint32_t) * n, hipMemcpyDeviceToHost, c->stream));
-            HIPCHK(c, hipMemcpyAsync(rg.data(), c->ranges.p, sizeof(uint32_t) * 2 * nt, hipMemcpyDeviceToHost, c->stream));
+            HIPCHK(c, hipMemcpyAsync(rg.data(), c->ranges().p, sizeof(uint32_t) * 2 * nt, hipMemcpyDeviceToHost, c->stream));
             HIPCHK(c, hipStreamSynchronize(c->stream));
             if (which == GS_ARR_SORTED_IDS) {
                 std::memcpy(dst, h.data(), sizeof(uint32_t) * ni);
@@ -95,8 +95,8 @@
             std::vector<GsPayload> pay(c->n1());
             std::vector<float> ic(4 * c->n1());
             if (n) HIPCHK(c, hipMemcpyAsync(fixed ? (void *)fx.data() : (void *)fl.data(), c->g2d.p, c->g2d_bytes(), hipMemcpyDeviceToHost, c->stream));
-            if (n) HIPCHK(c, hipMemcpyAsync(pay.data(), c->payload.p, sizeof(GsPayload) * n, hipMemcpyDeviceToHost, c->stream));
-            if (n) HIPCHK(c, hipMemcpyAsync(ic.data(), c->invcov.p, sizeof(float) * 4 * n, hipMemcpyDeviceToHost, c->stream));
+            if (n) HIPCHK(c, hipMemcpyAsync(pay.data(), c->payload().p, sizeof(GsPayload) * n, hipMemcpyDeviceToHost, c->stream));
+            if (n) HIPCHK(c, hipMemcpyAsync(ic.data(), c->invcov().p, sizeof(float) * 4 * n, hipMemcpyDeviceToHost, c->stream));
             HIPCHK(c, hipStreamSynchronize(c->stream));
             for (size_t g = 0; g < n; ++g) {
                 float row[10];
@@ -277,11 +277,17 @@
     if (!c->live.frame_capped || c->bin.n_rounds != 1) return GS_OK;
     unsigned long long *d = c->counters.as<CounterBlock>()->scratch, h = 0;
     uint32_t e = 0;
-    HIPCHK(c, gs_launch_sum_listed(c->tile_ext.as<uint2>(), (int)c->ntiles(), d, c->stream));
+    HIPCHK(c, gs_launch_sum_listed(c->tile_ext().as<uint2>(), (int)c->ntiles(), d, c->stream));
     HIPCHK(c, hipMemcpyAsync(&h, d, sizeof(h), hipMemcpyDeviceToHost, c->stream));
     HIPCHK(c, hipMemcpyAsync(&e, c->ext_count(), sizeof(e), hipMemcpyDeviceToHost, c->stream));
     HIPCHK(c, hipStreamSynchronize(c->stream));
     out[0] = (int64_t)h; out[1] = (int64_t)e; out[2] = 1;
+    return GS_OK;
+}
+
+int gs_get_overlapped_frames(gs_ctx *c, int64_t *out) {
+    if (!c || !out) return GS_ERR_INVALID;
+    *out = c->fr.overlapped;
     return GS_OK;
 }
 
diff --git a/gaussiansplat_amd/csrc/gs_api_density.hip b/gaussiansplat_amd/csrc/gs_api_density.hip
--- a/gaussiansplat_amd/csrc/gs_api_density.hip
+++ b/gaussiansplat_amd/csrc/gs_api_density.hip
@@ -13,7 +13,7 @@
     if (bind_device(c)) return GS_ERR_HIP;
     GsDensityAccArgs a{};
     a.n = c->n;
-    a.payload = c->payload.as<GsPayload>(); a.invcov = c->invcov.as<float>();
+    a.payload = c->payload().as<GsPayload>(); a.invcov = c->invcov().as<float>();
     c->rows(c->g2d).into(a);
     a.half_w = 0.5f * (float)c->cam.W; a.half_h = 0.5f * (float)c->cam.H;
     a.grad_sum = st->grad_sum; a.count = st->count; a.max_extent = st->max_extent;
@@ -122,7 +122,7 @@
     if (bind_device(c)) return GS_ERR_HIP;
     HIPCHK(c, gs_launch_opacity_reset(const_cast<float *>(c->opac), max_logit, m_opac, v_opac, c->n, c->stream));
     c->inputs_changed();
-    return GS_OK;
+    return model_written(c);
 }
 
 }
diff --git a/gaussiansplat_amd/csrc/gs_api_features.hip b/gaussiansplat_amd/csrc/gs_api_features.hip
--- a/gaussiansplat_amd/csrc/gs_api_features.hip
+++ b/gaussiansplat_amd/csrc/gs_api_features.hip
@@ -13,7 +13,7 @@
 
 static int build_feature_payload(gs_ctx *c, const float *feat) {
     HIPCHK(c, c->feat_payload.ensure(sizeof(GsPayload) * c->n1()));
-    HIPCHK(c, gs_launch_feature_payload(c->payload.as<GsPayload>(), feat, c->n, c->feat_payload.as<GsPayload>(), c->stream));
+    HIPCHK(c, gs_launch_feature_payload(c->payload().as<GsPayload>(), feat, c->n, c->feat_payload.as<GsPayload>(), c->stream));
     return GS_OK;
 }
 
@@ -56,7 +56,7 @@
     a.trans = trans_out ? trans_out : c->feat_trans.as<float>();
     a.final_round = 1;
     HIPCHK(c, gs_launch_composite_fwd(a, c->stream));
-    return GS_OK;
+    return c->fr.bwd_behind ? frame_read(c) : GS_OK;
 }
 
 int gs_backward_features(gs_ctx *c, const float *feat, const float *image_f, const float *dF, float *d_feat, const gs_grads *grads) {
diff --git a/gaussiansplat_amd/csrc/gs_api_mcmc.hip b/gaussiansplat_amd/csrc/gs_api_mcmc.hip
--- a/gaussiansplat_amd/csrc/gs_api_mcmc.hip
+++ b/gaussiansplat_amd/csrc/gs_api_mcmc.hip
@@ -83,7 +83,7 @@
     }
     HIPCHK(c, gs_launch_mcmc_relocate(a, c->stream));
     c->inputs_changed();
-    return GS_OK;
+    return model_written(c);
 }
 
 int gs_mcmc_noise(gs_ctx *c, const float *z, float lr, float gate_k, float gate_t) {
@@ -102,7 +102,7 @@
     if (c->n == 0) return GS_OK;
     HIPCHK(c, gs_launch_mcmc_noise(const_cast<float *>(c->means), c->scales, c->quats, c->opac, z, c->n, lr, gate_k, gate_t, c->stream));
     c->inputs_changed();
-    return GS_OK;
+    return model_written(c);
 }
 
 int gs_mcmc_regularize(gs_ctx *c, const gs_grads *grads, float c_opacity, float c_scale) {
diff --git a/gaussiansplat_amd/csrc/gs_ctx.h b/gaussiansplat_amd/csrc/gs_ctx.h
--- a/gaussiansplat_amd/csrc/gs_ctx.h
+++ b/gaussiansplat_amd/csrc/gs_ctx.h
@@ -1,6 +1,7 @@
 #pragma once
 #include "../../include/gsplat.h"
 #include "gs_common.h"
+#include "gs_frame_overlap.h"
 
 #include <rccl/rccl.h>
 
@@ -63,8 +64,9 @@
     ~gs_ctx() {
         comm_release(this);
         for (auto &pair : ev) for (hipEvent_t e : pair) if (e) (void)hipEventDestroy(e);
-        for (hipEvent_t e : {ev_count, ev_main, ev_order}) if (e) (void)hipEventDestroy(e);
+        for (hipEvent_t e : {ev_count, ev_main, ev_order, ev_front, ev_fwd, ev_model}) if (e) (void)hipEventDestroy(e);
         if (side) (void)hipStreamDestroy(side);
+        if (front) (void)hipStreamDestroy(front);
         for (void *h : {(void *)pinned, (void *)pinned_split}) if (h) (void)hipHostFree(h);
         if (own_stream && stream) (void)hipStreamDestroy(stream);
     }
@@ -109,13 +111,19 @@
     size_t n1() const { return n ? (size_t)n : 1; }
     size_t pixels() const { return (size_t)cam.W * cam.H; }
 
-    DevBuf invcov;
-    DevBuf payload, depth_key, rect, pairs_a, pairs_b, perm, offsets, block_sums;
-    DevBuf inst_a, inst_b, table, digit_total, ranges, image, trans, g2d, stage_in;
+    DevBuf payload2[2], invcov2[2], ranges2[2], ids2[2], tile_ext2[2];
+    GsFrontState fr;
+    DevBuf &payload() { return payload2[fr.parity]; }
+    DevBuf &invcov() { return invcov2[fr.parity]; }
+    DevBuf &ranges() { return ranges2[fr.parity]; }
+    DevBuf &ids() { return ids2[fr.parity]; }
+    DevBuf &tile_ext() { return tile_ext2[fr.parity]; }
+    DevBuf depth_key, rect, pairs_a, pairs_b, perm, offsets, block_sums;
+    DevBuf inst_a, inst_b, table, digit_total, image, trans, g2d, stage_in;
     enum Dbg { DBG_TS, DBG_TPS, DBG_MU, DBG_COV3D, DBG_COV2D, DBG_INVCOV, DBG_BBS, DBG_COUNT };
     static constexpr size_t DBG_WIDTH[DBG_COUNT] = {4, 4, 2, 9, 4, 4, 4};
     DevBuf dbg[DBG_COUNT];
-    DevBuf ids, words, cs, diff;
+    DevBuf words, cs, diff;
     int64_t n_inst = 0;
     PinnedWords *pinned = nullptr;
     const float *last_dC = nullptr;
@@ -145,7 +153,7 @@
     std::vector<ViewSlot> slots;
     const uint32_t *last_walked = nullptr;
     int wave_slots = 5120;
-    DevBuf tile_nopen, smax, tile_ext, zero_tiles;
+    DevBuf tile_nopen, smax, zero_tiles;
     struct FrameLive {
         bool frame_capped = false;
         const uint32_t *cap_src = nullptr;
@@ -204,6 +212,12 @@
     hipStream_t side = nullptr;
     hipEvent_t ev_main = nullptr, ev_order = nullptr;
     bool order_pending = false;
+    hipStream_t front = nullptr;
+    hipEvent_t ev_front = nullptr;
+    hipEvent_t ev_fwd = nullptr;
+    hipEvent_t ev_model = nullptr;
+    bool model_ev_set = false;
+    hipStream_t fs() const { return fr.open ? front : stream; }
     bool pending_totals = false;
     int64_t n_coarse = 0;
     DevBuf tile_dead;
@@ -341,18 +355,20 @@
 }
 struct StageTimer {
     gs_ctx *c; int st; bool on;
-    StageTimer(gs_ctx *c_, int st_) : c(c_), st(st_), on(c_->cfg.profile_stages == 1 || c_->cfg.profile_stages == 2 + st_) {
+    hipStream_t where;
+    static bool front_half(int st) { return st < GS_STAGE_COMPOSITE_FWD; }
+    StageTimer(gs_ctx *c_, int st_) : c(c_), st(st_), on(c_->cfg.profile_stages == 1 || c_->cfg.profile_stages == 2 + st_), where(front_half(st_) ? c_->fs() : c_->stream) {
         if (on) {
             if (c->ev_fresh[st] && !harvest_stage(c, st)) {
                 (void)hipEventSynchronize(c->ev[st][1]);
                 (void)harvest_stage(c, st);
             }
             c->ev_frame[st] = c->frame_id;
-            (void)hipEventRecord(c->ev[st][0], c->stream);
+            (void)hipEventRecord(c->ev[st][0], where);
         }
     }
     ~StageTimer() {
-        if (on) { (void)hipEventRecord(c->ev[st][1], c->stream); c->ev_valid[st] = true; c->ev_fresh[st] = true; }
+        if (on) { (void)hipEventRecord(c->ev[st][1], where); c->ev_valid[st] = true; c->ev_fresh[st] = true; }
     }
 };
 
@@ -381,6 +397,11 @@
 inline uint32_t *key_range_of(const gs_ctx *c, int parity) { return c->key_range.as<uint32_t>() + (size_t)parity * gs_depth_range_parity_words(); }
 inline int order_index(const gs_ctx *c) { return c->view_slot >= 0 ? c->view_slot : GS_MAX_VIEW_SLOTS; }
 
+int begin_frame(gs_ctx *c);
+int join_front(gs_ctx *c, bool close);
+int wait_model_final(gs_ctx *c, hipStream_t s);
+int model_written(gs_ctx *c);
+int frame_read(gs_ctx *c);
 int settle_totals(gs_ctx *c, bool *redo, bool may_relist);
 int bin_round(gs_ctx *c, int r);
 int depth_order(gs_ctx *c);
diff --git a/gaussiansplat_amd/csrc/gs_frame_overlap.h b/gaussiansplat_amd/csrc/gs_frame_overlap.h
--- /dev/null
+++ b/gaussiansplat_amd/csrc/gs_frame_overlap.h
@@ -0,0 +1,46 @@
+#pragma once
+#include <cstdint>
+
+struct GsFrontInputs {
+    bool has_front;
+    bool side_streams;
+    bool model_events;
+    bool serial_flag;
+    int profile_stages;
+    bool two_level;
+    int n_rounds;
+};
+
+struct GsFrontState {
+    int parity = 0;
+    bool open = false;
+    bool fwd_marked = false;
+    bool bwd_behind = false;
+    bool model_dirty = false;
+    int64_t overlapped = 0;
+
+    bool may_overlap(const GsFrontInputs &i) const {
+        if (!i.has_front || !i.side_streams || !i.model_events) return false;
+        if (i.serial_flag || i.profile_stages == 1) return false;
+        if (!bwd_behind || !fwd_marked || model_dirty) return false;
+        return i.two_level && i.n_rounds == 1;
+    }
+    bool begin(const GsFrontInputs &i) {
+        const bool overlap = may_overlap(i);
+        open = false;
+        bwd_behind = false;
+        if (!overlap) { fwd_marked = false; return false; }
+        parity ^= 1;
+        open = true;
+        overlapped += 1;
+        return true;
+    }
+    bool plan_disagrees(bool two_level, int n_rounds) const { return open && !(two_level && n_rounds == 1); }
+    void binning_on_main() { if (!open) fwd_marked = false; }
+    bool close() { const bool was = open; open = false; return was; }
+    void forward_marked(bool recorded) { fwd_marked = recorded; model_dirty = false; }
+    void mark() { fwd_marked = true; }
+    void model_written() { model_dirty = true; }
+    void backward_enqueued() { bwd_behind = true; }
+    void stream_changed() { fwd_marked = false; }
+};
diff --git a/include/gsplat.h b/include/gsplat.h
--- a/include/gsplat.h
+++ b/include/gsplat.h
@@ -50,6 +50,7 @@
 #define GS_DEBUG_SUPER8 16
 #define GS_DEBUG_TINY_CAPS 4
 #define GS_DEBUG_NO_TAIL_FILL 32
+#define GS_DEBUG_SERIAL_FRAMES 64
 
 typedef struct gs_ctx gs_ctx;
 
@@ -259,6 +260,8 @@
 
 int gs_get_list_stats(gs_ctx *ctx, int64_t out[3]);
 
+int gs_get_overlapped_frames(gs_ctx *ctx, int64_t *out);
+
 int gs_get_tile_parts(gs_ctx *ctx);
 
 int gs_get_bin_path(gs_ctx *ctx);
```

New measurement: 892.8 Msplats/s, median of 6. +7.0%, better.
